# mbertagna/Galaxy-Deconv

Hardware: AMD Instinct MI355X
Metric: galaxies/sec (256x256, n_iters=8) - unrolled ADMM spectral engine (higher is better)
Workload: dtype f32; 1 GPU; Unrolled_ADMM(n_iters=8, llh='Gaussian') forward, denoiser=identity (spectral engine: SubNet + OTF + init_l2 + 8 ADMM iterations), batch 4096/GPU, 256x256 fp32 (BASELINE.json configs[2]/[3]); global_batch=4096, n_iters=8, llh=Gaussian, parallelism=dp1 (batch shards, no data-path collective), ranks_seen=1, backend=none, pipeline_streams=2, init=fused, k_psf_rows + k_gal_reg_init (one launch)

## Files before the change

### galaxy-deconv_amd/csrc/gd_engine.hip

```cpp
#include <hip/hip_runtime.h>

#include <algorithm>
#include <cstdio>
#include <cstdlib>
#include <cstring>
#include <map>
#include <mutex>
#include <string>
#include <vector>

#include "../../include/gdeconv.h"
#include "gd_fft.hpp"
#include "gd_subnet.hpp"

namespace gd {

struct GalScalar {
    const float* p;
    long long stride;
    __device__ __forceinline__ float operator()(int g) const { return p[(long long)g * stride]; }
};

struct Args {
    int N;
    float2* T;
    float2* otf;
    const float* y;
    const float* psf;
    long long psf_gstride;
    int h;
    const float* a0;
    const float* a1;
    const float* a2;
    float* o0;
    float* o1;
    float* o2;
    GalScalar alpha, rho1, rho2, rho2n;
    int llh;
    int last;
    int first;
    float* s_hh;
    float2* s_g;
    float2* s_u1;
    float2* s_w;
    int t_slot;
    float2* Tw;
    const float* ltl;
    long long ltl_gstride;
    int otf_bcast;
    float2* s_x;
    int gH, gW;
    int pw;
    int rev;
    int tail;
    GalScalar rho1n;
    const float* a3;
    float* o3;
    float* part;
    float* apart;
};

enum RowFwdMode { RF_ITER, RF_PSF_Y, RF_PSF_YP, RF_PSF_RAW, RF_PSF, RF_ONE, RF_TWO, RF_YA, RF_PSF_YAR,
                  RF_PADV, RF_PSF_YPAD, RF_PAD2,
                  RF_TRAIN_BWD,
                  RF_TRAINF_BWD };
enum ColMode { C_ITER, C_OTF_INIT, C_OTF_CONV, C_WIENER, C_OTF, C_CONV, C_CONVC, C_CONV2, C_FWD, C_INV,
               C_G_INIT, C_G_ITER, C_G_W1, C_G_ITER_F, C_G_ITER_L, C_G_ITER_FL,
               C_TIKHONOV, C_POWER, C_GX_INIT, C_GX, C_GX_BWD,
               C_TRAIN, C_TRAIN_BWD,
               C_OTF_BWD, C_XCORR,
               C_TRAINF, C_TRAINF_BWD };
enum RowInvMode { RI_ITER, RI_INIT, RI_OUT1, RI_OUT2, RI_RL_FINAL, RI_CROP, RI_CROP_BWD,
                  RI_TRAIN, RI_TRAIN_BWD,
                  RI_PSF_BWD,
                  RI_TRAINF };
enum RowInvFwdMode { RIF_CLAMP, RIF_RL_RATIO, RIF_RL_UPDATE };

constexpr int rows_per_block(int lpb, int L) {
    int rw = lpb < L ? lpb : L;
    while (L % rw || rw % 2) --rw;
    return rw;
}
constexpr int cmax(int x, int y) { return x > y ? x : y; }

template <int L>
struct Geo {
    static constexpr int F1 = Plan<L>::F1, F2 = Plan<L>::F2;
    static constexpr int K = L / 2 + 1;
    static constexpr int LPB = 256 / F1;
    static constexpr int RB = rows_per_block(LPB, L);
    static constexpr int RLD = L + 2;
    static constexpr int XCH = xch_elems<L>();
    static constexpr int COL_LDS = LPB * XCH;
    static_assert(L % RB == 0 && RB % 2 == 0, "rows per block must be even and divide L");
};

__device__ __forceinline__ size_t tidx(int g, int img, int k, int row, int K, int L) {
    return ((size_t)(g * 2 + img) * K + k) * L + row;
}

__device__ __forceinline__ float shifted_psf(const Args& a, int g, int r, int c, int L) {
    const int c0 = a.h >> 1;
    int i = r + c0, jj = c + c0;
    if (i >= L) i -= L;
    if (jj >= L) jj -= L;
    if (i >= a.h || jj >= a.h) return 0.0f;
    return a.psf[(long long)g * a.psf_gstride + (long long)i * a.h + jj];
}

__device__ __forceinline__ float v_step(int llh, float vt, float yp, float rho2, float alpha) {
    if (llh == GD_LLH_POISSON) {
        const float t1 = rho2 * vt - alpha;
        return 0.5f * (1.0f / rho2) * (-t1 + sqrtf(t1 * t1 + 4.0f * yp * rho2));
    }
    return (rho2 * vt + yp / alpha) / (1.0f + rho2);
}

__device__ __forceinline__ void v_step_grad(int llh, float vt, float yp, float rho2, float alpha, float& dvt,
                                            float& drho) {
    if (llh == GD_LLH_POISSON) {
        const float t1 = rho2 * vt - alpha;
        const float s = sqrtf(t1 * t1 + 4.0f * yp * rho2);
        const float sm = t1 > 0.f ? 4.0f * yp * rho2 / (s + t1) : s - t1;
        const float ir = 1.0f / rho2;
        const float v = 0.5f * ir * sm;
        dvt = -0.5f * sm / s;
        drho = (yp - rho2 * v * vt) * ir / s - v * ir;
        return;
    }
    const float q = 1.0f / (1.0f + rho2);
    dvt = rho2 * q;
    drho = (vt - yp / alpha) * q * q;
}

__device__ __forceinline__ void v_step_grad_in(int llh, float vt, float yp, float rho2, float alpha, float& dy,
                                               float& dal) {
    if (llh == GD_LLH_POISSON) {
        const float t1 = rho2 * vt - alpha;
        const float s = sqrtf(t1 * t1 + 4.0f * yp * rho2);
        const float sm = t1 > 0.f ? 4.0f * yp * rho2 / (s + t1) : s - t1;
        dy = 1.0f / s;
        dal = 0.5f * sm / (rho2 * s);
        return;
    }
    const float q = 1.0f / (alpha * (1.0f + rho2));
    dy = q;
    dal = -yp * q / alpha;
}

template <int L, int NI, int RBX = 0>
struct RowGeo {
    using G = Geo<L>;
    static constexpr int RB = RBX ? RBX : rows_per_block(2 * G::LPB / NI, L);
    static constexpr int PAIRS = RB / 2;
    static constexpr int LINES = NI * PAIRS;
    static constexpr int THREADS = LINES * G::F1;
    static constexpr int LDS = cmax(cmax(LINES * G::RLD, LINES * G::XCH), (NI * RB * L + 1) / 2);
    static_assert(RB % 2 == 0 && L % RB == 0, "row pairs must tile the image");
    static_assert(THREADS <= 1024, "block too large");
};

template <int L, typename R>
__device__ __forceinline__ void split_store(const Args& a, const float2* rowbuf, int g, int row0, int tid) {
    using G = Geo<L>;
    for (int idx = tid; idx < R::LINES * G::K; idx += R::THREADS) {
        const int m = idx % R::PAIRS, t = idx / R::PAIRS;
        const int k = t % G::K, im = t / G::K;
        const int line = im * R::PAIRS + m;
        const float2 C = rowbuf[line * G::RLD + k];
        const float2 D = rowbuf[line * G::RLD + (k == 0 ? 0 : L - k)];
        *reinterpret_cast<float4*>((a.Tw ? a.Tw : a.T) + tidx(g, im + a.t_slot, k, row0 + 2 * m, G::K, L)) =
            make_float4(0.5f * (C.x + D.x), 0.5f * (C.y - D.y), 0.5f * (C.y + D.y), 0.5f * (D.x - C.x));
    }
}

template <int L, typename R>
__device__ __forceinline__ void gather_rows(const Args& a, float2* rowbuf, int g, int row0, int tid) {
    using G = Geo<L>;
    for (int idx = tid; idx < R::LINES * G::K; idx += R::THREADS) {
        const int m = idx % R::PAIRS, t = idx / R::PAIRS;
        const int k = t % G::K, im = t / G::K;
        const float4 q = *reinterpret_cast<const float4*>(a.T + tidx(g, im, k, row0 + 2 * m, G::K, L));
        float2 Re = make_float2(q.x, q.y), Ro = make_float2(q.z, q.w);
        const bool self = (k == 0) || (2 * k == L);
        if (self) {
            Re.y = 0.f;
            Ro.y = 0.f;
        }
        const int line = im * R::PAIRS + m;
        rowbuf[line * G::RLD + k] = make_float2(Re.x - Ro.y, Re.y + Ro.x);
        if (!self) rowbuf[line * G::RLD + (L - k)] = make_float2(Re.x + Ro.y, Ro.x - Re.y);
    }
}

template <int MODE>
struct RfTraits {
    static constexpr int NI = (MODE == RF_PSF || MODE == RF_ONE || MODE == RF_YA || MODE == RF_PADV) ? 1 : 2;
};

__device__ __forceinline__ float4 ld4(const float* p) { return *reinterpret_cast<const float4*>(p); }
__device__ __forceinline__ void st4(float* p, float4 v) { *reinterpret_cast<float4*>(p) = v; }
__device__ __forceinline__ float f4(const float4& v, int i) { return i == 0 ? v.x : i == 1 ? v.y : i == 2 ? v.z : v.w; }
__device__ __forceinline__ void f4set(float4& v, int i, float x) {
    if (i == 0) v.x = x; else if (i == 1) v.y = x; else if (i == 2) v.z = x; else v.w = x;
}

template <int L, int MODE>
__device__ __forceinline__ float4 rf_source4(const Args& a, int g, int im, int r, int c, size_t pix) {
    if constexpr (MODE == RF_ITER) {
        if (im == 0) {
            const float4 z = ld4(a.a0 + pix), u = ld4(a.a1 + pix);
            return make_float4(z.x - u.x, z.y - u.y, z.z - u.z, z.w - u.w);
// ... 50 lines not shown
    } else if constexpr (MODE == RF_YA) {
        const float4 y = ld4(a.y + pix);
        const float al = a.alpha(g);
        return make_float4(fmaxf(y.x, 0.f) / al, fmaxf(y.y, 0.f) / al, fmaxf(y.z, 0.f) / al, fmaxf(y.w, 0.f) / al);
    } else {
        return ld4((im == 0 ? a.a0 : a.a1) + pix);
    }
}

template <int L>
__device__ __forceinline__ float4 rf_train_bwd4(const Args& a, int g, int im, size_t pix, float& acc) {
    if (im == 0) {
        const float4 gz = ld4(a.a0 + pix);
        if (a.last) {
            const float sc = a.llh == GD_LLH_POISSON ? a.alpha(g) : 1.f;
            return make_float4(gz.x * sc, gz.y * sc, gz.z * sc, gz.w * sc);
        }
        const float4 gu = ld4(a.a1 + pix);
        return make_float4(2.f * gz.x + gu.x, 2.f * gz.y + gu.y, 2.f * gz.z + gu.z, 2.f * gz.w + gu.w);
    }
    if (a.last) return make_float4(0.f, 0.f, 0.f, 0.f);
    const float4 gw = ld4(a.a2 + pix), vt = ld4(a.a3 + pix), y = ld4(a.y + pix);
    const float al = a.alpha(g), r2n = a.rho2n(g);
    float4 ghx, wp;
#pragma unroll
    for (int e = 0; e < 4; ++e) {
        float dvt, drho;
        v_step_grad(a.llh, f4(vt, e), fmaxf(f4(y, e), 0.f), r2n, al, dvt, drho);
        const float gwe = f4(gw, e), gvt = gwe * dvt;
        acc += gwe * drho;
        f4set(ghx, e, 2.f * gvt - gwe);
        f4set(wp, e, gwe - gvt);
    }
    st4(a.o2 + pix, wp);
    return ghx;
}

template <int L>
__device__ __forceinline__ float4 rf_trainf_bwd4(const Args& a, int g, int im, size_t pix, float& acc, float& acc2) {
    if (im == 0) {
        const float4 gz = ld4(a.a0 + pix);
        if (a.last) {
            float sc = 1.f;
            if (a.llh == GD_LLH_POISSON) {
                const float4 x = ld4(a.a3 + pix);
                sc = a.alpha(g);
                acc2 += gz.x * x.x + gz.y * x.y + gz.z * x.z + gz.w * x.w;
            }
            return make_float4(gz.x * sc, gz.y * sc, gz.z * sc, gz.w * sc);
        }
        const float4 gu = ld4(a.a1 + pix);
        return make_float4(2.f * gz.x + gu.x, 2.f * gz.y + gu.y, 2.f * gz.z + gu.z, 2.f * gz.w + gu.w);
    }
    if (a.last) {
        st4(a.o3 + pix, make_float4(0.f, 0.f, 0.f, 0.f));
        return make_float4(0.f, 0.f, 0.f, 0.f);
    }
    const float4 gw = ld4(a.a2 + pix), vt = ld4(a.a3 + pix), y = ld4(a.y + pix);
    const float al = a.alpha(g), r2n = a.rho2n(g);
    float4 ghx, wp, gy;
#pragma unroll
    for (int e = 0; e < 4; ++e) {
        float dvt, drho, dy, dal;
        const float ye = f4(y, e), yp = fmaxf(ye, 0.f);
        v_step_grad(a.llh, f4(vt, e), yp, r2n, al, dvt, drho);
        v_step_grad_in(a.llh, f4(vt, e), yp, r2n, al, dy, dal);
        const float gwe = f4(gw, e), gvt = gwe * dvt;
        acc += gwe * drho;
        acc2 += gwe * dal;
        f4set(ghx, e, 2.f * gvt - gwe);
        f4set(wp, e, gwe - gvt);
        f4set(gy, e, ye > 0.f ? gwe * dy : 0.f);
    }
    st4(a.o2 + pix, wp);
    st4(a.o3 + pix, gy);
    return ghx;
}

template <int L, int MODE, int RBX = 0>
__global__ __launch_bounds__((RowGeo<L, RfTraits<MODE>::NI, RBX>::THREADS)) void k_row_fwd(Args a) {
    constexpr int NI = RfTraits<MODE>::NI;
    using G = Geo<L>;
    using R = RowGeo<L, NI, RBX>;
    constexpr int F1 = G::F1, F2 = G::F2;
    __shared__ float2 tw[L];
    __shared__ __attribute__((aligned(16))) float2 lds[R::LDS];
    const int tid = threadIdx.x;
    const int blocks_per_g = L / R::RB;
    const int g = blockIdx.x / blocks_per_g;
    const int row0 = (blockIdx.x - g * blocks_per_g) * R::RB;
    const int line = tid / F1, j = tid - line * F1;
    const int im = line / R::PAIRS, m = line - im * R::PAIRS;
    fill_twiddles<L>(tw, tid, R::THREADS);
    float* stage = reinterpret_cast<float*>(lds);
    [[maybe_unused]] float acc = 0.f, acc2 = 0.f;
    for (int q = tid * 4; q < NI * R::RB * L; q += R::THREADS * 4) {
        const int imq = q / (R::RB * L), rem = q - imq * (R::RB * L);
        const int rr = rem / L, c = rem - rr * L;
        const size_t pix = ((size_t)g * L + row0 + rr) * L + c;
        if constexpr (MODE == RF_TRAIN_BWD) st4(stage + q, rf_train_bwd4<L>(a, g, imq, pix, acc));
        else if constexpr (MODE == RF_TRAINF_BWD) st4(stage + q, rf_trainf_bwd4<L>(a, g, imq, pix, acc, acc2));
        else st4(stage + q, rf_source4<L, MODE>(a, g, imq, row0 + rr, c, pix));
    }
    if constexpr (MODE == RF_TRAINF_BWD) {
        __shared__ float red2[R::THREADS];
        red2[tid] = acc2;
        __syncthreads();
        if (tid < 64) {
            float sum = 0.f;
            for (int i = tid; i < R::THREADS; i += 64) sum += red2[i];
            red2[tid] = sum;
        }
        __syncthreads();
        if (tid < R::RB) {
            float sum = 0.f;
            if (tid == 0)
                for (int i = 0; i < (R::THREADS < 64 ? R::THREADS : 64); ++i) sum += red2[i];
            a.apart[(size_t)g * L + row0 + tid] = sum;
        }
    }
    if constexpr (MODE == RF_TRAIN_BWD || MODE == RF_TRAINF_BWD) {
        __shared__ float red[R::THREADS];
        red[tid] = acc;
        __syncthreads();
        if (tid < 64) {
            float sum = 0.f;
            for (int i = tid; i < R::THREADS; i += 64) sum += red[i];
            red[tid] = sum;
        }
        __syncthreads();
        if (tid < R::RB) {
            float sum = 0.f;
            if (tid == 0)
                for (int i = 0; i < (R::THREADS < 64 ? R::THREADS : 64); ++i) sum += red[i];
            a.part[(size_t)g * (2 * G::K + L) + 2 * G::K + row0 + tid] = sum;
        }
    }
    __syncthreads();
    float2 v[F2];
#pragma unroll
    for (int s = 0; s < F2; ++s) {
        const int c = j + F1 * s;
        v[s] = make_float2(stage[(im * R::RB + 2 * m) * L + c], stage[(im * R::RB + 2 * m + 1) * L + c]);
    }
    __syncthreads();
    line_fft<L, false>(v, j, lds + line * G::XCH, tw);
    __syncthreads();
#pragma unroll
    for (int s = 0; s < F2; ++s) lds[line * G::RLD + j + F1 * s] = v[s];
    __syncthreads();
    split_store<L, R>(a, lds, g, row0, tid);
}

template <int L, bool TO_STATE = false>
__global__ __launch_bounds__(256) void k_psf_rows(Args a) {
    using G = Geo<L>;
    constexpr int F1 = G::F1, F2 = G::F2, LPB = G::LPB, K = G::K;
    __shared__ float2 tw[L];
    __shared__ __attribute__((aligned(16))) float2 lds[cmax(LPB * G::RLD, LPB * G::XCH)];
    const int tid = threadIdx.x, line = tid / F1, j = tid - line * F1;
    const int h = a.h, c0 = h >> 1, pairs = h >> 1;
    const int blocks_per_g = (pairs + LPB - 1) / LPB;
    const int g = blockIdx.x / blocks_per_g;
    const int p0 = (blockIdx.x - g * blocks_per_g) * LPB;
    fill_twiddles<L>(tw, tid, 256);
    const int p = p0 + line;
    const float* ps = a.psf + (long long)g * a.psf_gstride + (long long)(2 * p) * h;
    float2 v[F2];
#pragma unroll
    for (int s = 0; s < F2; ++s) {
        int jj = j + F1 * s + c0;
        if (jj >= L) jj -= L;
        v[s] = (p < pairs && jj < h) ? make_float2(ps[jj], ps[h + jj]) : make_float2(0.f, 0.f);
    }
    __syncthreads();
    line_fft<L, false>(v, j, lds + line * G::XCH, tw);
    __syncthreads();
#pragma unroll
    for (int s = 0; s < F2; ++s) lds[line * G::RLD + j + F1 * s] = v[s];
    __syncthreads();
    float2* P = TO_STATE ? a.s_u1 + (size_t)g * K * L : a.T + tidx(g, 1, 0, 0, K, L);
    for (int idx = tid; idx < LPB * K; idx += 256) {
        const int m = idx % LPB, k = idx / LPB;
        if (p0 + m >= pairs) continue;
        const float2 C = lds[m * G::RLD + k];
        const float2 D = lds[m * G::RLD + (k == 0 ? 0 : L - k)];
        float4 o = make_float4(0.5f * (C.x + D.x), 0.5f * (C.y - D.y), 0.5f * (C.y + D.y), 0.5f * (D.x - C.x));
        if (TO_STATE && k == 0) {
            const float2 Cn = lds[m * G::RLD + L / 2];
            o = make_float4(C.x, Cn.x, C.y, Cn.y);
        }
        *reinterpret_cast<float4*>(P + (size_t)k * h + 2 * (p0 + m)) = o;
    }
}

template <int MODE>
struct ColTraits {
    static constexpr bool IN2 = (MODE == C_ITER || MODE == C_OTF_INIT || MODE == C_OTF_CONV ||
                                 MODE == C_WIENER || MODE == C_CONV2 || MODE == C_TIKHONOV || MODE == C_GX_INIT ||
                                 MODE == C_GX_BWD || MODE == C_TRAIN || MODE == C_TRAIN_BWD || MODE == C_XCORR ||
                                 MODE == C_TRAINF || MODE == C_TRAINF_BWD);
    static constexpr bool OUT2 = (MODE == C_ITER || MODE == C_CONV2 || MODE == C_TRAIN || MODE == C_TRAIN_BWD ||
                                  MODE == C_TRAINF || MODE == C_TRAINF_BWD);
    static constexpr bool HAS_OUT = (MODE != C_OTF && MODE != C_FWD && MODE != C_G_W1 && MODE != C_POWER &&
                                     MODE != C_XCORR);
    static constexpr bool STORE_OTF = (MODE == C_OTF_INIT || MODE == C_OTF_CONV || MODE == C_OTF);
    static constexpr bool LOAD_OTF = (MODE == C_ITER || MODE == C_CONV || MODE == C_CONVC || MODE == C_CONV2 ||
                                      MODE == C_TRAIN || MODE == C_TRAIN_BWD || MODE == C_TRAINF || MODE == C_TRAINF_BWD);
    static constexpr bool FWD = (MODE != C_INV && MODE != C_OTF_BWD);
};

#ifndef GD_RCP_DIV
#define GD_RCP_DIV 1
#endif
__device__ __forceinline__ float ld_s(const float* p) { return *p; }
__device__ __forceinline__ float2 ld_s(const float2* p) { return *p; }
__device__ __forceinline__ void st_s(float* p, float v) { __builtin_nontemporal_store(v, p); }
__device__ __forceinline__ void st_s(float2* p, float2 v) {
    unsigned long long u;
    __builtin_memcpy(&u, &v, 8);
    __builtin_nontemporal_store(u, reinterpret_cast<unsigned long long*>(p));
}
typedef float f4v __attribute__((ext_vector_type(4)));
template <int L>
__device__ __forceinline__ int sidx_c(int ky) {
    if constexpr (L == 256) {
        const int j = ky & 15, s = ky >> 4;
        return 32 * (s >> 1) + 2 * j + (s & 1);
    } else {
        return ky;
    }
}
template <int L>
__device__ __forceinline__ int sidx_h(int ky) {
    if constexpr (L == 256) {
        const int j = ky & 15, s = ky >> 4;
        return 64 * (s >> 2) + 4 * j + (s & 3);
    } else {
        return ky;
    }
}
template <int L>
__device__ __forceinline__ size_t sflat_c(size_t o) {
    if constexpr (L == 256) return (o & ~size_t(255)) | (size_t)sidx_c<L>((int)(o & 255));
    else return o;
}
template <int L>
__device__ __forceinline__ size_t sflat_h(size_t o) {
    if constexpr (L == 256) return (o & ~size_t(255)) | (size_t)sidx_h<L>((int)(o & 255));
    else return o;
}
__device__ __forceinline__ float2 w1_value(float hh, float2 Gk, float2 Xk, float r2n) {
    const float d0 = 1.0f + r2n;
#if GD_RCP_DIV
    const float rd = __builtin_amdgcn_rcpf(d0);
    return make_float2((r2n * (hh * Xk.x + 0.0f) + Gk.x) * rd, (r2n * (hh * Xk.y + 0.0f) + Gk.y) * rd);
#else
    return make_float2((r2n * (hh * Xk.x + 0.0f) + Gk.x) / d0, (r2n * (hh * Xk.y + 0.0f) + Gk.y) / d0);
#endif
}

struct GState {
    float hh;
    float2 G, U1, W;
};
template <int L, bool FIRST, bool LAST>
__device__ __forceinline__ GState gauss_load(const Args& a, size_t o) {
    GState st;
    const size_t oc = sflat_c<L>(o);
    st.hh = ld_s(a.s_hh + sflat_h<L>(o));
    st.G = make_float2(0.f, 0.f);
    st.U1 = make_float2(0.f, 0.f);
    if constexpr (!LAST || FIRST) st.G = ld_s(a.s_g + oc);
    if constexpr (!FIRST) st.U1 = ld_s(a.s_u1 + oc);
    st.W = ld_s(a.s_w + oc);
    return st;
}
template <bool LAST>
__device__ __forceinline__ float2 gauss_math_w(float hh, float2 Gk, float2 U1, float2 Wt, float2 Zk, float r1, float r2,
                                               float r2w, float r2n, float inv_n, float2& U1o, float2& Wo) {
    const float lhs = r1 * hh + r2;
    const float2 A = csub(Zk, U1);
#if GD_RCP_DIV
    const float rl = __builtin_amdgcn_rcpf(lhs);
    const float2 X = make_float2((r1 * A.x + r2w * Wt.x) * rl, (r1 * A.y + r2w * Wt.y) * rl);
#else
    const float2 X = make_float2((r1 * A.x + r2w * Wt.x) / lhs, (r1 * A.y + r2w * Wt.y) / lhs);
#endif
    if constexpr (LAST) return cscale(X, inv_n);
    const float2 U1n = csub(cadd(U1, X), Zk);
    const float2 HHX = cscale(X, hh);
    const float2 U2t = csub(HHX, Wt);
    const float d = 1.0f + r2n;
#if GD_RCP_DIV
    const float rd = __builtin_amdgcn_rcpf(d);
    const float2 Vt = make_float2((r2n * (HHX.x + U2t.x) + Gk.x) * rd, (r2n * (HHX.y + U2t.y) + Gk.y) * rd);
#else
    const float2 Vt = make_float2((r2n * (HHX.x + U2t.x) + Gk.x) / d, (r2n * (HHX.y + U2t.y) + Gk.y) / d);
#endif
    U1o = U1n;
    Wo = csub(Vt, U2t);
    return cscale(cadd(X, U1n), inv_n);
}
template <bool LAST>
__device__ __forceinline__ float2 gauss_math(float hh, float2 Gk, float2 U1, float2 Wt, float2 Zk, float r1, float r2,
                                             float r2n, float inv_n, float2& U1o, float2& Wo) {
    return gauss_math_w<LAST>(hh, Gk, U1, Wt, Zk, r1, r2, r2, r2n, inv_n, U1o, Wo);
}
__device__ __forceinline__ float2 gauss_math_rt(float hh, float2 Gk, float2 U1, float2 Wt, float2 Zk, float r1,
                                                float r2, float r2w, float r2n, float inv_n, float2& U1o, float2& Wo,
                                                bool last) {
    if (last) return gauss_math_w<true>(hh, Gk, U1, Wt, Zk, r1, r2, r2w, r2n, inv_n, U1o, Wo);
    return gauss_math_w<false>(hh, Gk, U1, Wt, Zk, r1, r2, r2w, r2n, inv_n, U1o, Wo);
}
__device__ __forceinline__ float2 gauss_tail_c(float2 U1n, float2 Wn, float r1n, float r2n) {
    return make_float2(r2n * Wn.x - r1n * U1n.x, r2n * Wn.y - r1n * U1n.y);
}
template <int L, bool FIRST, bool LAST>
__device__ __forceinline__ float2 gauss_iter_st(const Args& a, size_t o, float2 Zk, const GState& st, float r1,
                                                float r2, float r2n, bool valid, float inv_n) {
    const float hh = st.hh;
    const float2 U1 = st.U1, Gk = st.G;
    float2 Wt = st.W;
    if constexpr (FIRST) Wt = w1_value(hh, Gk, st.W, r2);
    const float lhs = r1 * hh + r2;
    const float2 A = csub(Zk, U1);
#if GD_RCP_DIV
    const float rl = __builtin_amdgcn_rcpf(lhs);
    const float2 X = make_float2((r1 * A.x + r2 * Wt.x) * rl, (r1 * A.y + r2 * Wt.y) * rl);
#else
    const float2 X = make_float2((r1 * A.x + r2 * Wt.x) / lhs, (r1 * A.y + r2 * Wt.y) / lhs);
#endif
    if constexpr (LAST) return cscale(X, inv_n);
    const float2 U1n = csub(cadd(U1, X), Zk);
// ... 144 lines not shown
            if (valid) {
                a.s_hh[sflat_h<L>(ob + ky)] = hh;
                a.s_g[sflat_c<L>(ob + ky)] = a.llh == GD_LLH_POISSON ? Hk2 : Gk;
            }
            const float lhs = hh + 1.0f / al;
            P[s] = cscale(make_float2(Gk.x / lhs, Gk.y / lhs), inv_n);
        } else if constexpr (giter) {
            P[s] = gauss_iter_elem<L, gfirst, glast>(a, ob + ky, P[s], r1, r2, r2n, valid, inv_n);
        } else if constexpr (MODE == C_G_W1) {
            if (valid)
                a.s_w[sflat_c<L>(ob + ky)] = a.llh == GD_LLH_POISSON ? cmul(a.s_g[sflat_c<L>(ob + ky)], P[s]) : P[s];
        } else if constexpr (MODE == C_WIENER) {
            const float HtH = Hk.x * Hk.x + Hk.y * Hk.y;
            const float div = HtH + 350.0f / al;
            const float2 num = cmulc(Q[s], Hk);
            P[s] = cscale(make_float2(num.x / div, num.y / div), inv_n);
        } else if constexpr (MODE == C_TIKHONOV) {
            const float HtH = Hk.x * Hk.x + Hk.y * Hk.y;
            const float div = a.ltl ? HtH + lam * a.ltl[(size_t)g * a.ltl_gstride + (size_t)kx * L + ky] : HtH + lam;
            const float2 num = cmulc(Q[s], Hk);
            P[s] = cscale(make_float2(num.x / div, num.y / div), inv_n);
        } else if constexpr (MODE == C_GX_INIT) {
            const float2 Hk2 = P[s];
            const float hh = Hk2.x * Hk2.x + Hk2.y * Hk2.y;
            const float2 Gk = cmulc(Q[s], Hk2);
            if (valid) {
                a.s_hh[ob + ky] = hh;
                a.s_g[ob + ky] = Gk;
            }
            const float lhs = hh + 1.0f / al;
            P[s] = cscale(make_float2(Gk.x / lhs, Gk.y / lhs), inv_n);
        } else if constexpr (MODE == C_GX) {
            const float hh = a.s_hh[ob + ky];
            const float2 Gk = a.s_g[ob + ky];
            const float lhs = rgx + hh;
            const float2 rhs = cadd(Gk, P[s]);
            const float2 X = make_float2(rhs.x / lhs, rhs.y / lhs);
            if (a.s_w && valid) a.s_w[ob + ky] = X;
            P[s] = cscale(X, inv_n);
        } else if constexpr (MODE == C_GX_BWD) {
            const float hh = a.s_hh[ob + ky];
            const float D = rgx + hh;
            const float2 X = a.s_w[ob + ky];
            const float2 d = csub(Q[s], X);
            const float wk = (kx == 0 || 2 * kx == L) ? 1.f : 2.f;
            drho += wk * (P[s].x * d.x + P[s].y * d.y) / D;
            P[s] = cscale(make_float2(P[s].x / D, P[s].y / D), inv_n);
        } else if constexpr (MODE == C_POWER) {
            if (valid) a.s_hh[ob + ky] = P[s].x * P[s].x + P[s].y * P[s].y;
        } else if constexpr (MODE == C_OTF_CONV) {
            P[s] = cscale(cmul(Q[s], Hk), inv_n);
        } else if constexpr (MODE == C_CONV) {
            P[s] = cscale(cmul(P[s], Hk), inv_n);
        } else if constexpr (MODE == C_CONVC) {
            P[s] = cscale(cmulc(P[s], Hk), inv_n);
        } else if constexpr (MODE == C_CONV2) {
            P[s] = cscale(cmul(P[s], Hk), inv_n);
            Q[s] = cscale(cmul(Q[s], Hk), inv_n);
        } else if constexpr (MODE == C_INV) {
            P[s] = cscale(P[s], inv_n);
        } else if constexpr (MODE == C_OTF_BWD) {
            P[s] = cscale(P[s], (kx == 0 || 2 * kx == L) ? 1.f : 0.5f);
        } else if constexpr (MODE == C_XCORR) {
            const float wk = ((kx == 0 || 2 * kx == L) ? 1.f : 2.f) * inv_n;
            if (valid) a.otf[ob + ky] = cscale(a.last ? cmulc(Q[s], P[s]) : cmulc(P[s], Q[s]), wk);
        }
    }
    if constexpr (MODE == C_GX_BWD) {
#pragma unroll
        for (int off = F1 / 2; off > 0; off >>= 1) drho += __shfl_xor(drho, off, F1);
        if (valid && j == 0) a.o2[(size_t)g * K + kx] = drho * inv_n;
    }
    if constexpr (MODE == C_TRAIN_BWD || MODE == C_TRAINF_BWD) {
#pragma unroll
        for (int off = F1 / 2; off > 0; off >>= 1) drho += __shfl_xor(drho, off, F1);
        if (valid && j == 0) {
            float* pg = a.part + (size_t)g * (2 * K + L);
            pg[kx] = -(r2 / r1) * (drho * inv_n);
            pg[K + kx] = drho * inv_n;
        }
    }
    if constexpr (TR::HAS_OUT && MODE != C_FWD && VAR != 1) {
        line_fft<L, true, CLEAN, CDPP>(P, j, my, tw);
        if constexpr (TR::OUT2) line_fft<L, true, CLEAN, CDPP>(Q, j, my, tw);
    }
    if (valid) {
        if constexpr (MODE == C_FWD) {
#pragma unroll
            for (int s = 0; s < F2; ++s) a.T[c0 + j + F1 * s] = P[s];
        } else if constexpr (TR::HAS_OUT) {
#pragma unroll
            for (int s = 0; s < F2; ++s) {
                a.T[c0 + j + F1 * s] = P[s];
                if constexpr (TR::OUT2) a.T[c1 + j + F1 * s] = Q[s];
            }
        }
    }
}

__device__ __forceinline__ int opaque(int v) {
    asm volatile("" : "+v"(v));
    return v;
}

#if GD_FUSED_TRACE
__device__ unsigned long long* g_fused_trace;
#define GD_TRACE(k)                                                                                   \
    if (tid == 0) g_fused_trace[(size_t)blockIdx.x * 16 + (k)] = __builtin_amdgcn_s_memrealtime()
#else
#define GD_TRACE(k)
#endif

template <int L>
struct FusedGeo {
    static constexpr int F1 = Plan<L>::F1, F2 = Plan<L>::F2, K = L / 2 + 1;
    static constexpr int THREADS = 1024, LINES = THREADS / F1;
    static constexpr int NP = L / 2, PPL = NP / LINES;
    static constexpr int KS = L / 4;
    static constexpr int SLD = 2 * KS + 4;
    static constexpr int ALD = KS + 2;
    static constexpr int XCH = xch_elems<L>();
    static constexpr int U = cmax(cmax(NP * SLD, L * ALD), LINES * XCH);
    static_assert(LINES == KS, "one column per line and slice");
    static_assert(NP == 2 * LINES && PPL == 2, "two row pairs per line; half the rows per inverse pass");
    static_assert(KS % F1 == 0 && (L / 2) % F1 == 0, "slice edges on lane-register boundaries");
    static_assert(L <= THREADS && (NP * KS) % THREADS == 0, "Nyquist column: one element per thread");
};

template <int L, int SLD = FusedGeo<L>::SLD>
__device__ __forceinline__ void fused_gather(const float2* S, int c, int j, float2 (&C)[FusedGeo<L>::F2]) {
    using FG = FusedGeo<L>;
    c = opaque(c);
    j = opaque(j);
#pragma unroll
    for (int s = 0; s < FG::F2; ++s) {
        const int y = j + FG::F1 * s;
        const float2 u = S[(y >> 1) * SLD + c], v = S[(y >> 1) * SLD + FG::KS + c];
        C[s] = (y & 1) ? make_float2(0.5f * (u.y + v.y), 0.5f * (v.x - u.x))
                       : make_float2(0.5f * (u.x + v.x), 0.5f * (u.y - v.y));
    }
}

__device__ __forceinline__ void lds_barrier() {
    __builtin_amdgcn_fence(__ATOMIC_RELEASE, "workgroup", "local");
    __builtin_amdgcn_s_barrier();
    __builtin_amdgcn_fence(__ATOMIC_ACQUIRE, "workgroup", "local");
}

template <int L>
__device__ __forceinline__ void init_hload(const Args& a, float2 (&Hc)[FusedGeo<L>::F2], int g, int kx, int j) {
    using FG = FusedGeo<L>;
    static_assert((L & (L - 1)) == 0, "power-of-two side");
    const int h = a.h, c0p = h >> 1;
    const float2* P0 = a.s_u1 + (size_t)g * FG::K * L + (size_t)opaque(kx) * h;
    j = opaque(j);
    static_assert(FG::F1 == 16 && FG::F2 == 16, "sparse OTF column for 16 x 16 lines");
#pragma unroll
    for (int s = 0; s < FG::F2; ++s) {
        Hc[s] = make_float2(0.f, 0.f);
        if (s < 2 || s >= FG::F2 - 2) {
            const int i = (j + FG::F1 * s + c0p) & (L - 1);
            if (i < h) Hc[s] = P0[i];
        }
    }
}
template <int L>
__device__ __forceinline__ void init_hload4(const Args& a, float2 (&h4)[4], int g, int kx, int j) {
    using FG = FusedGeo<L>;
    const int h = a.h, c0p = h >> 1;
    const float2* P0 = a.s_u1 + (size_t)g * FG::K * L + (size_t)opaque(kx) * h;
    j = opaque(j);
#pragma unroll
    for (int t = 0; t < 4; ++t) {
        const int s = t < 2 ? t : FG::F2 - 4 + t;
        const int i = (j + FG::F1 * s + c0p) & (L - 1);
        h4[t] = i < h ? P0[i] : make_float2(0.f, 0.f);
    }
}
template <int L>
__device__ __forceinline__ void init_hcol(float2 (&Hc)[FusedGeo<L>::F2], const float2 (&h4)[4]) {
    using FG = FusedGeo<L>;
#pragma unroll
    for (int s = 0; s < FG::F2; ++s) Hc[s] = make_float2(0.f, 0.f);
    Hc[0] = h4[0];
    Hc[1] = h4[1];
    Hc[FG::F2 - 2] = h4[2];
    Hc[FG::F2 - 1] = h4[3];
}
template <int L>
__device__ __forceinline__ float2 init_bin(const Args& a, size_t o, float2 Yk, float2 Hk, float al, float inv_n,
                                           bool store_h = false) {
    const float hh = Hk.x * Hk.x + Hk.y * Hk.y;
    const float2 Gk = cmulc(Yk, Hk);
    a.s_hh[sflat_h<L>(o)] = hh;
    a.s_g[sflat_c<L>(o)] = store_h ? Hk : Gk;
    const float lhs = hh + 1.0f / al;
    return cscale(make_float2(Gk.x / lhs, Gk.y / lhs), inv_n);
}
template <int L>
__device__ __forceinline__ void w1_bin(const Args& a, size_t o, float2 Xk) {
    a.s_w[sflat_c<L>(o)] = a.llh == GD_LLH_POISSON ? cmul(a.s_g[sflat_c<L>(o)], Xk) : Xk;
}
#include "gd_galreg.hpp"
#include "gd_rlreg.hpp"
#include "gd_poisreg.hpp"

template <int L>
__device__ __forceinline__ void small_split(const float2 (&v)[Plan<L>::F2], int j, float2* my, float2* D, int r) {
    constexpr int F1 = Plan<L>::F1, F2 = Plan<L>::F2, K = L / 2 + 1;
#pragma unroll
    for (int s = 0; s < F2; ++s) my[j + F1 * s] = v[s];
    wave_lds_sync();
    for (int k = j; k < K; k += F1) {
        const float2 C = my[k], Dm = my[k == 0 ? 0 : L - k];
        D[k * L + r] = make_float2(0.5f * (C.x + Dm.x), 0.5f * (C.y - Dm.y));
        D[k * L + r + 1] = make_float2(0.5f * (C.y + Dm.y), 0.5f * (Dm.x - C.x));
    }
    wave_lds_sync();
}
template <int L>
__device__ __forceinline__ void small_gather(const float2* D, int j, int r, float2 (&v)[Plan<L>::F2]) {
    constexpr int F1 = Plan<L>::F1, F2 = Plan<L>::F2;
#pragma unroll
    for (int s = 0; s < F2; ++s) {
        const int k = j + F1 * s;
        const bool self = (k == 0) || (2 * k == L);
        float2 be, bo;
        if (2 * k <= L) {
            be = D[k * L + r];
            bo = D[k * L + r + 1];
        } else {
            be = cconj(D[(L - k) * L + r]);
            bo = cconj(D[(L - k) * L + r + 1]);
        }
        if (self) {
            be.y = 0.f;
            bo.y = 0.f;
        }
        v[s] = make_float2(be.x - bo.y, be.y + bo.x);
    }
}

#ifndef GD_SMALL_ZPRE
#define GD_SMALL_ZPRE 1
#endif
template <int L, bool FIRST, bool LAST>
__global__ __launch_bounds__(256) void k_gal_small(Args a) {
    constexpr int F1 = Plan<L>::F1, F2 = Plan<L>::F2, K = L / 2 + 1, LINES = 256 / F1, XCH = xch_elems<L>();
    static_assert(XCH >= L + 2, "row buffer inside the exchange area");
    constexpr float inv_n = float(1.0 / double(L * L));
    __shared__ float2 tw[L];
    __shared__ float2 S[K * L];
    __shared__ float2 xch[LINES * XCH];
    const int tid = threadIdx.x, line = tid / F1, j = tid - line * F1;
    const int g = blockIdx.x;
    float2* my = xch + line * XCH;
    GD_TRACE(0);
    constexpr bool ZPRE = GD_SMALL_ZPRE && L / 2 <= LINES;
    const float* z = a.a0 + (size_t)g * L * L;
    float2 zv[ZPRE ? F2 : 1];
    if (ZPRE && line < L / 2) {
#pragma unroll
        for (int s = 0; s < (ZPRE ? F2 : 0); ++s)
            zv[s] = make_float2(z[(2 * line) * L + j + F1 * s], z[(2 * line + 1) * L + j + F1 * s]);
    }
    fill_twiddles<L>(tw, tid, 256);
    const float r1 = a.rho1(g), r2 = a.rho2(g), r2n = LAST ? 0.f : a.rho2n(g);
    constexpr bool PRE = L <= 64;
    GState pre[PRE ? F2 : 1];
    if (PRE && line < K) {
        const size_t ob = ((size_t)g * K + line) * L + j;
#pragma unroll
        for (int s = 0; s < (PRE ? F2 : 0); ++s) pre[s] = gauss_load<L, FIRST, LAST>(a, ob + F1 * s);
    }
    __syncthreads();
    GD_TRACE(1);

    for (int p = line; p < L / 2; p += LINES) {
        float2 v[F2];
        if constexpr (ZPRE) {
#pragma unroll
            for (int s = 0; s < F2; ++s) v[s] = zv[s];
        } else {
#pragma unroll
            for (int s = 0; s < F2; ++s) v[s] = make_float2(z[(2 * p) * L + j + F1 * s], z[(2 * p + 1) * L + j + F1 * s]);
        }
        line_fft<L, false>(v, j, my, tw);
        small_split<L>(v, j, my, S, 2 * p);
    }
    __syncthreads();
    GD_TRACE(2);

    for (int kx = line; kx < K; kx += LINES) {
        float2 v[F2];
#pragma unroll
        for (int s = 0; s < F2; ++s) v[s] = S[kx * L + j + F1 * s];
        line_fft<L, false>(v, j, my, tw);
        const size_t ob = ((size_t)g * K + kx) * L + j;
        if (PRE && kx == line) {
#pragma unroll
            for (int s = 0; s < (PRE ? F2 : 0); ++s)
                v[s] = gauss_iter_st<L, FIRST, LAST>(a, ob + F1 * s, v[s], pre[s], r1, r2, r2n, true, inv_n);
        } else {
#pragma unroll
            for (int s = 0; s < F2; ++s)
                v[s] = gauss_iter_elem<L, FIRST, LAST>(a, ob + F1 * s, v[s], r1, r2, r2n, true, inv_n);
        }
        line_fft<L, true>(v, j, my, tw);
#pragma unroll
        for (int s = 0; s < F2; ++s) S[kx * L + j + F1 * s] = v[s];
    }
    __syncthreads();
    GD_TRACE(3);

    float* out = a.o0 + (size_t)g * L * L;
    for (int p = line; p < L / 2; p += LINES) {
        float2 v[F2];
        small_gather<L>(S, j, 2 * p, v);
        line_fft<L, true>(v, j, my, tw);
#pragma unroll
        for (int s = 0; s < F2; ++s) {
            out[(2 * p) * L + j + F1 * s] = v[s].x;
            out[(2 * p + 1) * L + j + F1 * s] = v[s].y;
// ... 1016 lines not shown
__global__ __launch_bounds__(256) void k_sparse_power(const int* rc, const float* vals, int ntaps, float* out,
                                                      int H, int W, int K) {
    const int idx = blockIdx.x * 256 + threadIdx.x;
    if (idx >= K * H) return;
    const int kx = idx / H, ky = idx - kx * H;
    const long long HW = (long long)H * W;
    double re = 0.0, im = 0.0;
    for (int t = 0; t < ntaps; ++t) {
        const long long ph = ((long long)ky * rc[2 * t] * W + (long long)kx * rc[2 * t + 1] * H) % HW;
        double sn, cs;
        sincospi(-2.0 * double(ph) / double(HW), &sn, &cs);
        re += double(vals[t]) * cs;
        im += double(vals[t]) * sn;
    }
    out[idx] = float(re * re + im * im);
}

thread_local std::string g_last_error;

constexpr const char* kRowFwdName = "k_row_fwd";
constexpr const char* kPsfRowsName = "k_psf_rows";
constexpr const char* kColName = "k_col";
constexpr const char* kRowInvName = "k_row_inv";
constexpr const char* kRowInvFwdName = "k_row_invfwd";
constexpr const char* kGalRegName = "k_gal_reg";
constexpr const char* kGalInitName = "k_gal_init";
constexpr const char* kGalSmallName = "k_gal_small";
constexpr const char* kGalSmallInitName = "k_gal_small_init";

inline int fail(int code, const char* msg) {
    g_last_error = msg;
    return code;
}
inline int fail(int code, const std::string& msg) {
    g_last_error = msg;
    return code;
}

inline int check_launch(const char* what) {
    hipError_t e = hipGetLastError();
    if (e != hipSuccess) {
        g_last_error = std::string(what) + ": " + hipGetErrorString(e);
        return GD_ERR_HIP;
    }
    return GD_OK;
}

struct ProfEntry {
    std::string name;
    hipEvent_t start, stop;
};
struct ProfStat {
    double ms = 0.0;
    long long launches = 0;
};
std::mutex g_prof_mu;
int g_prof_level = 0;
std::vector<ProfEntry> g_prof_pending;
std::vector<hipEvent_t> g_prof_pool;
std::map<std::string, ProfStat> g_prof_stats;

inline hipEvent_t prof_event() {
    if (!g_prof_pool.empty()) {
        hipEvent_t e = g_prof_pool.back();
        g_prof_pool.pop_back();
        return e;
    }
    hipEvent_t e;
    (void)hipEventCreate(&e);
    return e;
}

struct ProfScope {
    bool on;
    ProfEntry ent;
    hipStream_t st;
    ProfScope(const std::string& name, hipStream_t s, int level = 2) : on(false), st(s) {
        std::lock_guard<std::mutex> lk(g_prof_mu);
        if (g_prof_level < level) return;
        on = true;
        ent.name = name;
        ent.start = prof_event();
        ent.stop = prof_event();
        (void)hipEventRecord(ent.start, st);
    }
    ~ProfScope() {
        if (!on) return;
        (void)hipEventRecord(ent.stop, st);
        std::lock_guard<std::mutex> lk(g_prof_mu);
        g_prof_pending.push_back(ent);
    }
};

template <int L>
struct Launcher {
    using G = Geo<L>;
    template <int NI>
    static int row_grid(int N) { return N * (L / RowGeo<L, NI>::RB); }
    static int col_grid(int N) { return (N * G::K + G::LPB - 1) / G::LPB; }
    static std::string nm(const char* k, int mode) {
        return std::string(k) + "<" + std::to_string(L) + "," + std::to_string(mode) + ">";
    }

    template <int MODE>
    static int rf(const Args& a, hipStream_t st) {
        ProfScope ps(nm(kRowFwdName, MODE), st);
        hipLaunchKernelGGL((k_row_fwd<L, MODE>), dim3(row_grid<RfTraits<MODE>::NI>(a.N)), dim3(RowGeo<L, RfTraits<MODE>::NI>::THREADS), 0, st, a);
        return check_launch("k_row_fwd");
    }
    static int psf_rows(const Args& a, hipStream_t st) {
        ProfScope ps(nm(kPsfRowsName, 0), st);
        const int bpg = (a.h / 2 + G::LPB - 1) / G::LPB;
        hipLaunchKernelGGL((k_psf_rows<L>), dim3(a.N * bpg), dim3(256), 0, st, a);
        return check_launch("k_psf_rows");
    }
    template <int MODE>
    static int col(const Args& a, hipStream_t st) {
        ProfScope ps(nm(kColName, MODE), st);
        hipLaunchKernelGGL((k_col<L, MODE>), dim3(col_grid(a.N)), dim3(256), 0, st, a);
        return check_launch("k_col");
    }
    template <int MODE>
    static int ri(const Args& a, hipStream_t st) {
        ProfScope ps(nm(kRowInvName, MODE), st);
        hipLaunchKernelGGL((k_row_inv<L, MODE>), dim3(row_grid<RiTraits<MODE>::NI>(a.N)), dim3(RowGeo<L, RiTraits<MODE>::NI>::THREADS), 0, st, a);
        return check_launch("k_row_inv");
    }
    static int psf_rows_state(const Args& a, hipStream_t st) {
        ProfScope ps(nm(kPsfRowsName, 1), st);
        const int bpg = (a.h / 2 + G::LPB - 1) / G::LPB;
        hipLaunchKernelGGL((k_psf_rows<L, true>), dim3(a.N * bpg), dim3(256), 0, st, a);
        return check_launch("k_psf_rows");
    }
    template <bool FIRST, bool LAST>
    static int gal_small_v(const Args& a, hipStream_t st) {
        ProfScope ps(nm(kGalSmallName, FIRST + 2 * LAST), st);
        if constexpr (L == 48)
            hipLaunchKernelGGL((k_gal_small_p<L, 8, 6, FIRST, LAST>), dim3(a.N), dim3(256), 0, st, a);
        else
            hipLaunchKernelGGL((k_gal_small<L, FIRST, LAST>), dim3(a.N), dim3(256), 0, st, a);
        return check_launch("k_gal_small");
    }
    static int gal_small_init(const Args& a, hipStream_t st) {
        ProfScope ps(nm(kGalSmallInitName, 0), st);
        hipLaunchKernelGGL((k_gal_small_init<L>), dim3(a.N), dim3(256), 0, st, a);
        return check_launch("k_gal_small_init");
    }
    static int gal_small(const Args& a, hipStream_t st) {
        if (a.first) return a.last ? gal_small_v<true, true>(a, st) : gal_small_v<true, false>(a, st);
        return a.last ? gal_small_v<false, true>(a, st) : gal_small_v<false, false>(a, st);
    }
    static int gal_reg(const Args& a, hipStream_t st) {
        ProfScope ps(nm(kGalRegName, a.first + 2 * a.last), st);
        if (a.tail == 1)
            hipLaunchKernelGGL((k_gal_reg<L, false, true>), dim3(a.N), dim3(RegGeo<L>::THREADS), 0, st, a);
        else
            hipLaunchKernelGGL((k_gal_reg<L>), dim3(a.N), dim3(RegGeo<L>::THREADS), 0, st, a);
        return check_launch("k_gal_reg");
    }
    static int pois_a(const Args& a, hipStream_t st) {
        ProfScope ps(nm("k_pois_a", a.first + 2 * a.last), st);
        hipLaunchKernelGGL((k_gal_reg<L, true>), dim3(a.N), dim3(RegGeo<L>::THREADS), 0, st, a);
        return check_launch("k_gal_reg<POIS>");
    }
    static int pois_b(const Args& a, int init, hipStream_t st) {
        ProfScope ps(nm("k_pois_b", init), st);
        hipLaunchKernelGGL((k_pois_b<L>), dim3(a.N), dim3(RegGeo<L>::THREADS), 0, st, a, init);
        return check_launch("k_pois_b");
    }
    static int gal_reg_init_pois(const Args& a, hipStream_t st) {
        ProfScope ps(nm(kGalInitName, 5), st);
        hipLaunchKernelGGL((k_gal_reg_init<L, true>), dim3(a.N), dim3(RegGeo<L>::THREADS), 0, st, a);
        return check_launch("k_gal_reg_init<POIS>");
    }
    static int rl_reg(const Args& a, int n_iters, hipStream_t st) {
        ProfScope ps(nm("k_rl_reg", 0), st);
        hipLaunchKernelGGL((k_rl_reg<L>), dim3(a.N), dim3(RegGeo<L>::THREADS), 0, st, a, n_iters);
        return check_launch("k_rl_reg");
    }
    static int gal_reg_init(const Args& a, hipStream_t st) {
        ProfScope ps(nm(kGalInitName, 4), st);
        hipLaunchKernelGGL((k_gal_reg_init<L>), dim3(a.N), dim3(RegGeo<L>::THREADS), 0, st, a);
        return check_launch("k_gal_reg_init");
    }
    template <int MODE>
    static int rif(const Args& a, hipStream_t st) {
        ProfScope ps(nm(kRowInvFwdName, MODE), st);
        hipLaunchKernelGGL((k_row_invfwd<L, MODE>), dim3(row_grid<1>(a.N)), dim3(RowGeo<L, 1>::THREADS), 0, st, a);
        return check_launch("k_row_invfwd");
    }
};

#define GD_TRY(x)                    \
    do {                             \
        int _rc = (x);               \
        if (_rc != GD_OK) return _rc; \
    } while (0)

size_t g_chunk_bytes = size_t(96) << 20;
int g_pipe_streams = 2;
constexpr int kMaxPipe = 8;
int g_fused = 1;
int g_fused_rl = 1;
int g_subnet_fused_max = 256;
int g_sri_map = 0;
int g_fused_init = 1;
int g_fused_min_n = 96;
int g_combined_tail = [] {
    const char* e = std::getenv("GD_COMBINED_TAIL");
    return (e && e[0] == '0' && e[1] == '\0') ? 0 : 1;
}();
int g_pois2_min_n = 192;
int g_rl_min_n = 96;

constexpr int kCapSets = 64;
struct PipeRes {
    bool ok = false;
    hipStream_t st[kMaxPipe];
    hipEvent_t fork;
    hipEvent_t join[kMaxPipe];
    std::mutex mu;
};
PipeRes g_pipe[64];
std::mutex g_pipe_mu;
struct CapRes {
    hipStream_t st[kMaxPipe];
    hipEvent_t cfork[kCapSets];
    hipEvent_t cjoin[kCapSets][kMaxPipe];
    int cpos = 0;
};
thread_local CapRes* t_cap[64];

thread_local int g_capture_pipe_override = -1;
inline int capture_pipeline_mode() {
    static const int mode = [] {
        const char* e = std::getenv("GD_CAPTURE_PIPELINE");
        const int m = e ? std::atoi(e) : 0;
        return m == 2 ? 2 : 0;
    }();
    return g_capture_pipe_override >= 0 ? g_capture_pipe_override : mode;
}

inline CapRes* cap_res() {
    int dev = 0;
    if (hipGetDevice(&dev) != hipSuccess || dev < 0 || dev >= 64) return nullptr;
    if (t_cap[dev]) return t_cap[dev];
    CapRes* r = new CapRes();
    for (int i = 0; i < kMaxPipe; ++i)
        if (hipStreamCreateWithFlags(&r->st[i], hipStreamNonBlocking) != hipSuccess) return nullptr;
    for (int c = 0; c < kCapSets; ++c) {
        if (hipEventCreateWithFlags(&r->cfork[c], hipEventDisableTiming) != hipSuccess) return nullptr;
        for (int i = 0; i < kMaxPipe; ++i)
            if (hipEventCreateWithFlags(&r->cjoin[c][i], hipEventDisableTiming) != hipSuccess) return nullptr;
    }
    t_cap[dev] = r;
    return r;
}

inline PipeRes* pipe_res() {
    int dev = 0;
    if (hipGetDevice(&dev) != hipSuccess || dev < 0 || dev >= 64) return nullptr;
    std::lock_guard<std::mutex> lk(g_pipe_mu);
    PipeRes& r = g_pipe[dev];
    if (!r.ok) {
        for (int i = 0; i < kMaxPipe; ++i) {
            if (hipStreamCreateWithFlags(&r.st[i], hipStreamNonBlocking) != hipSuccess) return nullptr;
            if (hipEventCreateWithFlags(&r.join[i], hipEventDisableTiming) != hipSuccess) return nullptr;
        }
        if (hipEventCreateWithFlags(&r.fork, hipEventDisableTiming) != hipSuccess) return nullptr;
        r.ok = true;
    }
    return &r;
}

template <int L>
constexpr bool has_fused() { return L == 256; }

inline Args offset_args(const Args& a, int g0, int n, int H, int W) {
    Args b = a;
    b.N = n;
    const size_t img = (size_t)g0 * H * W;
    const size_t spec = (size_t)g0 * (W / 2 + 1) * H;
    if (b.otf && !b.otf_bcast) b.otf += spec;
    if (b.s_hh) b.s_hh += spec;
    if (b.s_g) b.s_g += spec;
    if (b.s_u1) b.s_u1 += spec;
    if (b.s_w) b.s_w += spec;
    if (b.ltl) b.ltl += (long long)g0 * a.ltl_gstride;
    if (b.Tw) b.Tw += 2 * spec;
    if (b.y) b.y += img;
    if (b.a0) b.a0 += img;
    if (b.a1) b.a1 += img;
    if (b.a2) b.a2 += img;
    if (b.o0) b.o0 += img;
    if (b.o1) b.o1 += img;
    if (b.o2) b.o2 += img;
    if (b.a3) b.a3 += img;
    if (b.o3) b.o3 += img;
    if (b.part) b.part += (size_t)g0 * (2 * (W / 2 + 1) + H);
    if (b.apart) b.apart += (size_t)g0 * H;
    if (b.psf) b.psf += (long long)g0 * a.psf_gstride;
    GalScalar* gs[] = {&b.alpha, &b.rho1, &b.rho2, &b.rho2n};
    for (GalScalar* x : gs)
        if (x->p) x->p += (long long)g0 * x->stride;
    return b;
}

template <typename F>
int for_chunks_hw(const Args& a, int H, int W, hipStream_t st, F&& f) {
    const size_t tgal = (size_t)2 * (W / 2 + 1) * H * sizeof(float2);
    int G = a.N;
    if (g_chunk_bytes) {
        const size_t g = g_chunk_bytes / tgal;
        G = (int)(g < 1 ? 1 : (g > (size_t)a.N ? (size_t)a.N : g));
    }
    if (G >= a.N) return f(a, st);
    int S = g_pipe_streams < kMaxPipe ? g_pipe_streams : kMaxPipe;
    if (S > a.N / G) S = a.N / G;
    hipStreamCaptureStatus cap = hipStreamCaptureStatusNone;
    const bool capturing = S > 1 && hipStreamIsCapturing(st, &cap) == hipSuccess && cap != hipStreamCaptureStatusNone;
    if (capturing && capture_pipeline_mode() != 2) S = 1;
    PipeRes* r = (S > 1 && !capturing) ? pipe_res() : nullptr;
    CapRes* cr = (S > 1 && capturing) ? cap_res() : nullptr;
    if (!r && !cr) S = 1;
    std::unique_lock<std::mutex> lk;
    if (r) lk = std::unique_lock<std::mutex>(r->mu);
    hipEvent_t fork = nullptr;
    hipEvent_t* join = nullptr;
    hipStream_t* streams = nullptr;
    if (S > 1) {
        if (cr) {
            const int c = cr->cpos;
            cr->cpos = (c + 1) % kCapSets;
            fork = cr->cfork[c];
            join = cr->cjoin[c];
            streams = cr->st;
        } else {
            fork = r->fork;
            join = r->join;
            streams = r->st;
        }
        if (hipEventRecord(fork, st) != hipSuccess) return fail(GD_ERR_HIP, "pipeline fork");
        for (int i = 0; i < S; ++i)
            if (hipStreamWaitEvent(streams[i], fork, 0) != hipSuccess) return fail(GD_ERR_HIP, "pipeline fork");
    }
    int rc = GD_OK;
    for (int g0 = 0, c = 0; g0 < a.N && rc == GD_OK; g0 += G, ++c) {
        const int n = (a.N - g0 < G) ? a.N - g0 : G;
        Args b = offset_args(a, g0, n, H, W);
        b.T = a.T + (size_t)(c % S) * G * 2 * (W / 2 + 1) * H;
        rc = f(b, S > 1 ? streams[c % S] : st);
    }
    if (S > 1) {
        for (int i = 0; i < S; ++i) {
            if (hipEventRecord(join[i], streams[i]) != hipSuccess || hipStreamWaitEvent(st, join[i], 0) != hipSuccess)
                return fail(GD_ERR_HIP, "pipeline join");
        }
    }
    return rc;
}
template <typename F>
int for_chunks(const Args& a, int L, hipStream_t st, F&& f) {
    return for_chunks_hw(a, L, L, st, std::forward<F>(f));
}

#ifndef GD_REG_REV
#define GD_REG_REV 1
#endif
#ifndef GD_POIS_SMALL
#define GD_POIS_SMALL 1
#endif
inline bool pois_split(int H, int W) {
    return GD_POIS_SMALL && g_fused && g_fused_init && H == W &&
           (H == 32 || H == 48 || H == 64 || H == 80 || H == 96 || H == 112);
}
template <int L>
int pois_small_init_launch(const Args& a, hipStream_t st) {
    using PL = PoisSmallPlan<L>;
    ProfScope ps("k_pois_small_init<" + std::to_string(L) + ">", st);
    if (pois_split(L, L)) hipLaunchKernelGGL((k_pois_small_init<L, PL::TP, PL::TQ, PL::NT, true>), dim3(a.N), dim3(PL::NT), 0, st, a);
    else hipLaunchKernelGGL((k_pois_small_init<L, PL::TP, PL::TQ, PL::NT, false>), dim3(a.N), dim3(PL::NT), 0, st, a);
    return check_launch("k_pois_small_init");
}
template <int L>
int pois_small_launch(const Args& a, hipStream_t st) {
    using PL = PoisSmallPlan<L>;
    static const std::string names[4] = {"k_pois_small<" + std::to_string(L) + ",MID>", "k_pois_small<" + std::to_string(L) + ",FIRST>",
                                         "k_pois_small<" + std::to_string(L) + ",LAST>",
                                         "k_pois_small<" + std::to_string(L) + ",FIRST_LAST>"};
    const bool first = a.first && pois_split(L, L);
    ProfScope ps(names[first + 2 * a.last], st);
    if (first) {
        if (a.last) hipLaunchKernelGGL((k_pois_small<L, PL::TP, PL::TQ, PL::NT, true, true>), dim3(a.N), dim3(PL::NT), 0, st, a);
        else hipLaunchKernelGGL((k_pois_small<L, PL::TP, PL::TQ, PL::NT, false, true>), dim3(a.N), dim3(PL::NT), 0, st, a);
    } else {
        if (a.last) hipLaunchKernelGGL((k_pois_small<L, PL::TP, PL::TQ, PL::NT, true>), dim3(a.N), dim3(PL::NT), 0, st, a);
        else hipLaunchKernelGGL((k_pois_small<L, PL::TP, PL::TQ, PL::NT, false>), dim3(a.N), dim3(PL::NT), 0, st, a);
    }
    return check_launch("k_pois_small");
}

#ifndef GD_MID_EXTRA
#define GD_MID_EXTRA 1
#endif
template <int L>
int gal_mid_launch_t(const Args& a, hipStream_t st);
template <int L>
int gal_mid_init_launch_t(const Args& a, hipStream_t st);
template <int L>
struct Ops {
    static constexpr size_t IMG = (size_t)L * L * 4, HALF = (size_t)(L / 2 + 1) * L * 8;
    using Lc = Launcher<L>;
    static int psf_to_otf(Args a, hipStream_t st) {
        GD_TRY(Lc::template rf<RF_PSF>(a, st));
        return Lc::template col<C_OTF>(a, st);
    }
    static int conv(Args a, int conj, hipStream_t st) {
        GD_TRY(Lc::template rf<RF_ONE>(a, st));
        GD_TRY(conj ? Lc::template col<C_CONVC>(a, st) : Lc::template col<C_CONV>(a, st));
        return Lc::template ri<RI_OUT1>(a, st);
    }
    static int rfft2(Args a, hipStream_t st) {
        GD_TRY(Lc::template rf<RF_ONE>(a, st));
        return Lc::template col<C_FWD>(a, st);
    }
    static int irfft2(Args a, hipStream_t st) {
        GD_TRY(Lc::template col<C_INV>(a, st));
        return Lc::template ri<RI_OUT1>(a, st);
    }
    static int psf_to_otf_bwd(Args a, hipStream_t st) {
        GD_TRY(Lc::template col<C_OTF_BWD>(a, st));
        return Lc::template ri<RI_PSF_BWD>(a, st);
    }
    static int conv_bwd_otf(Args a, hipStream_t st) {
        GD_TRY(Lc::template rf<RF_TWO>(a, st));
        return Lc::template col<C_XCORR>(a, st);
    }
    static int admm_init_pois2(Args a0, hipStream_t st0) {
        if (g_fused_init && a0.h <= 64) {
            GD_TRY(Lc::psf_rows_state(a0, st0));
            GD_TRY(Lc::gal_reg_init_pois(a0, st0));
        } else {
            GD_TRY(for_chunks(a0, L, st0, [&](const Args& a, hipStream_t st) {
                Args b = a;
                GD_TRY(Lc::template rf<RF_YA>(b, st));
                GD_TRY(Lc::psf_rows(b, st));
                GD_TRY(Lc::template col<C_G_INIT>(b, st));
                b.o0 = a.o2;
                b.t_slot = 1;
                GD_TRY(Lc::template rif<RIF_CLAMP>(b, st));
                return Lc::template col<C_G_W1>(b, st);
            }));
        }
        Args b = a0;
        b.s_x = a0.s_w;
        return Lc::pois_b(b, 1, st0);
    }
    static int admm_iter_pois2(Args a, hipStream_t st0) {
        GD_TRY(Lc::pois_a(a, st0));
        if (a.last) return GD_OK;
        return Lc::pois_b(a, 0, st0);
    }
    static int admm_init(Args a0, hipStream_t st0) {
        if constexpr (L <= 112) {
            if (GD_POIS_SMALL && g_fused_init) return pois_small_init_launch<L>(a0, st0);
        }
        return for_chunks(a0, L, st0, [&](const Args& a, hipStream_t st) {
            Args b = a;
            GD_TRY(Lc::template rf<RF_PSF_Y>(b, st));
            GD_TRY(Lc::template col<C_OTF_INIT>(b, st));
            b.o0 = a.o2;
            GD_TRY(Lc::template rif<RIF_CLAMP>(b, st));
            GD_TRY(Lc::template col<C_CONV>(b, st));
            return Lc::template ri<RI_INIT>(a, st);
        });
    }
    static int admm_init_gauss(Args a0, hipStream_t st0) {
        if constexpr (GD_MID_EXTRA && (L == 96 || L == 128)) {
            if (g_fused && g_fused_init) return gal_mid_init_launch_t<L>(a0, st0);
        }
        if constexpr (L <= 96) {
            if (g_fused) return Lc::gal_small_init(a0, st0);
        }
        if constexpr (has_fused<L>()) {
            if (g_fused_init && a0.h <= 64 && a0.N >= g_fused_min_n) {
                GD_TRY(Lc::psf_rows_state(a0, st0));
                return Lc::gal_reg_init(a0, st0);
            }
        }
        return for_chunks(a0, L, st0, [&](const Args& a, hipStream_t st) {
            Args b = a;
            GD_TRY(Lc::template rf<RF_YA>(b, st));
            GD_TRY(Lc::psf_rows(b, st));
            GD_TRY(Lc::template col<C_G_INIT>(b, st));
            b.o0 = a.o2;
            b.t_slot = 1;
            GD_TRY(Lc::template rif<RIF_CLAMP>(b, st));
            return Lc::template col<C_G_W1>(b, st);
        });
    }
    static int admm_iter_gauss(Args a, hipStream_t st0) {
        if constexpr (has_fused<L>()) {
            if (g_fused && a.N >= g_fused_min_n) return Lc::gal_reg(a, st0);
        }
        if constexpr (GD_MID_EXTRA && (L == 96 || L == 128)) {
            if (g_fused) return gal_mid_launch_t<L>(a, st0);
        }
        if constexpr (L <= 128) {
            if (g_fused) return Lc::gal_small(a, st0);
        }
        return for_chunks(a, L, st0, [&](const Args& b, hipStream_t st) {
            GD_TRY(Lc::template rf<RF_ONE>(b, st));
            if (b.first)
                GD_TRY(b.last ? Lc::template col<C_G_ITER_FL>(b, st) : Lc::template col<C_G_ITER_F>(b, st));
            else
                GD_TRY(b.last ? Lc::template col<C_G_ITER_L>(b, st) : Lc::template col<C_G_ITER>(b, st));
            return Lc::template ri<RI_OUT1>(b, st);
        });
    }
    static int admm_iter(Args a0, hipStream_t st0) {
        if constexpr (L <= 112) {
            if (GD_POIS_SMALL && g_fused) return pois_small_launch<L>(a0, st0);
        }
        return for_chunks(a0, L, st0, [&](const Args& a, hipStream_t st) {
            GD_TRY(Lc::template rf<RF_ITER>(a, st));
            GD_TRY(Lc::template col<C_ITER>(a, st));
            return Lc::template ri<RI_ITER>(a, st);
        });
    }
    static int train_init(Args a0, hipStream_t st0) {
        return for_chunks(a0, L, st0, [&](const Args& a, hipStream_t st) {
            GD_TRY(Lc::template rf<RF_PSF_Y>(a, st));
            GD_TRY(Lc::template col<C_OTF_INIT>(a, st));
            GD_TRY(Lc::template rif<RIF_CLAMP>(a, st));
            GD_TRY(Lc::template col<C_CONV>(a, st));
            Args b = a;
            b.o0 = a.o1;
            return Lc::template ri<RI_OUT1>(b, st);
        });
    }
    static int train_iter(Args a0, hipStream_t st0) {
        return for_chunks(a0, L, st0, [&](const Args& a, hipStream_t st) {
            GD_TRY(Lc::template rf<RF_ITER>(a, st));
            GD_TRY(Lc::template col<C_TRAIN>(a, st));
            return Lc::template ri<RI_TRAIN>(a, st);
        });
    }
    static int train_iter_bwd(Args a0, hipStream_t st0) {
        return for_chunks(a0, L, st0, [&](const Args& a, hipStream_t st) {
            GD_TRY(Lc::template rf<RF_TRAIN_BWD>(a, st));
            GD_TRY(Lc::template col<C_TRAIN_BWD>(a, st));
            return Lc::template ri<RI_TRAIN_BWD>(a, st);
        });
    }
    static int train_iter_full(Args a0, hipStream_t st0) {
        return for_chunks(a0, L, st0, [&](const Args& a, hipStream_t st) {
            GD_TRY(Lc::template rf<RF_ITER>(a, st));
            GD_TRY(Lc::template col<C_TRAINF>(a, st));
            return Lc::template ri<RI_TRAINF>(a, st);
        });
    }
    static int train_iter_full_bwd(Args a0, hipStream_t st0) {
        return for_chunks(a0, L, st0, [&](const Args& a, hipStream_t st) {
            GD_TRY(Lc::template rf<RF_TRAINF_BWD>(a, st));
            GD_TRY(Lc::template col<C_TRAINF_BWD>(a, st));
            return Lc::template ri<RI_TRAIN_BWD>(a, st);
        });
    }
    static int wiener(Args a0, hipStream_t st0) {
        return for_chunks(a0, L, st0, [&](const Args& a, hipStream_t st) {
            GD_TRY(Lc::template rf<RF_PSF_RAW>(a, st));
            GD_TRY(Lc::template col<C_WIENER>(a, st));
            return Lc::template ri<RI_OUT1>(a, st);
        });
    }
    static int tikhonov(Args a0, hipStream_t st0) {
        return for_chunks(a0, L, st0, [&](const Args& a, hipStream_t st) {
            GD_TRY(Lc::template rf<RF_PSF_YAR>(a, st));
            GD_TRY(Lc::template col<C_TIKHONOV>(a, st));
            return Lc::template ri<RI_OUT1>(a, st);
        });
    }
    static int gx_init(Args a, hipStream_t st) {
        GD_TRY(Lc::template rf<RF_PSF_YPAD>(a, st));
        GD_TRY(Lc::template col<C_GX_INIT>(a, st));
        return Lc::template ri<RI_CROP>(a, st);
    }
    static int gx_x(Args a, hipStream_t st) {
        GD_TRY(Lc::template rf<RF_PADV>(a, st));
        GD_TRY(Lc::template col<C_GX>(a, st));
        return Lc::template ri<RI_CROP>(a, st);
    }
    static int gx_x_bwd(Args a, hipStream_t st) {
        GD_TRY(Lc::template rf<RF_PAD2>(a, st));
        GD_TRY(Lc::template col<C_GX_BWD>(a, st));
        return Lc::template ri<RI_CROP_BWD>(a, st);
    }
    static int power(Args a, hipStream_t st) {
        GD_TRY(Lc::template rf<RF_ONE>(a, st));
        return Lc::template col<C_POWER>(a, st);
    }
    static int richardson_lucy(Args a0, int n_iters, hipStream_t st0) {
        if constexpr (has_fused<L>()) {
            if (g_fused_rl && n_iters > 0 && a0.N >= g_rl_min_n) {
                GD_TRY(for_chunks(a0, L, st0, [&](const Args& a, hipStream_t st) { return psf_to_otf(a, st); }));
                return Lc::rl_reg(a0, n_iters, st0);
            }
        }
        return for_chunks(a0, L, st0, [&](const Args& a, hipStream_t st) {
            GD_TRY(Lc::template rf<RF_PSF_YP>(a, st));
            if (n_iters <= 0) return GD_OK;
            GD_TRY(Lc::template col<C_OTF_CONV>(a, st));
            for (int it = 0; it < n_iters; ++it) {
                if (it > 0) GD_TRY(Lc::template col<C_CONV>(a, st));
                GD_TRY(Lc::template rif<RIF_RL_RATIO>(a, st));
                GD_TRY(Lc::template col<C_CONVC>(a, st));
                if (it + 1 < n_iters)
                    GD_TRY(Lc::template rif<RIF_RL_UPDATE>(a, st));
                else
                    GD_TRY(Lc::template ri<RI_RL_FINAL>(a, st));
            }
            return GD_OK;
        });
    }
};

inline bool mid_size(int H, int W) { return H == W && (H == 80 || H == 112 || H == 144 || H == 160); }
#ifndef GD_MID_BIG_THREADS
#define GD_MID_BIG_THREADS 512
#endif
#ifndef GD_MID_SMALL_THREADS
#define GD_MID_SMALL_THREADS 256
#endif
template <int L>
constexpr int mid_threads() { return L <= 112 ? GD_MID_SMALL_THREADS : GD_MID_BIG_THREADS; }
template <int L>
int gal_mid_launch_t(const Args& a, hipStream_t st) {
    constexpr int NT = mid_threads<L>(), TP = 16, TQ = L / 16;
    static const std::string names[4] = {"k_gal_mid<" + std::to_string(L) + ",MID>", "k_gal_mid<" + std::to_string(L) + ",FIRST>",
                                         "k_gal_mid<" + std::to_string(L) + ",LAST>",
                                         "k_gal_mid<" + std::to_string(L) + ",FIRST_LAST>"};
    ProfScope ps(names[a.first + 2 * a.last], st);
    if (a.first) {
        if (a.last) hipLaunchKernelGGL((k_gal_mid<L, TP, TQ, NT, true, true>), dim3(a.N), dim3(NT), 0, st, a);
        else hipLaunchKernelGGL((k_gal_mid<L, TP, TQ, NT, true, false>), dim3(a.N), dim3(NT), 0, st, a);
    } else {
        if (a.last) hipLaunchKernelGGL((k_gal_mid<L, TP, TQ, NT, false, true>), dim3(a.N), dim3(NT), 0, st, a);
        else hipLaunchKernelGGL((k_gal_mid<L, TP, TQ, NT, false, false>), dim3(a.N), dim3(NT), 0, st, a);
    }
    return check_launch("k_gal_mid");
}
template <int L>
int gal_mid_init_launch_t(const Args& a, hipStream_t st) {
    constexpr int NT = mid_threads<L>();
    ProfScope ps("k_gal_mid_init<" + std::to_string(L) + ">", st);
    hipLaunchKernelGGL((k_gal_mid_init<L, 16, L / 16, NT>), dim3(a.N), dim3(NT), 0, st, a);
    return check_launch("k_gal_mid_init");
}
inline int gal_mid_launch(const Args& a, hipStream_t st) {
    switch (a.gH) {
        case 80: return gal_mid_launch_t<80>(a, st);
        case 112: return gal_mid_launch_t<112>(a, st);
        case 144: return gal_mid_launch_t<144>(a, st);
        default: return gal_mid_launch_t<160>(a, st);
    }
}
inline int gal_mid_init_launch(const Args& a, hipStream_t st) {
    switch (a.gH) {
        case 80: return gal_mid_init_launch_t<80>(a, st);
        case 112: return gal_mid_init_launch_t<112>(a, st);
        case 144: return gal_mid_init_launch_t<144>(a, st);
        default: return gal_mid_init_launch_t<160>(a, st);
    }
}

#include "gd_generic.hpp"

inline bool specialised_size(int H, int W) {
    if (H != W) return false;
    switch (H) {
        case 32: case 48: case 64: case 96: case 128: case 256: return true;
        default: return false;
    }
}

template <template <int> class OP, typename F>
int dispatch(int H, int W, F&& f) {
    if (H == W) {
        switch (H) {
            case 32: return f(OP<32>{});
            case 48: return f(OP<48>{});
            case 64: return f(OP<64>{});
            case 96: return f(OP<96>{});
            case 128: return f(OP<128>{});
            case 256: return f(OP<256>{});
            default: break;
        }
    }
    if (gen::size_ok(H, W)) return f(GOps{});
    return fail(GD_ERR_UNSUPPORTED, "unsupported image size (H and W must be in [2, 1024])");
}

inline int check_shape(int N, int H, int W) {
    if (N < 0) return fail(GD_ERR_ARG, "negative batch");
    if (!specialised_size(H, W) && !gen::size_ok(H, W))
        return fail(GD_ERR_UNSUPPORTED, "unsupported image size (H and W must be in [2, 1024])");
    return GD_OK;
}

inline int check_psf(int h, int w, int H, int W) {
    if (h != w) return fail(GD_ERR_ARG, "psf must be square (psf_to_otf uses ker.shape[2] for both axes)");
    if (h <= 0 || (h & 1)) return fail(GD_ERR_ARG, "psf side must be even (odd sizes fail in the reference's quadrant copy)");
    if (h > H || h > W) return fail(GD_ERR_ARG, "psf larger than the image");
    return GD_OK;
}

inline Args base_args(int N, void* ws, int H, int W) {
    Args a;
    std::memset(&a, 0, sizeof(a));
    a.N = N;
    a.T = reinterpret_cast<float2*>(ws);
    a.gH = H;
    a.gW = W;
    a.alpha = GalScalar{nullptr, 0};
    a.rho1 = a.rho2 = a.rho2n = a.alpha;
    return a;
}

}

using namespace gd;
#ifndef GD_KERNELS_ONLY

extern "C" {

int gd_abi_version(void) { return GD_ABI_VERSION; }

const char* gd_engine_rev(void) { return "r09.0"; }

#ifndef GD_SRC_HASH
#define GD_SRC_HASH "unknown"
#endif
static const char g_src_hash_marker[] = "gdsrc:" GD_SRC_HASH;
const char* gd_engine_src_hash(void) { return g_src_hash_marker + 6; }

int gd_hip_runtime_version(void) {
    int v = 0;
    if (hipRuntimeGetVersion(&v) != hipSuccess) return fail(GD_ERR_HIP, "hipRuntimeGetVersion");
    return v;
}

const char* gd_last_error(void) { return g_last_error.c_str(); }

int gd_supported_size(int H, int W) {
    if (specialised_size(H, W)) return 1;
    return gen::size_ok(H, W) ? 2 : 0;
}

size_t gd_workspace_bytes(int N, int H, int W) {
    if (!gd_supported_size(H, W) || N <= 0) return 0;
    const size_t K = (size_t)W / 2 + 1;
    return (size_t)N * 2 * K * H * sizeof(float2);
}

size_t gd_otf_bytes(int N, int H, int W) {
    if (!gd_supported_size(H, W) || N <= 0) return 0;
    return (size_t)N * (W / 2 + 1) * H * sizeof(float2);
}

int gd_psf_to_otf(const float* psf, long long psf_gstride, int h, int w, int N, int H, int W,
                  void* otf_half, void* ws, void* stream) {
    GD_TRY(check_shape(N, H, W));
    GD_TRY(check_psf(h, w, H, W));
    if (N == 0) return GD_OK;
    Args a = base_args(N, ws, H, W);
    a.psf = psf; a.psf_gstride = psf_gstride; a.h = h;
    a.otf = reinterpret_cast<float2*>(otf_half);
    return dispatch<Ops>(H, W, [&](auto op) { return decltype(op)::psf_to_otf(a, (hipStream_t)stream); });
}

int gd_conv_fft_batch(const void* otf_half, int conj, const float* x, float* out, int N, int H, int W,
                      void* ws, void* stream) {
    return gd_conv_fft_batch_strided(otf_half, (long long)(W / 2 + 1) * H, conj, x, out, N, H, W, ws, stream);
}

int gd_conv_fft_batch_strided(const void* otf_half, long long otf_gstride, int conj, const float* x, float* out,
                              int N, int H, int W, void* ws, void* stream) {
    GD_TRY(check_shape(N, H, W));
    if (otf_gstride != 0 && otf_gstride != (long long)(W / 2 + 1) * H)
        return fail(GD_ERR_ARG, "otf_gstride must be 0 (one shared OTF) or (W/2+1)*H");
    if (N == 0) return GD_OK;
    Args a = base_args(N, ws, H, W);
    a.otf = reinterpret_cast<float2*>(const_cast<void*>(otf_half));
    a.otf_bcast = otf_gstride == 0;
    a.a0 = x; a.o0 = out;
    return dispatch<Ops>(H, W, [&](auto op) { return decltype(op)::conv(a, conj, (hipStream_t)stream); });
}

int gd_rfft2(const float* x, void* spec, int N, int H, int W, void* stream) {
    GD_TRY(check_shape(N, H, W));
    if (N == 0) return GD_OK;
    Args a = base_args(N, spec, H, W);
    a.a0 = x;
    return dispatch<Ops>(H, W, [&](auto op) { return decltype(op)::rfft2(a, (hipStream_t)stream); });
}

int gd_irfft2(void* spec, float* x, int N, int H, int W, void* stream) {
    GD_TRY(check_shape(N, H, W));
    if (N == 0) return GD_OK;
    Args a = base_args(N, spec, H, W);
    a.o0 = x;
    return dispatch<Ops>(H, W, [&](auto op) { return decltype(op)::irfft2(a, (hipStream_t)stream); });
}

int gd_psf_to_otf_backward(const void* g_otf_half, int h, int w, int N, int H, int W, float* g_psf, void* ws,
                           void* stream) {
    GD_TRY(check_shape(N, H, W));
    GD_TRY(check_psf(h, w, H, W));
    if (N == 0) return GD_OK;
    if (!g_otf_half || !g_psf || !ws) return fail(GD_ERR_ARG, "gd_psf_to_otf_backward: null pointer");
    if ((const void*)g_psf == g_otf_half || (void*)g_psf == ws || g_otf_half == ws)
        return fail(GD_ERR_ARG, "gd_psf_to_otf_backward: g_psf, g_otf_half and ws must be distinct buffers");
    Args a = base_args(N, ws, H, W);
    a.h = h;
    a.otf = reinterpret_cast<float2*>(const_cast<void*>(g_otf_half));
    a.o0 = g_psf;
    return dispatch<Ops>(H, W, [&](auto op) { return decltype(op)::psf_to_otf_bwd(a, (hipStream_t)stream); });
}

int gd_conv_fft_batch_backward_otf(const float* x, const float* g_out, int conj, int N, int H, int W, void* g_otf_half,
                                   void* ws, void* stream) {
    GD_TRY(check_shape(N, H, W));
    if (N == 0) return GD_OK;
    if (!x || !g_out || !g_otf_half || !ws) return fail(GD_ERR_ARG, "gd_conv_fft_batch_backward_otf: null pointer");
    if (g_otf_half == (const void*)x || g_otf_half == (const void*)g_out || g_otf_half == ws)
        return fail(GD_ERR_ARG, "gd_conv_fft_batch_backward_otf: g_otf_half aliases an input or the workspace");
    Args a = base_args(N, ws, H, W);
    a.a0 = g_out; a.a1 = x;
    a.last = conj != 0;
    a.otf = reinterpret_cast<float2*>(g_otf_half);
    return dispatch<Ops>(H, W, [&](auto op) { return decltype(op)::conv_bwd_otf(a, (hipStream_t)stream); });
}

constexpr size_t kStateSlotGap = 256 * 1024;
inline size_t state_slot_gap(int H, int W, int llh) { return (llh == GD_LLH_GAUSSIAN && H == 256 && W == 256) ? kStateSlotGap : 0; }

size_t gd_admm_state_bytes(int N, int H, int W, int llh) {
    if (!gd_supported_size(H, W) || N <= 0) return 0;
    const size_t spec = (size_t)N * (W / 2 + 1) * H * sizeof(float2), img = (size_t)N * H * W * sizeof(float);
    if (llh == GD_LLH_GAUSSIAN)
        return (spec / 8 + 1) / 2 * 8 + 3 * spec + 3 * state_slot_gap(H, W, llh);
    return (H == 256 && W == 256) ? std::max(spec + 2 * img, spec / 2 + 4 * spec + img) : spec + 2 * img;
}

namespace {
bool pois_two_pass(int N, int H, int W, int llh) {
    return llh == GD_LLH_POISSON && H == 256 && W == 256 && g_fused != 0 && N >= g_pois2_min_n;
}
void bind_state(Args& a, void* state, int N, int H, int W, int llh) {
    const size_t spec = (size_t)N * (W / 2 + 1) * H;
    float2* base = reinterpret_cast<float2*>(state);
    if (pois_two_pass(N, H, W, llh)) {
        a.s_hh = reinterpret_cast<float*>(base);
        float2* c = base + spec / 2;
        a.s_g = c;
        a.s_u1 = c + spec;
        a.s_w = c + 2 * spec;
        a.s_x = c + 3 * spec;
        a.o1 = reinterpret_cast<float*>(c + 4 * spec);
        return;
    }
    if (llh == GD_LLH_GAUSSIAN) {
        const size_t gap = state_slot_gap(H, W, llh) / sizeof(float2);
        a.s_hh = reinterpret_cast<float*>(base);
        float2* c = base + (spec + 1) / 2 + gap;
        a.s_g = c;
        a.s_u1 = c + spec + gap;
        a.s_w = c + 2 * (spec + gap);
    } else {
        a.otf = base;
        float* u1 = reinterpret_cast<float*>(base + spec);
        a.o0 = u1;
        a.o1 = u1 + (size_t)N * H * W;
    }
}
}

int gd_admm_state_layout(int N, int H, int W, int llh) {
    if (!gd_supported_size(H, W)) return GD_ERR_UNSUPPORTED;
    if (N < 0) return GD_ERR_ARG;
    if (llh == GD_LLH_GAUSSIAN) return 1;
    if (llh != GD_LLH_POISSON) return GD_ERR_ARG;
    return pois_two_pass(N, H, W, llh) ? 2 : (pois_split(H, W) ? 4 : 3);
}

int gd_admm_init_reads_rho(int H, int W, int llh) {
    if (!gd_supported_size(H, W)) return GD_ERR_UNSUPPORTED;
    if (llh == GD_LLH_GAUSSIAN) return 0;
    if (llh != GD_LLH_POISSON) return GD_ERR_ARG;
    return pois_split(H, W) ? 0 : 1;
}

int gd_admm_init(const float* y, const float* psf, long long psf_gstride, int h, int w,
                 const float* alpha, long long alpha_stride, const float* rho2, long long rho2_stride,
                 int llh, int N, int H, int W, void* state, float* zin, void* ws, void* stream) {
    GD_TRY(check_shape(N, H, W));
    GD_TRY(check_psf(h, w, H, W));
    if (llh != GD_LLH_GAUSSIAN && llh != GD_LLH_POISSON) return fail(GD_ERR_ARG, "llh must be Gaussian or Poisson");
    if (llh == GD_LLH_POISSON && rho2 == nullptr && !pois_split(H, W))
        return fail(GD_ERR_ARG, "the Poisson init takes the first V step: it needs rho2");
    if (N == 0) return GD_OK;
    Args a = base_args(N, ws, H, W);
    a.y = y; a.psf = psf; a.psf_gstride = psf_gstride; a.h = h;
    a.alpha = GalScalar{alpha, alpha_stride};
    a.rho2n = GalScalar{rho2, rho2_stride};
    a.llh = llh;
    bind_state(a, state, N, H, W, llh);
    a.o2 = zin;
    ProfScope ps("op_admm_init<" + std::to_string(H) + "," + std::to_string(llh) + ">", (hipStream_t)stream, 1);
    if (llh == GD_LLH_GAUSSIAN)
        return dispatch<Ops>(H, W, [&](auto op) { return decltype(op)::admm_init_gauss(a, (hipStream_t)stream); });
    if (pois_two_pass(N, H, W, llh)) return Ops<256>::admm_init_pois2(a, (hipStream_t)stream);
    return dispatch<Ops>(H, W, [&](auto op) { return decltype(op)::admm_init(a, (hipStream_t)stream); });
}

int gd_admm_tail_supported(int N, int H, int W, int llh) {
    return llh == GD_LLH_GAUSSIAN && H == 256 && W == 256 && has_fused<256>() && g_fused != 0 && N >= g_fused_min_n &&
                   g_combined_tail != 0
               ? 1
               : 0;
}

int gd_admm_iter_tail(const float* y, const float* z, float* zin_or_out, const float* alpha, long long alpha_stride,
                      const float* rho1, long long rho1_stride, const float* rho2, long long rho2_stride,
                      const float* rho2_next, long long rho2_next_stride, int llh, int iter, int last, int N, int H,
                      int W, void* state, void* ws, void* stream, const float* rho1_next, long long rho1_next_stride,
                      int tail) {
    GD_TRY(check_shape(N, H, W));
    if (llh != GD_LLH_GAUSSIAN && llh != GD_LLH_POISSON) return fail(GD_ERR_ARG, "llh must be Gaussian or Poisson");
    if (tail < 0 || tail > 2) return fail(GD_ERR_ARG, "tail must be 0, 1 (tail-write) or 2 (tail-read)");
    if (tail == 1 && last) return fail(GD_ERR_ARG, "tail = 1 (the next call is the last) with last set");
    if (tail == 1 && rho1_next == nullptr) return fail(GD_ERR_ARG, "tail = 1 needs rho1_next (the last iteration's rho1)");
    if (tail == 2 && !last) return fail(GD_ERR_ARG, "tail = 2 (the W~ slot holds the combined term) is the last call only");
    if (tail == 2 && iter == 0) return fail(GD_ERR_ARG, "tail = 2 follows a tail = 1 call: it cannot be iteration 0");
    if (tail != 0 && !gd_admm_tail_supported(N, H, W, llh))
        return fail(GD_ERR_UNSUPPORTED, "no combined tail on the path this call routes to (gd_admm_tail_supported)");
    if (N == 0) return GD_OK;
    if (!last && rho2_next == nullptr) return fail(GD_ERR_ARG, "rho2_next required unless last");
    Args a = base_args(N, ws, H, W);
    a.y = y;
    bind_state(a, state, N, H, W, llh);
    a.alpha = GalScalar{alpha, alpha_stride};
    a.rho1 = GalScalar{rho1, rho1_stride};
    a.rho2 = GalScalar{rho2, rho2_stride};
    a.rho2n = GalScalar{rho2_next ? rho2_next : rho2, rho2_next ? rho2_next_stride : rho2_stride};
    a.tail = tail;
    if (tail == 1) a.rho1n = GalScalar{rho1_next, rho1_next_stride};
    a.llh = llh;
    a.last = last;
    a.first = iter == 0;
    a.rev = GD_REG_REV ? (llh == GD_LLH_POISSON ? 1 : (iter % 2 == 0)) : 0;
    ProfScope ps("op_admm_iter<" + std::to_string(H) + "," + std::to_string(llh) + ">", (hipStream_t)stream, 1);
    if (llh == GD_LLH_GAUSSIAN) {
        a.a0 = z;
        a.o0 = zin_or_out;
        return dispatch<Ops>(H, W, [&](auto op) { return decltype(op)::admm_iter_gauss(a, (hipStream_t)stream); });
    }
    if (pois_two_pass(N, H, W, llh)) {
        a.a0 = z;
        a.o0 = zin_or_out;
        return Ops<256>::admm_iter_pois2(a, (hipStream_t)stream);
    }
    a.a0 = z; a.a1 = a.o0; a.a2 = a.o1;
    a.o2 = zin_or_out;
    return dispatch<Ops>(H, W, [&](auto op) { return decltype(op)::admm_iter(a, (hipStream_t)stream); });
}

int gd_admm_iter(const float* y, const float* z, float* zin_or_out, const float* alpha, long long alpha_stride,
                 const float* rho1, long long rho1_stride, const float* rho2, long long rho2_stride,
                 const float* rho2_next, long long rho2_next_stride, int llh, int iter, int last, int N, int H,
                 int W, void* state, void* ws, void* stream) {
    return gd_admm_iter_tail(y, z, zin_or_out, alpha, alpha_stride, rho1, rho1_stride, rho2, rho2_stride, rho2_next,
                             rho2_next_stride, llh, iter, last, N, H, W, state, ws, stream, nullptr, 0, 0);
}

int gd_admm_iter_tail_v(const long long* v) {
    if (v == nullptr) return fail(GD_ERR_ARG, "gd_admm_iter_tail_v: null argument vector");
    const auto p = [v](int i) { return reinterpret_cast<void*>(static_cast<intptr_t>(v[i])); };
    return gd_admm_iter_tail(static_cast<const float*>(p(0)), static_cast<const float*>(p(1)), static_cast<float*>(p(2)),
                             static_cast<const float*>(p(3)), v[4], static_cast<const float*>(p(5)), v[6],
                             static_cast<const float*>(p(7)), v[8], static_cast<const float*>(p(9)), v[10], (int)v[11],
                             (int)v[12], (int)v[13], (int)v[14], (int)v[15], (int)v[16], p(17), p(18), p(19),
                             static_cast<const float*>(p(20)), v[21], (int)v[22]);
}

int gd_admm_iter_v(const long long* v) {
    if (v == nullptr) return fail(GD_ERR_ARG, "gd_admm_iter_v: null argument vector");
    const auto p = [v](int i) { return reinterpret_cast<void*>(static_cast<intptr_t>(v[i])); };
    return gd_admm_iter(static_cast<const float*>(p(0)), static_cast<const float*>(p(1)), static_cast<float*>(p(2)),
                        static_cast<const float*>(p(3)), v[4], static_cast<const float*>(p(5)), v[6],
                        static_cast<const float*>(p(7)), v[8], static_cast<const float*>(p(9)), v[10], (int)v[11],
                        (int)v[12], (int)v[13], (int)v[14], (int)v[15], (int)v[16], p(17), p(18), p(19));
}

size_t gd_admm_train_saved_bytes(int N, int H, int W) {
    if (!gd_supported_size(H, W) || N <= 0) return 0;
    return (size_t)N * (W / 2 + 1) * H * sizeof(float2) + (size_t)N * H * W * sizeof(float);
}

int gd_admm_train_init(const float* y, const float* psf, long long psf_gstride, int h, int w, const float* alpha,
                       long long alpha_stride, int N, int H, int W, void* otf_half, float* x0, float* hx0, void* ws,
                       void* stream) {
    GD_TRY(check_shape(N, H, W));
    GD_TRY(check_psf(h, w, H, W));
    if (!y || !psf || !alpha || !otf_half || !x0 || !hx0 || !ws) return fail(GD_ERR_ARG, "gd_admm_train_init: null pointer");
    if (x0 == hx0 || x0 == y || hx0 == y) return fail(GD_ERR_ARG, "gd_admm_train_init: x0, hx0 and y must be distinct buffers");
    if (N == 0) return GD_OK;
    Args a = base_args(N, ws, H, W);
    a.y = y; a.psf = psf; a.psf_gstride = psf_gstride; a.h = h;
    a.alpha = GalScalar{alpha, alpha_stride};
    a.otf = reinterpret_cast<float2*>(otf_half);
    a.o0 = x0; a.o1 = hx0;
    ProfScope ps("op_admm_train_init<" + std::to_string(H) + ">", (hipStream_t)stream, 1);
    return dispatch<Ops>(H, W, [&](auto op) { return decltype(op)::train_init(a, (hipStream_t)stream); });
}

int gd_admm_train_iter(const float* y, const float* z, const float* u1, const float* w, const float* alpha,
                       long long alpha_stride, const float* rho1, long long rho1_stride, const float* rho2,
                       long long rho2_stride, const float* rho2_next, long long rho2_next_stride, int llh, int last,
                       int N, int H, int W, const void* otf_half, float* zin_or_out, float* u1_out, float* w_out,
                       void* saved, void* ws, void* stream) {
    GD_TRY(check_shape(N, H, W));
    if (llh != GD_LLH_GAUSSIAN && llh != GD_LLH_POISSON) return fail(GD_ERR_ARG, "llh must be Gaussian or Poisson");
    if (!y || !z || !u1 || !w || !alpha || !rho1 || !rho2 || !otf_half || !zin_or_out || !saved || !ws)
        return fail(GD_ERR_ARG, "gd_admm_train_iter: null pointer");
    if (!last && (!rho2_next || !u1_out || !w_out))
        return fail(GD_ERR_ARG, "gd_admm_train_iter: rho2_next, u1_out and w_out required unless last");
    {
        const void* in[] = {y, z, u1, w};
        const void* out[] = {zin_or_out, last ? nullptr : u1_out, last ? nullptr : w_out, saved};
        for (int i = 0; i < 4; ++i) {
            if (!out[i]) continue;
            for (const void* p : in)
                if (out[i] == p) return fail(GD_ERR_ARG, "gd_admm_train_iter: an output aliases an input (the body is out of place)");
            for (int k = 0; k < i; ++k)
                if (out[i] == out[k]) return fail(GD_ERR_ARG, "gd_admm_train_iter: two outputs share a buffer");
        }
    }
    if (N == 0) return GD_OK;
    Args a = base_args(N, ws, H, W);
    a.y = y; a.a0 = z; a.a1 = u1; a.a2 = w;
    a.alpha = GalScalar{alpha, alpha_stride};
    a.rho1 = GalScalar{rho1, rho1_stride};
    a.rho2 = GalScalar{rho2, rho2_stride};
    a.rho2n = GalScalar{rho2_next ? rho2_next : rho2, rho2_next ? rho2_next_stride : rho2_stride};
    a.llh = llh;
    a.last = last != 0;
    a.otf = reinterpret_cast<float2*>(const_cast<void*>(otf_half));
    a.o0 = u1_out; a.o1 = w_out; a.o2 = zin_or_out;
    a.s_w = reinterpret_cast<float2*>(saved);
    a.o3 = reinterpret_cast<float*>(a.s_w + (size_t)N * (W / 2 + 1) * H);
    ProfScope ps("op_admm_train_iter<" + std::to_string(H) + "," + std::to_string(llh) + ">", (hipStream_t)stream, 1);
    return dispatch<Ops>(H, W, [&](auto op) { return decltype(op)::train_iter(a, (hipStream_t)stream); });
}

int gd_admm_train_iter_backward(const float* g_zin_or_out, const float* g_u1_out, const float* g_w_out, const float* y,
                                const float* alpha, long long alpha_stride, const float* rho1, long long rho1_stride,
                                const float* rho2, long long rho2_stride, const float* rho2_next,
                                long long rho2_next_stride, int llh, int last, int N, int H, int W, const void* otf_half,
                                const void* saved, float* g_z, float* g_u1, float* g_w, float* g_rho_part, void* ws,
                                void* stream) {
    GD_TRY(check_shape(N, H, W));
    if (llh != GD_LLH_GAUSSIAN && llh != GD_LLH_POISSON) return fail(GD_ERR_ARG, "llh must be Gaussian or Poisson");
    if (!g_zin_or_out || !y || !alpha || !rho1 || !rho2 || !otf_half || !saved || !g_z || !g_u1 || !g_w || !g_rho_part || !ws)
        return fail(GD_ERR_ARG, "gd_admm_train_iter_backward: null pointer");
    if (!last && (!rho2_next || !g_u1_out || !g_w_out))
        return fail(GD_ERR_ARG, "gd_admm_train_iter_backward: rho2_next, g_u1_out and g_w_out required unless last");
    {
        const void* in[] = {g_zin_or_out, g_u1_out, g_w_out, y, saved};
        const void* out[] = {g_z, g_u1, g_w, g_rho_part};
        for (int i = 0; i < 4; ++i) {
            for (const void* p : in)
                if (out[i] == p) return fail(GD_ERR_ARG, "gd_admm_train_iter_backward: an output aliases an input");
            for (int k = 0; k < i; ++k)
                if (out[i] == out[k]) return fail(GD_ERR_ARG, "gd_admm_train_iter_backward: two outputs share a buffer");
        }
    }
    if (N == 0) return GD_OK;
    Args a = base_args(N, ws, H, W);
    a.y = y; a.a0 = g_zin_or_out; a.a1 = g_u1_out; a.a2 = g_w_out;
    a.alpha = GalScalar{alpha, alpha_stride};
    a.rho1 = GalScalar{rho1, rho1_stride};
    a.rho2 = GalScalar{rho2, rho2_stride};
    a.rho2n = GalScalar{rho2_next ? rho2_next : rho2, rho2_next ? rho2_next_stride : rho2_stride};
    a.llh = llh;
    a.last = last != 0;
    a.otf = reinterpret_cast<float2*>(const_cast<void*>(otf_half));
    a.s_w = reinterpret_cast<float2*>(const_cast<void*>(saved));
    a.a3 = reinterpret_cast<const float*>(a.s_w + (size_t)N * (W / 2 + 1) * H);
    a.o0 = g_z; a.o1 = g_u1; a.o2 = g_w;
    a.part = g_rho_part;
    ProfScope ps("op_admm_train_bwd<" + std::to_string(H) + "," + std::to_string(llh) + ">", (hipStream_t)stream, 1);
    return dispatch<Ops>(H, W, [&](auto op) { return decltype(op)::train_iter_bwd(a, (hipStream_t)stream); });
}

size_t gd_admm_train_full_saved_bytes(int N, int H, int W) {
    if (!gd_supported_size(H, W) || N <= 0) return 0;
    return 2 * (size_t)N * (W / 2 + 1) * H * sizeof(float2) + (size_t)N * H * W * sizeof(float);
}

int gd_admm_train_iter_full(const float* y, const float* z, const float* u1, const float* w, const float* alpha,
                            long long alpha_stride, const float* rho1, long long rho1_stride, const float* rho2,
                            long long rho2_stride, const float* rho2_next, long long rho2_next_stride, int llh, int last,
                            int N, int H, int W, const void* otf_half, float* zin_or_out, float* u1_out, float* w_out,
                            void* saved, void* ws, void* stream) {
    GD_TRY(check_shape(N, H, W));
    if (llh != GD_LLH_GAUSSIAN && llh != GD_LLH_POISSON) return fail(GD_ERR_ARG, "llh must be Gaussian or Poisson");
    if (!y || !z || !u1 || !w || !alpha || !rho1 || !rho2 || !otf_half || !zin_or_out || !saved || !ws)
        return fail(GD_ERR_ARG, "gd_admm_train_iter_full: null pointer");
    if (!last && (!rho2_next || !u1_out || !w_out))
        return fail(GD_ERR_ARG, "gd_admm_train_iter_full: rho2_next, u1_out and w_out required unless last");
    {
        const void* in[] = {y, z, u1, w, otf_half};
        const void* out[] = {zin_or_out, last ? nullptr : u1_out, last ? nullptr : w_out, saved};
        for (int i = 0; i < 4; ++i) {
            if (!out[i]) continue;
            for (const void* p : in)
                if (out[i] == p) return fail(GD_ERR_ARG, "gd_admm_train_iter_full: an output aliases an input (the body is out of place)");
            for (int k = 0; k < i; ++k)
                if (out[i] == out[k]) return fail(GD_ERR_ARG, "gd_admm_train_iter_full: two outputs share a buffer");
        }
    }
    if (N == 0) return GD_OK;
    const size_t spec = (size_t)N * (W / 2 + 1) * H;
    Args a = base_args(N, ws, H, W);
    a.y = y; a.a0 = z; a.a1 = u1; a.a2 = w;
    a.alpha = GalScalar{alpha, alpha_stride};
    a.rho1 = GalScalar{rho1, rho1_stride};
    a.rho2 = GalScalar{rho2, rho2_stride};
    a.rho2n = GalScalar{rho2_next ? rho2_next : rho2, rho2_next ? rho2_next_stride : rho2_stride};
    a.llh = llh;
    a.last = last != 0;
    a.otf = reinterpret_cast<float2*>(const_cast<void*>(otf_half));
    a.o0 = u1_out; a.o1 = w_out; a.o2 = zin_or_out;
    a.s_w = reinterpret_cast<float2*>(saved);
    a.s_u1 = a.s_w + spec;
// ... 122 lines not shown
size_t gd_gx_spec_bytes(int N, int H, int W) {
    if (check_gx(N, H, W) != GD_OK || N <= 0) return 0;
    return gx_spec_elems(N, H, W) * sizeof(float2);
}

int gd_gx_init(const float* y, const float* psf, long long psf_gstride, int h, int w, const float* alpha,
               long long alpha_stride, int N, int H, int W, void* state, float* z0, void* ws, void* stream) {
    GD_TRY(check_gx(N, H, W));
    if (h != H || w != W) return fail(GD_ERR_ARG, "UnrolledADMMGaussian pads the PSF like the image: psf must be H x W");
    if (N == 0) return GD_OK;
    Args a = base_args(N, ws, 2 * H, 2 * W);
    a.y = y; a.psf = psf; a.psf_gstride = psf_gstride; a.h = h;
    a.pw = w == h ? 0 : w;
    a.alpha = GalScalar{alpha, alpha_stride};
    bind_gx_state(a, state, N, H, W);
    a.o0 = z0;
    return dispatch<Ops>(2 * H, 2 * W, [&](auto op) { return decltype(op)::gx_init(a, (hipStream_t)stream); });
}

int gd_gx_xupdate(const float* z, float* u, const float* x_prev, const float* rho, long long rho_stride,
                  const float* rho_prev, long long rho_prev_stride, float* x, float* zin, void* xspec,
                  int N, int H, int W, void* state, void* ws, void* stream) {
    GD_TRY(check_gx(N, H, W));
    if (x_prev && (!u || !rho_prev)) return fail(GD_ERR_ARG, "the fused dual update needs u and rho_prev");
    if (N == 0) return GD_OK;
    Args a = base_args(N, ws, 2 * H, 2 * W);
    bind_gx_state(a, state, N, H, W);
    a.a0 = z; a.a1 = u; a.a2 = x_prev; a.o1 = u;
    a.rho1 = GalScalar{rho, rho_stride};
    a.rho2 = GalScalar{rho_prev ? rho_prev : rho, rho_prev ? rho_prev_stride : rho_stride};
    a.s_w = reinterpret_cast<float2*>(xspec);
    a.o0 = x; a.o2 = zin;
    return dispatch<Ops>(2 * H, 2 * W, [&](auto op) { return decltype(op)::gx_x(a, (hipStream_t)stream); });
}

int gd_gx_xupdate_backward(const float* grad_x, const float* z, const float* rho, long long rho_stride,
                           const void* xspec, float* grad_z, float* grad_u, float* grad_rho_part, int N, int H,
                           int W, void* state, void* ws, void* stream) {
    GD_TRY(check_gx(N, H, W));
    if (!xspec) return fail(GD_ERR_ARG, "backward needs the forward's saved spectrum");
    if (N == 0) return GD_OK;
    Args a = base_args(N, ws, 2 * H, 2 * W);
    bind_gx_state(a, state, N, H, W);
    a.a0 = grad_x; a.a1 = z;
    a.rho1 = GalScalar{rho, rho_stride};
    a.s_w = reinterpret_cast<float2*>(const_cast<void*>(xspec));
    a.o0 = grad_z; a.o1 = grad_u; a.o2 = grad_rho_part;
    return dispatch<Ops>(2 * H, 2 * W, [&](auto op) { return decltype(op)::gx_x_bwd(a, (hipStream_t)stream); });
}

int gd_filter_power_taps(const int* rc, const float* vals, int ntaps, float* power_half, int H, int W,
                         void* stream) {
    if (H <= 0 || W <= 0 || H > 4096 || W > 4096) return fail(GD_ERR_UNSUPPORTED, "image sides must be in [1, 4096]");
    if (ntaps < 0 || (ntaps > 0 && (!rc || !vals))) return fail(GD_ERR_ARG, "bad tap list");
    const int K = W / 2 + 1;
    hipLaunchKernelGGL(k_sparse_power, dim3((K * H + 255) / 256), dim3(256), 0, (hipStream_t)stream, rc, vals, ntaps,
                       power_half, H, W, K);
    return check_launch("k_sparse_power");
}

int gd_profile_enable(int level) {
    std::lock_guard<std::mutex> lk(g_prof_mu);
    g_prof_level = level < 0 ? 0 : level;
    return GD_OK;
}

int gd_profile_collect(void) {
    std::lock_guard<std::mutex> lk(g_prof_mu);
    for (auto& e : g_prof_pending) {
        float ms = 0.f;
        if (hipEventSynchronize(e.stop) != hipSuccess || hipEventElapsedTime(&ms, e.start, e.stop) != hipSuccess)
            return fail(GD_ERR_HIP, "profile event query failed");
        ProfStat& st = g_prof_stats[e.name];
        st.ms += ms;
        st.launches += 1;
        g_prof_pool.push_back(e.start);
        g_prof_pool.push_back(e.stop);
    }
    g_prof_pending.clear();
    return (int)g_prof_stats.size();
}

int gd_profile_get(int i, char* name, int name_len, double* total_ms, long long* launches) {
    std::lock_guard<std::mutex> lk(g_prof_mu);
    if (i < 0 || i >= (int)g_prof_stats.size()) return fail(GD_ERR_ARG, "profile index out of range");
    auto it = g_prof_stats.begin();
    std::advance(it, i);
    if (name && name_len > 0) {
        std::strncpy(name, it->first.c_str(), (size_t)name_len - 1);
        name[name_len - 1] = 0;
    }
    if (total_ms) *total_ms = it->second.ms;
    if (launches) *launches = it->second.launches;
    return GD_OK;
}

int gd_profile_reset(void) {
    std::lock_guard<std::mutex> lk(g_prof_mu);
    g_prof_stats.clear();
    return GD_OK;
}

size_t gd_set_chunk_bytes(size_t bytes) {
    const size_t old = g_chunk_bytes;
    g_chunk_bytes = bytes;
    return old;
}

int gd_set_capture_pipeline(int mode) {
    if (mode != -1 && mode != 0 && mode != 2) return fail(GD_ERR_UNSUPPORTED, "capture pipeline mode must be -1, 0 or 2");
    const int old = g_capture_pipe_override;
    g_capture_pipe_override = mode;
    return old;
}

int gd_set_pipeline_streams(int streams) {
    const int old = g_pipe_streams;
    if (streams >= 1) g_pipe_streams = streams < kMaxPipe ? streams : kMaxPipe;
    return old;
}

int gd_set_fused_init(int on) {
    if (on != 0 && on != 1) return fail(GD_ERR_ARG, "gd_set_fused_init: 0 or 1");
    const int old = g_fused_init;
    g_fused_init = on;
    return old;
}

int gd_set_fused_rl(int on) {
    if (on != 0 && on != 1) return fail(GD_ERR_ARG, "gd_set_fused_rl: 0 or 1");
    const int old = g_fused_rl;
    g_fused_rl = on;
    return old;
}

int gd_set_fused_min_batch(int op, int n) {
    int* t = op == GD_LLH_GAUSSIAN ? &g_fused_min_n : op == GD_LLH_POISSON ? &g_pois2_min_n : op == 2 ? &g_rl_min_n : nullptr;
    if (!t) return fail(GD_ERR_ARG, "gd_set_fused_min_batch: op must be 0 (Gaussian), 1 (Poisson) or 2 (Richardson-Lucy)");
    const int old = *t;
    if (n >= 0) *t = n;
    return old;
}

int gd_set_subnet_fused_max(int n) {
    const int old = g_subnet_fused_max;
    if (n >= 0) g_subnet_fused_max = n;
    return old;
}

int gd_set_combined_tail(int on) {
    if (on != 0 && on != 1) return fail(GD_ERR_ARG, "gd_set_combined_tail: 0 or 1");
    const int old = g_combined_tail;
    g_combined_tail = on;
    return old;
}

int gd_set_fused_iteration(int on) {
    if (on != 0 && on != 1) return fail(GD_ERR_ARG, "gd_set_fused_iteration: 0 or 1");
    const int old = g_fused;
    g_fused = on;
    return old;
}

static int subnet_mlp(const float* feat, const float* mlp_params, const float* alpha, long long alpha_stride, float* rhos,
                      int n_out, int N, hipStream_t stream) {
    ProfScope ps("k_subnet_mlp<128,0>", stream, 1);
    if (GD_MLP_MFMA) {
        hipLaunchKernelGGL(gd::subnet::k_subnet_mlp_mfma, dim3((N + gd::subnet::kMG - 1) / gd::subnet::kMG),
                           dim3(gd::subnet::kMlpThreads), 0, stream, feat, mlp_params, alpha, alpha_stride, rhos, n_out, N);
        return check_launch("k_subnet_mlp_mfma");
    }
    hipLaunchKernelGGL(gd::subnet::k_subnet_mlp, dim3((N + gd::subnet::kMlpG - 1) / gd::subnet::kMlpG),
                       dim3(gd::subnet::kMlpThreads), 0, stream, feat, mlp_params, alpha, alpha_stride, rhos, n_out, N);
    return check_launch("k_subnet_mlp");
}

int gd_subnet_param_count(void) { return gd::subnet::kParams; }

int gd_subnet_mlp_param_count(int n_out) {
    return (n_out >= 1 && n_out <= gd::subnet::kMaxOut) ? gd::subnet::mlp_param_count(n_out) : 0;
}

int gd_subnet_rhos(const void* otf128_half, const float* params, const float* mlp_params, const float* alpha,
                   long long alpha_stride, float* feat, float* rhos, int n_out, int N, void* stream) {
    if (N < 0) return fail(GD_ERR_ARG, "negative batch");
    if (n_out < 1 || n_out > gd::subnet::kMaxOut) return fail(GD_ERR_ARG, "n_out must be in [1, 64]");
    if (N == 0) return GD_OK;
    GD_TRY(gd_subnet_features(otf128_half, params, feat, N, stream));
    return subnet_mlp(feat, mlp_params, alpha, alpha_stride, rhos, n_out, N, (hipStream_t)stream);
}

int gd_subnet_rhos_psf(const float* psf, long long psf_gstride, int h, const float* params, const float* mlp_params,
                       const float* alpha, long long alpha_stride, float* feat, float* rhos, int n_out, int N,
                       void* stream) {
    if (N < 0) return fail(GD_ERR_ARG, "negative batch");
    if (n_out < 1 || n_out > gd::subnet::kMaxOut) return fail(GD_ERR_ARG, "n_out must be in [1, 64]");
    if (h < 2 || h > gd::subnet::kPsfMaxH || (h & 1)) return fail(GD_ERR_UNSUPPORTED, "PSF side must be even and <= 64");
    if (N == 0) return GD_OK;
    if (N <= g_subnet_fused_max) {
        ProfScope ps("k_subnet_rhos<128,2>", (hipStream_t)stream, 1);
        hipLaunchKernelGGL(gd::subnet::k_subnet_rhos_psf, dim3(N), dim3(gd::subnet::kThreads), 0, (hipStream_t)stream,
                           psf, psf_gstride, h, params, mlp_params, alpha, alpha_stride, rhos, n_out, N);
        return check_launch("k_subnet_rhos_psf");
    }
    {
        ProfScope ps("k_subnet_features<128,1>", (hipStream_t)stream, 1);
        hipLaunchKernelGGL(gd::subnet::k_subnet_features_psf, dim3(N), dim3(gd::subnet::kThreads), 0,
                           (hipStream_t)stream, psf, psf_gstride, h, params, feat, N);
        GD_TRY(check_launch("k_subnet_features_psf"));
    }
    return subnet_mlp(feat, mlp_params, alpha, alpha_stride, rhos, n_out, N, (hipStream_t)stream);
}

int gd_admm_init_subnet_supported(int N, int H, int W, int h, int w, int llh, int n_out) {
    if (H != W || !(H == 32 || H == 48 || H == 64) || !g_fused) return 0;
    if (llh != GD_LLH_GAUSSIAN && !(llh == GD_LLH_POISSON && pois_split(H, W))) return 0;
    if (h != w || h < 2 || (h & 1) || h > gd::subnet::kPsfMaxH || h > H) return 0;
    return N >= 1 && N <= g_subnet_fused_max && n_out >= 1 && n_out <= gd::subnet::kMaxOut;
}

int gd_admm_init_subnet(const float* y, const float* psf, long long psf_gstride, int h, int w, const float* alpha,
                        long long alpha_stride, int llh, int N, int H, int W, void* state, float* zin,
                        const float* params, const float* mlp_params, float* rhos, int n_out, void* ws, void* stream) {
    GD_TRY(check_shape(N, H, W));
    GD_TRY(check_psf(h, w, H, W));
    if (!gd_admm_init_subnet_supported(N, H, W, h, w, llh, n_out))
        return fail(GD_ERR_UNSUPPORTED, "gd_admm_init_subnet: not fusable here (gd_admm_init_subnet_supported)");
    Args a = base_args(N, ws, H, W);
    a.y = y; a.psf = psf; a.psf_gstride = psf_gstride; a.h = h;
    a.alpha = GalScalar{alpha, alpha_stride};
    a.llh = llh;
    bind_state(a, state, N, H, W, llh);
    a.o2 = zin;
    ProfScope ps("op_admm_init_subnet<" + std::to_string(H) + "," + std::to_string(llh) + ">", (hipStream_t)stream, 1);
    const int map = g_sri_map;
    const dim3 grid(map == 1 ? 2 * ((N + 7) / 8 * 8) : 2 * N), block(gd::subnet::kThreads);
#define GD_SRI_LAUNCH(LL)                                                                                            \
    hipLaunchKernelGGL(k_subnet_rhos_init<LL>, grid, block, 0, (hipStream_t)stream, a, psf, psf_gstride, h, params, \
                       mlp_params, alpha, alpha_stride, rhos, n_out, map)
    if (H == 32) GD_SRI_LAUNCH(32);
    else if (H == 48) GD_SRI_LAUNCH(48);
    else GD_SRI_LAUNCH(64);
#undef GD_SRI_LAUNCH
    return check_launch("k_subnet_rhos_init");
}

int gd_subnet_features(const void* otf128_half, const float* params, float* feat, int N, void* stream) {
    if (N < 0) return fail(GD_ERR_ARG, "negative batch");
    if (N == 0) return GD_OK;
    ProfScope ps("k_subnet_features<128,0>", (hipStream_t)stream, 1);
    hipLaunchKernelGGL(gd::subnet::k_subnet_features, dim3(N), dim3(gd::subnet::kThreads), 0, (hipStream_t)stream,
                       reinterpret_cast<const float2*>(otf128_half), params, feat, N);
    return check_launch("k_subnet_features");
}

}

#include "gd_ingest.hpp"
#endif
```

### galaxy-deconv_amd/csrc/gd_galreg.hpp

```cpp

__device__ __forceinline__ void pin4(float2& a, float2& b, float2& c, float2& d) {
    asm volatile("" : "+v"(a.x), "+v"(a.y), "+v"(b.x), "+v"(b.y), "+v"(c.x), "+v"(c.y), "+v"(d.x), "+v"(d.y));
}
template <int N>
__device__ __forceinline__ void pin(float2 (&v)[N]) {
    static_assert(N % 4 == 0, "pin in fours");
#pragma unroll
    for (int i = 0; i < N; i += 4) pin4(v[i], v[i + 1], v[i + 2], v[i + 3]);
}

__device__ __forceinline__ void drain_vm() { asm volatile("s_waitcnt vmcnt(0)" ::: "memory"); }

__device__ __forceinline__ int soff_c(int kx, int m, int j) { return kx * 256 + 32 * m + 2 * j; }
__device__ __forceinline__ int soff_h(int kx, int q, int j) { return kx * 256 + 64 * q + 4 * j; }
__device__ __forceinline__ f4v ld4v(const void* p) { return *reinterpret_cast<const f4v*>(p); }
__device__ __forceinline__ f4v ld4s(const void* p) { return *reinterpret_cast<const f4v*>(p); }
__device__ __forceinline__ void st4v(void* p, f4v v) { __builtin_nontemporal_store(v, reinterpret_cast<f4v*>(p)); }

__device__ __forceinline__ float2 pois_math(float2 Hk, float2 U1, float2 Wf, float2 Zk, float r1, float r2, float inv_n,
                                            float2& U1o, float2& HXo, bool last) {
    const float hh = Hk.x * Hk.x + Hk.y * Hk.y;
    const float2 Wt = cmulc(Wf, Hk);
    const float lhs = r1 * hh + r2;
    const float2 A = csub(Zk, U1);
    const float rl = __builtin_amdgcn_rcpf(lhs);
    const float2 X = make_float2((r1 * A.x + r2 * Wt.x) * rl, (r1 * A.y + r2 * Wt.y) * rl);
    HXo = cmul(Hk, X);
    if (last) return cscale(X, inv_n);
    const float2 U1n = csub(cadd(U1, X), Zk);
    U1o = U1n;
    return cscale(cadd(X, U1n), inv_n);
}

template <int L, bool POIS = false>
__device__ __forceinline__ float2 gauss_bin4(const Args& a, int g, int ky, float2 Zk, float r1, float r2, float r2n,
                                             bool first, bool last, float r2w, bool tread, bool twrite, float r1n) {
    constexpr float inv_n = float(1.0 / double(L * L));
    const size_t cb = ((size_t)g * (L / 2 + 1) + L / 2) * L;
    const int pc = sidx_c<L>(ky);
    if constexpr (POIS) {
        const float2 U1 = first ? make_float2(0.f, 0.f) : a.s_u1[cb + pc];
        float2 U1n, HXo;
        const float2 r = pois_math(a.s_g[cb + pc], U1, a.s_w[cb + pc], Zk, r1, r2, inv_n, U1n, HXo, last);
        if (!last) {
            st_s(a.s_u1 + cb + pc, U1n);
            st_s(a.s_x + cb + pc, HXo);
        }
        return r;
    }
    const float hh = a.s_hh[cb + sidx_h<L>(ky)];
    const float2 Gk = (last && !first) ? make_float2(0.f, 0.f) : a.s_g[cb + pc];
    const float2 U1 = (first || tread) ? make_float2(0.f, 0.f) : a.s_u1[cb + pc];
    float2 Wt = a.s_w[cb + pc];
    if (first) Wt = w1_value(hh, Gk, Wt, r2);
    float2 U1n, Wn;
    const float2 r = gauss_math_rt(hh, Gk, U1, Wt, Zk, r1, r2, r2w, r2n, inv_n, U1n, Wn, last);
    if (!last) {
        if (twrite) Wn = gauss_tail_c(U1n, Wn, r1n, r2n);
        else st_s(a.s_u1 + cb + pc, U1n);
        st_s(a.s_w + cb + pc, Wn);
    }
    return r;
}

#ifndef GD_REG_DEPTH
#define GD_REG_DEPTH 2
#endif
#ifndef GD_POIS_DEPTH
#define GD_POIS_DEPTH 2
#endif

struct SGroup {
    f4v h, g[2], u[2], w[2];
};
template <int L, bool POIS = false>
__device__ __forceinline__ void sgroup_load(const Args& a, SGroup& G, size_t gb, int kx, int q, int j, bool first,
                                            bool last, bool tread) {
    G.h = POIS ? f4v{0.f, 0.f, 0.f, 0.f} : ld4s(a.s_hh + gb + soff_h(kx, q, j));
#pragma unroll
    for (int h = 0; h < 2; ++h) {
        const size_t off = gb + soff_c(kx, 2 * q + h, j);
        G.g[h] = (!POIS && last && !first) ? f4v{0.f, 0.f, 0.f, 0.f} : ld4s(a.s_g + off);
        G.u[h] = (first || tread) ? f4v{0.f, 0.f, 0.f, 0.f} : ld4s(a.s_u1 + off);
        G.w[h] = ld4s(a.s_w + off);
    }
}
#ifndef GD_REG_PAIR
#define GD_REG_PAIR 3
#endif
#ifndef GD_POIS_PAIR
#define GD_POIS_PAIR 0
#endif
#ifndef GD_POIS_SPF
#define GD_POIS_SPF 1
#endif
#ifndef GD_REG_SPF
#define GD_REG_SPF 1
#endif
template <int L, int NC, bool POIS = false, int D = GD_REG_DEPTH>
__device__ __forceinline__ void fused_prefetch4x(const Args& a, SGroup (&P)[D], int g, int kx0, int kstep, int j, bool first,
                                                 bool last, bool tread) {
    j = opaque(j);
    kx0 = opaque(kx0);
    const size_t gb = (size_t)g * (L / 2 + 1) * L;
#pragma unroll
    for (int t = 0; t < D && t < 4 * NC; ++t) sgroup_load<L, POIS>(a, P[t], gb, kx0 + kstep * (t / 4), t % 4, j, first, last, tread);
    __builtin_amdgcn_sched_barrier(0);
}
template <int L, int NC, bool POIS = false, int D = GD_REG_DEPTH, bool PRE = false, bool TWRITE = false>
__device__ __forceinline__ void fused_update4x(const Args& a, float2 (&C)[NC][16], int g, int kx0, int kstep, int j,
                                               float r1, float r2, float r2n, bool first, bool last, float r2w, bool tread,
                                               float r1n,
                                               const SGroup (*pre)[D] = nullptr) {
    constexpr float inv_n = float(1.0 / double(L * L));
    constexpr int NG = 4 * NC;
    j = opaque(j);
    kx0 = opaque(kx0);
    __builtin_amdgcn_sched_barrier(0);
    const size_t gb = (size_t)g * (L / 2 + 1) * L;
    SGroup G[NG];
#pragma unroll
    for (int t = 0; t < D && t < NG; ++t) {
        if constexpr (PRE) G[t] = (*pre)[t];
        else sgroup_load<L, POIS>(a, G[t], gb, kx0 + kstep * (t / 4), t % 4, j, first, last, tread);
    }
    __builtin_amdgcn_sched_barrier(0);
#pragma unroll
    for (int t = 0; t < NG; ++t) {
        const int u = t / 4, q = t % 4;
        f4v uo[2], wo[2];
#pragma unroll
        for (int e = 0; e < 4; ++e) {
            const int h = e >> 1, c = 2 * (e & 1);
            float2 U1n, Wn;
            const float2 Gk = make_float2(G[t].g[h][c], G[t].g[h][c + 1]);
            float2 Wt = make_float2(G[t].w[h][c], G[t].w[h][c + 1]);
            if constexpr (POIS) {
                C[u][4 * q + e] = pois_math(Gk, make_float2(G[t].u[h][c], G[t].u[h][c + 1]), Wt, C[u][4 * q + e],
                                            r1, r2, inv_n, U1n, Wn, last);
            } else {
                if (first) Wt = w1_value(G[t].h[e], Gk, Wt, r2);
                C[u][4 * q + e] = gauss_math_rt(G[t].h[e], Gk, make_float2(G[t].u[h][c], G[t].u[h][c + 1]), Wt,
                                                C[u][4 * q + e], r1, r2, r2w, r2n, inv_n, U1n, Wn, last);
                if constexpr (TWRITE) Wn = gauss_tail_c(U1n, Wn, r1n, r2n);
            }
            uo[h][c] = U1n.x; uo[h][c + 1] = U1n.y;
            wo[h][c] = Wn.x; wo[h][c + 1] = Wn.y;
        }
        if (!last) {
#pragma unroll
            for (int h = 0; h < 2; ++h) {
                const size_t off = gb + soff_c(kx0 + kstep * u, 2 * q + h, j);
                if constexpr (!TWRITE) st4v(a.s_u1 + off, uo[h]);
                st4v((POIS ? a.s_x : a.s_w) + off, wo[h]);
            }
        }
        if (t + D < NG) sgroup_load<L, POIS>(a, G[t + D], gb, kx0 + kstep * ((t + D) / 4), (t + D) % 4, j, first, last, tread);
        __builtin_amdgcn_sched_barrier(0);
    }
}

#ifndef GD_REG_LEAN
#define GD_REG_LEAN 1
#endif
template <int L, bool INV, bool DPP = false>
__device__ __forceinline__ void reg_fft(float2 (&v)[16], int j, float2* xch, const float2* tw) {
    line_fft<L, INV, GD_REG_LEAN != 0, DPP>(v, j, xch, tw);
}
template <int L, bool INV>
__device__ __forceinline__ void reg_fft2(float2 (&v0)[16], float2 (&v1)[16], int j, float2* xch, const float2* tw) {
    line_fft2<L, INV, GD_REG_LEAN != 0>(v0, v1, j, xch, tw);
}

template <int L>
struct RegGeo {
    static constexpr int F1 = Plan<L>::F1, F2 = Plan<L>::F2, K = L / 2 + 1;
    static constexpr int THREADS = 512, LINES = THREADS / F1;
    static constexpr int NP = L / 2, PPL = NP / LINES;
    static constexpr int KS = L / 4, CPL = KS / LINES;
    static constexpr int SLD = FusedGeo<L>::SLD + 1;
    static constexpr int XCH = xch_elems<L>();
    static constexpr int HPL = (NP / 2) / LINES;
    static constexpr int U = cmax(NP * SLD, LINES * XCH);
    static constexpr int RB0 = KS / F1, RB1 = (L - KS) / F1;
    static constexpr int XA = LINES * XCH;
    static constexpr int PK = (U - XA) / THREADS;
    static constexpr int PXB = PK / PPL;
    static_assert(F1 == 16 && F2 == 16 && PPL == 4 && CPL == 2 && HPL == 2, "256 x 256 geometry");
    static_assert(SLD >= 2 * KS && SLD > L / 2, "row half spectra fit a slice row");
    static_assert(PK >= F2 && PXB >= 1 && RB0 + PXB <= RB1, "parking area above the exchange areas");
};

#ifndef GD_REG_STAGGER
#define GD_REG_STAGGER 60
#endif
#ifndef GD_INIT_STAGGER
#define GD_INIT_STAGGER 60
#endif
#ifndef GD_RL_STAGGER
#define GD_RL_STAGGER 0
#endif
#ifndef GD_STAGGER_N
#define GD_STAGGER_N 4
#endif
#ifndef GD_STAGGER_MIN_N
#define GD_STAGGER_MIN_N 256
#endif
template <int US>
__device__ __forceinline__ void stagger_start(int g, int N) {
    if (US > 0 && N > GD_STAGGER_MIN_N && g < 256 && (g % GD_STAGGER_N) != 0) {
        const unsigned long long t0 = __builtin_amdgcn_s_memrealtime();
        const unsigned long long d = (unsigned long long)US * 100 * (g % GD_STAGGER_N) / GD_STAGGER_N;
        while (__builtin_amdgcn_s_memrealtime() - t0 < d) __builtin_amdgcn_s_sleep(32);
    }
}

template <int L, bool POIS = false, bool TWRITE = false>
__global__ __launch_bounds__(512) void k_gal_reg(Args a) {
    static_assert(!POIS || !TWRITE, "the combined tail is Gaussian only");
    using RG = RegGeo<L>;
    constexpr int F1 = RG::F1, F2 = RG::F2, KS = RG::KS, SLD = RG::SLD, LINES = RG::LINES, T = RG::THREADS;
    constexpr int RB0 = RG::RB0, RB1 = RG::RB1;
    constexpr float inv_n = float(1.0 / double(L * L));
    __shared__ float2 tw[L];
    __shared__ __attribute__((aligned(16))) float2 S[RG::U];
    __shared__ float2 nyq[RG::NP];
    __shared__ float2 nyqc[L];
    __shared__ float2 nyqx[L];
    __shared__ float nyqo[L];
    const int tid = threadIdx.x, line = tid / F1, j = tid - line * F1;
    const int b = blockIdx.x, g = a.rev ? a.N - 1 - b : b;
    const bool l0 = (line == 0);
    float2* my = S + line * RG::XCH;
    fill_twiddles<L>(tw, tid, T);
    const float r1 = a.rho1(g), r2 = a.rho2(g);
    const bool first = __builtin_amdgcn_readfirstlane(a.first) != 0, last = __builtin_amdgcn_readfirstlane(a.last) != 0;
    const float r2n = (POIS || last) ? 0.f : a.rho2n(g);
    bool tread = false;
    float r1n = 0.f;
    if constexpr (TWRITE) r1n = a.rho1n(g);
    else if constexpr (!POIS) tread = __builtin_amdgcn_readfirstlane(a.tail) == 2;
    const float r2w = tread ? 1.f : r2;
    const float al = POIS ? a.alpha(g) : 1.f;
    GD_TRACE(0);

    float2 X[RG::PPL][F2];
    {
        const float* z = a.a0 + (size_t)g * L * L;
#pragma unroll
        for (int q = 0; q < RG::PPL; ++q) {
            const float* r0 = z + (size_t)(2 * (opaque(line) + LINES * q)) * L + opaque(j);
#pragma unroll
            for (int r = 0; r < F2; ++r) X[q][r] = make_float2(ld_s(r0 + F1 * r), ld_s(r0 + L + F1 * r));
        }
    }
    stagger_start<GD_REG_STAGGER>(b, a.N);
    __syncthreads();
    GD_TRACE(1);
#pragma unroll
    for (int q = 0; q < RG::PPL; ++q) {
        reg_fft<L, false>(X[q], opaque(j), my, tw);
        pin(X[q]);
        __builtin_amdgcn_sched_barrier(0);
    }
    lds_barrier();
    GD_TRACE(2);

#pragma unroll
    for (int q = 0; q < RG::PPL; ++q) {
        const int p = opaque(line) + LINES * q, jq = opaque(j);
        float2* row = S + p * SLD;
#pragma unroll
        for (int r = 0; r < F2; ++r) {
            const int k = jq + F1 * r;
            if (r < KS / F1) row[k] = X[q][r];
            if (r == 0 && jq == 0) row[KS] = X[q][r];
            if (r == L / 2 / F1 && jq == 0) nyq[p] = X[q][r];
            if (r > (L - KS) / F1 || (r == (L - KS) / F1 && jq > 0)) row[KS + L - k] = X[q][r];
        }
        __builtin_amdgcn_sched_barrier(0);
    }
    lds_barrier();
    float2 CA[RG::CPL][F2];
#pragma unroll
    for (int u = 0; u < RG::CPL; ++u) fused_gather<L, SLD>(S, line + LINES * u, j, CA[u]);
#pragma unroll
    for (int s = 0; s < F2; ++s) {
        const int y = j + F1 * s;
        const float2 w = nyq[y >> 1];
        if (l0) CA[0][s].y = (y & 1) ? w.y : w.x;
    }
    lds_barrier();
    float2* park = S + RG::XA;
#pragma unroll
    for (int q = 0; q < RG::PPL; ++q)
#pragma unroll
        for (int r = RB0; r < RB0 + RG::PXB; ++r) park[(q * RG::PXB + r - RB0) * T + tid] = X[q][r];
    __builtin_amdgcn_sched_barrier(0);
    GD_TRACE(3);
    constexpr int DPT = POIS ? GD_POIS_DEPTH : GD_REG_DEPTH;
    constexpr bool SPF = GD_REG_SPF && (!POIS || GD_POIS_SPF);
    SGroup preA[DPT];
    if constexpr (SPF) fused_prefetch4x<L, RG::CPL, POIS, DPT>(a, preA, g, line, LINES, j, first, last, tread);
    if constexpr ((GD_REG_PAIR & 1) != 0 && (!POIS || GD_POIS_PAIR)) {
        reg_fft2<L, false>(CA[0], CA[1], opaque(j), my, tw);
        __builtin_amdgcn_sched_barrier(0);
    } else {
#pragma unroll
        for (int u = 0; u < RG::CPL; ++u) {
            reg_fft<L, false>(CA[u], opaque(j), my, tw);
            __builtin_amdgcn_sched_barrier(0);
        }
    }
    if (l0) {
#pragma unroll
        for (int s = 0; s < F2; ++s) nyqx[j + F1 * s] = CA[0][s];
        wave_lds_sync();
#pragma unroll
        for (int s = 0; s < F2; ++s) {
            const int ky = j + F1 * s;
            const float2 z = CA[0][s], zm = nyqx[(L - ky) & (L - 1)];
            nyqc[ky] = make_float2(0.5f * (z.y + zm.y), 0.5f * (zm.x - z.x));
            CA[0][s] = make_float2(0.5f * (z.x + zm.x), 0.5f * (z.y - zm.y));
        }
    }
    lds_barrier();
    if (__builtin_amdgcn_readfirstlane(tid >> 6) < L / 64) {
        nyqc[tid] = gauss_bin4<L, POIS>(a, g, tid, nyqc[tid], r1, r2, r2n, first, last, r2w, tread, TWRITE, r1n);
    }
    fused_update4x<L, RG::CPL, POIS, DPT, SPF, TWRITE>(a, CA, g, line, LINES, j, r1, r2, r2n, first, last, r2w, tread, r1n, &preA);
    lds_barrier();
    GD_TRACE(4);
#pragma unroll
    for (int s = 0; s < F2; ++s) {
        const float2 cn = nyqc[j + F1 * s];
        if (l0) CA[0][s] = make_float2(CA[0][s].x - cn.y, CA[0][s].y + cn.x);
    }
    if constexpr ((GD_REG_PAIR & 2) != 0 && (!POIS || GD_POIS_PAIR)) {
        reg_fft2<L, true>(CA[0], CA[1], opaque(j), my, tw);
        __builtin_amdgcn_sched_barrier(0);
    } else
#pragma unroll
    for (int u = 0; u < RG::CPL; ++u) {
        reg_fft<L, true>(CA[u], opaque(j), my, tw);
        if (POIS) pin(CA[u]);
        __builtin_amdgcn_sched_barrier(0);
    }
    if (l0) {
#pragma unroll
        for (int s = 0; s < F2; ++s) nyqo[j + F1 * s] = CA[0][s].y;
    }
#pragma unroll
    for (int q = 0; q < RG::PPL; ++q)
#pragma unroll
        for (int r = RB0; r < RB0 + RG::PXB; ++r) X[q][r] = park[(q * RG::PXB + r - RB0) * T + opaque(tid)];
    lds_barrier();
    GD_TRACE(5);

#pragma unroll
    for (int q = 0; q < RG::PPL; ++q) {
        const int jq = opaque(j);
        float2* row = S + (opaque(line) + LINES * q) * SLD;
#pragma unroll
        for (int r = RB0; r <= RB1; ++r) {
            const int k = jq + F1 * r;
            if (r < 2 * KS / F1) row[k - KS] = X[q][r];
            if (r > L / 2 / F1 || (r == L / 2 / F1 && jq > 0)) {
                if (r < RB1 || jq == 0) row[L - k] = X[q][r];
            }
        }
        __builtin_amdgcn_sched_barrier(0);
    }
    lds_barrier();
    float2 CB[RG::CPL][F2];
#pragma unroll
    for (int u = 0; u < RG::CPL; ++u) fused_gather<L, SLD>(S, line + LINES * u, j, CB[u]);
    lds_barrier();
#pragma unroll
    for (int s = 0; s < F2; ++s) park[s * T + tid] = CA[RG::CPL - 1][s];
    __builtin_amdgcn_sched_barrier(0);
    GD_TRACE(6);
    SGroup preB[DPT];
    if constexpr (SPF) fused_prefetch4x<L, RG::CPL, POIS, DPT>(a, preB, g, KS + line, LINES, j, first, last, tread);
    if constexpr ((GD_REG_PAIR & 1) != 0 && (!POIS || GD_POIS_PAIR)) {
        reg_fft2<L, false>(CB[0], CB[1], opaque(j), my, tw);
        __builtin_amdgcn_sched_barrier(0);
    } else {
#pragma unroll
        for (int u = 0; u < RG::CPL; ++u) {
            reg_fft<L, false>(CB[u], opaque(j), my, tw);
            __builtin_amdgcn_sched_barrier(0);
        }
    }
    fused_update4x<L, RG::CPL, POIS, DPT, SPF, TWRITE>(a, CB, g, KS + line, LINES, j, r1, r2, r2n, first, last, r2w, tread, r1n, &preB);
    if constexpr ((GD_REG_PAIR & 2) != 0 && (!POIS || GD_POIS_PAIR)) {
        reg_fft2<L, true>(CB[0], CB[1], opaque(j), my, tw);
        __builtin_amdgcn_sched_barrier(0);
    } else
#pragma unroll
    for (int u = 0; u < RG::CPL; ++u) {
        reg_fft<L, true>(CB[u], opaque(j), my, tw);
        if (POIS) pin(CB[u]);
        __builtin_amdgcn_sched_barrier(0);
    }
#pragma unroll
    for (int s = 0; s < F2; ++s) CA[RG::CPL - 1][s] = park[s * T + opaque(tid)];

    float* out = a.o0 + (size_t)g * L * L;
    static_for<0, 2>([&](auto hfc) {
        constexpr int hf = decltype(hfc)::value;
        lds_barrier();
        GD_TRACE(7 + hf);
#pragma unroll
        for (int s = hf * F2 / 2; s < (hf + 1) * F2 / 2; ++s) {
            float2* rr = S + (j + F1 * s - hf * L / 2) * SLD;
#pragma unroll
            for (int u = 0; u < RG::CPL; ++u) {
                const float2 c = CA[u][s];
                rr[line + LINES * u] = (u == 0 && l0) ? make_float2(c.x, 0.f) : c;
                rr[KS + line + LINES * u] = CB[u][s];
            }
        }
        for (int i = tid; i < L / 2; i += T) S[i * SLD + L / 2] = make_float2(nyqo[hf * L / 2 + i], 0.f);
        lds_barrier();
        float2 V[RG::HPL][F2];
#pragma unroll
        for (int w = 0; w < RG::HPL; ++w) {
            const int jj = opaque(j);
            const float2* re = S + (2 * (opaque(line) + LINES * w)) * SLD;
            const float2* ro = re + SLD;
#pragma unroll
            for (int r = 0; r < F2; ++r) {
                const int k = jj + F1 * r;
                float2 be, bo;
                if (k <= L / 2) {
                    be = re[k];
                    bo = ro[k];
                } else {
                    be = cconj(re[L - k]);
                    bo = cconj(ro[L - k]);
                }
                V[w][r] = make_float2(be.x - bo.y, be.y + bo.x);
            }
        }
        lds_barrier();
#pragma unroll
        for (int w = 0; w < RG::HPL; ++w) {
            reg_fft<L, true>(V[w], opaque(j), my, tw);
            float* o = out + (size_t)(hf * L / 2 + 2 * (opaque(line) + LINES * w)) * L + opaque(j);
            if constexpr (POIS) {
                if (last) {
#pragma unroll
                    for (int r = 0; r < F2; ++r) V[w][r] = make_float2(V[w][r].x * al, V[w][r].y * al);
                }
            }
#pragma unroll
            for (int r = 0; r < F2; ++r) {
                st_s(o + F1 * r, V[w][r].x);
                st_s(o + L + F1 * r, V[w][r].y);
            }
        }
    });
    drain_vm();
    __syncthreads();
    GD_TRACE(9);
}


template <int L, bool POIS = false>
__device__ __forceinline__ void init_update4(const Args& a, float2 (&C)[16], const float2 (&Hc)[16], int g, int kx,
                                             int j, float ial) {
    constexpr float inv_n = float(1.0 / double(L * L));
    j = opaque(j);
    kx = opaque(kx);
    __builtin_amdgcn_sched_barrier(0);
    const size_t gb = (size_t)g * (L / 2 + 1) * L;
    if constexpr (POIS) {
#pragma unroll
        for (int m = 0; m < 8; ++m)
            *reinterpret_cast<f4v*>(a.s_g + gb + soff_c(kx, m, j)) =
                f4v{Hc[2 * m].x, Hc[2 * m].y, Hc[2 * m + 1].x, Hc[2 * m + 1].y};
    }
#pragma unroll
    for (int q = 0; q < 4; ++q) {
        f4v h4, g4[2];
#pragma unroll
        for (int e = 0; e < 4; ++e) {
            const int s = 4 * q + e, h = e >> 1, c = 2 * (e & 1);
            const float2 Hk = Hc[s];
            const float hh = Hk.x * Hk.x + Hk.y * Hk.y;
            const float2 Gk = cmulc(C[s], Hk);
            h4[e] = hh;
            g4[h][c] = Gk.x;
            g4[h][c + 1] = Gk.y;
            const float rl = __builtin_amdgcn_rcpf(hh + ial);
            C[s] = cscale(make_float2(Gk.x * rl, Gk.y * rl), inv_n);
        }
        if constexpr (!POIS) {
            *reinterpret_cast<f4v*>(a.s_hh + gb + soff_h(kx, q, j)) = h4;
#pragma unroll
            for (int h = 0; h < 2; ++h) *reinterpret_cast<f4v*>(a.s_g + gb + soff_c(kx, 2 * q + h, j)) = g4[h];
        }
    }
}
template <int L, bool POIS = false>
__device__ __forceinline__ void w1_update4(const Args& a, const float2 (&C)[16], int g, int kx, int j) {
    j = opaque(j);
    kx = opaque(kx);
    __builtin_amdgcn_sched_barrier(0);
    const size_t gb = (size_t)g * (L / 2 + 1) * L;
#pragma unroll
    for (int m = 0; m < 8; ++m) {
        float2 c0 = C[2 * m], c1 = C[2 * m + 1];
        if constexpr (POIS) {
            const f4v h = ld4v(a.s_g + gb + soff_c(kx, m, j));
            c0 = cmul(make_float2(h[0], h[1]), c0);
            c1 = cmul(make_float2(h[2], h[3]), c1);
        }
        st4v(a.s_w + gb + soff_c(kx, m, j), f4v{c0.x, c0.y, c1.x, c1.y});
    }
}
#ifndef GD_INIT_HPF
#define GD_INIT_HPF 1
#endif
template <int L>
__device__ __forceinline__ void init_otf_column(const Args& a, float2 (&Hc)[16], int g, int kx, int j, bool l0,
                                                float2* my, const float2* tw, float2* nyqh,
                                                const float2 (*h4)[4] = nullptr) {
    if (h4)
        init_hcol<L>(Hc, *h4);
    else
        init_hload<L>(a, Hc, g, kx, j);
    reg_fft<L, false>(Hc, opaque(j), my, tw);
    if (l0) {
#pragma unroll
        for (int s = 0; s < 16; ++s) my[j + 16 * s] = Hc[s];
        wave_lds_sync();
        float2 zm[16];
#pragma unroll
        for (int s = 0; s < 16; ++s) zm[s] = my[(L - j - 16 * s) & (L - 1)];
        wave_lds_sync();
#pragma unroll
        for (int s = 0; s < 16; ++s) {
            const float2 z = Hc[s];
            nyqh[j + 16 * s] = make_float2(0.5f * (z.y + zm[s].y), 0.5f * (zm[s].x - z.x));
            Hc[s] = make_float2(0.5f * (z.x + zm[s].x), 0.5f * (z.y - zm[s].y));
        }
// ... 308 lines not shown
```

### galaxy-deconv_amd/gdeconv/_lib.py

```python
import ctypes
import os

import torch

LIB_PATH = os.path.join(os.path.dirname(os.path.abspath(__file__)), "libgdeconv.so")

GD_OK = 0
ABI_VERSION = 5
GD_LLH = {"Gaussian": 0, "Poisson": 1}

_P = ctypes.c_void_p
_I = ctypes.c_int
_LL = ctypes.c_longlong
_SZ = ctypes.c_size_t

SIGNATURES = {
    "gd_abi_version": (_I, []),
    "gd_engine_rev": (ctypes.c_char_p, []),
    "gd_engine_src_hash": (ctypes.c_char_p, []),
    "gd_hip_runtime_version": (_I, []),
    "gd_last_error": (ctypes.c_char_p, []),
    "gd_supported_size": (_I, [_I, _I]),
    "gd_workspace_bytes": (_SZ, [_I, _I, _I]),
    "gd_otf_bytes": (_SZ, [_I, _I, _I]),
    "gd_psf_to_otf": (_I, [_P, _LL, _I, _I, _I, _I, _I, _P, _P, _P]),
    "gd_conv_fft_batch": (_I, [_P, _I, _P, _P, _I, _I, _I, _P, _P]),
    "gd_conv_fft_batch_strided": (_I, [_P, _LL, _I, _P, _P, _I, _I, _I, _P, _P]),
    "gd_rfft2": (_I, [_P, _P, _I, _I, _I, _P]),
    "gd_irfft2": (_I, [_P, _P, _I, _I, _I, _P]),
    "gd_admm_state_bytes": (_SZ, [_I, _I, _I, _I]),
    "gd_admm_state_layout": (_I, [_I, _I, _I, _I]),
    "gd_admm_init_reads_rho": (_I, [_I, _I, _I]),
    "gd_admm_init": (_I, [_P, _P, _LL, _I, _I, _P, _LL, _P, _LL, _I, _I, _I, _I, _P, _P, _P, _P]),
    "gd_admm_iter": (_I, [_P, _P, _P, _P, _LL, _P, _LL, _P, _LL, _P, _LL, _I, _I, _I, _I, _I, _I, _P, _P,
                          _P]),
    "gd_admm_iter_v": (_I, [_P]),
    "gd_admm_iter_tail": (_I, [_P, _P, _P, _P, _LL, _P, _LL, _P, _LL, _P, _LL, _I, _I, _I, _I, _I, _I, _P, _P,
                               _P, _P, _LL, _I]),
    "gd_admm_iter_tail_v": (_I, [_P]),
    "gd_admm_tail_supported": (_I, [_I, _I, _I, _I]),
    "gd_set_combined_tail": (_I, [_I]),
    "gd_admm_train_saved_bytes": (_SZ, [_I, _I, _I]),
    "gd_admm_train_init": (_I, [_P, _P, _LL, _I, _I, _P, _LL, _I, _I, _I, _P, _P, _P, _P, _P]),
    "gd_admm_train_iter": (_I, [_P, _P, _P, _P, _P, _LL, _P, _LL, _P, _LL, _P, _LL, _I, _I, _I, _I, _I, _P, _P, _P,
                                _P, _P, _P, _P]),
    "gd_admm_train_iter_backward": (_I, [_P, _P, _P, _P, _P, _LL, _P, _LL, _P, _LL, _P, _LL, _I, _I, _I, _I, _I, _P,
                                         _P, _P, _P, _P, _P, _P, _P]),
    "gd_admm_train_full_saved_bytes": (_SZ, [_I, _I, _I]),
    "gd_admm_train_iter_full": (_I, [_P, _P, _P, _P, _P, _LL, _P, _LL, _P, _LL, _P, _LL, _I, _I, _I, _I, _I, _P, _P,
                                     _P, _P, _P, _P, _P]),
    "gd_admm_train_iter_full_backward": (_I, [_P, _P, _P, _P, _P, _LL, _P, _LL, _P, _LL, _P, _LL, _I, _I, _I, _I, _I,
                                              _P, _P, _P, _P, _P, _P, _P, _P, _P, _P, _P]),
    "gd_psf_to_otf_backward": (_I, [_P, _I, _I, _I, _I, _I, _P, _P, _P]),
    "gd_conv_fft_batch_backward_otf": (_I, [_P, _P, _I, _I, _I, _I, _P, _P, _P]),
    "gd_wiener": (_I, [_P, _P, _LL, _I, _I, _P, _LL, _P, _I, _I, _I, _P, _P]),
    "gd_richardson_lucy": (_I, [_P, _P, _LL, _I, _I, _I, _P, _I, _I, _I, _P, _P, _P]),
    "gd_tikhonov": (_I, [_P, _P, _LL, _I, _I, _P, _LL, _P, _LL, _P, _LL, _P, _I, _I, _I, _P, _P]),
    "gd_filter_power": (_I, [_P, _P, _I, _I, _I, _P, _P]),
    "gd_filter_power_taps": (_I, [_P, _P, _I, _P, _I, _I, _P]),
    "gd_gx_state_bytes": (_SZ, [_I, _I, _I]),
    "gd_gx_spec_bytes": (_SZ, [_I, _I, _I]),
    "gd_gx_init": (_I, [_P, _P, _LL, _I, _I, _P, _LL, _I, _I, _I, _P, _P, _P, _P]),
    "gd_gx_xupdate": (_I, [_P, _P, _P, _P, _LL, _P, _LL, _P, _P, _P, _I, _I, _I, _P, _P, _P]),
    "gd_gx_xupdate_backward": (_I, [_P, _P, _P, _LL, _P, _P, _P, _P, _I, _I, _I, _P, _P, _P]),
    "gd_set_chunk_bytes": (_SZ, [_SZ]),
    "gd_set_pipeline_streams": (_I, [_I]),
    "gd_set_capture_pipeline": (_I, [_I]),
    "gd_set_fused_iteration": (_I, [_I]),
    "gd_set_fused_rl": (_I, [_I]),
    "gd_set_subnet_fused_max": (_I, [_I]),
    "gd_set_fused_init": (_I, [_I]),
    "gd_set_fused_min_batch": (_I, [_I, _I]),
    "gd_subnet_param_count": (_I, []),
    "gd_subnet_features": (_I, [_P, _P, _P, _I, _P]),
    "gd_subnet_mlp_param_count": (_I, [_I]),
    "gd_subnet_rhos": (_I, [_P, _P, _P, _P, _LL, _P, _P, _I, _I, _P]),
    "gd_subnet_rhos_psf": (_I, [_P, _LL, _I, _P, _P, _P, _LL, _P, _P, _I, _I, _P]),
    "gd_admm_init_subnet_supported": (_I, [_I, _I, _I, _I, _I, _I, _I]),
    "gd_admm_init_subnet": (_I, [_P, _P, _LL, _I, _I, _P, _LL, _I, _I, _I, _I, _P, _P, _P, _P, _P, _I, _P, _P]),
    "gd_profile_enable": (_I, [_I]),
    "gd_profile_collect": (_I, []),
    "gd_profile_get": (_I, [_I, ctypes.c_char_p, _I, ctypes.POINTER(ctypes.c_double), ctypes.POINTER(_LL)]),
    "gd_profile_reset": (_I, []),
    "gd_pack_open": (_I, [ctypes.c_char_p, ctypes.POINTER(_P), ctypes.POINTER(_LL), ctypes.POINTER(_I)]),
    "gd_pack_section_bytes": (_LL, [_P, _I]),
    "gd_pack_read": (_I, [_P, _I, _LL, _LL, _P, _I]),
    "gd_pack_gather": (_I, [_P, _I, _P, _LL, _P, _I]),
    "gd_pack_close": (_I, [_P]),
}

_lib = None

ROOT = os.path.dirname(os.path.dirname(os.path.dirname(os.path.abspath(__file__))))


def source_files():
    import glob
    csrc = os.path.join(ROOT, "galaxy-deconv_amd", "csrc")
    return [os.path.join(csrc, "gd_engine.hip"), *sorted(glob.glob(os.path.join(csrc, "*.hpp"))),
            os.path.join(ROOT, "include", "gdeconv.h")]


BUILD_FLAGS = ["--offload-arch=gfx950", "-O3", "-std=c++17", "-fPIC", "-shared", "-Wno-unused-result"]


def _toolchain_id():
    try:
        with open("/opt/rocm/.info/version") as f:
            return f.read().strip()
    except OSError:
        return "unknown"


def source_hash():
    import hashlib
    h = hashlib.sha256()
    for p in source_files():
        h.update(os.path.basename(p).encode() + b"\0")
        with open(p, "rb") as f:
            h.update(f.read())
        h.update(b"\0")
    h.update(("flags:" + " ".join(BUILD_FLAGS) + "\0rocm:" + _toolchain_id()).encode())
    return h.hexdigest()[:16]


class EngineError(RuntimeError):
    pass


def load(path=LIB_PATH):
    global _lib
    if _lib is not None:
        return _lib
    if not os.path.exists(path):
        raise EngineError(f"HIP engine library not found at {path}: build it with "
                          "`python -c 'import __graft_entry__ as g; g.build()'` (no CPU fallback)")
    lib = ctypes.CDLL(path)
    for name, (res, args) in SIGNATURES.items():
        fn = getattr(lib, name)
        fn.restype = res
        fn.argtypes = args
    if lib.gd_abi_version() != ABI_VERSION:
        raise EngineError("libgdeconv.so ABI version mismatch")
    _lib = lib
    return lib


def profile_enable(level=2):
    load().gd_profile_enable(int(level))


def profile_reset():
    load().gd_profile_reset()


def profile_collect():
    lib = load()
    n = lib.gd_profile_collect()
    if n < 0:
        check(n, "gd_profile_collect")
    out = {}
    buf = ctypes.create_string_buffer(128)
    for i in range(n):
        ms, cnt = ctypes.c_double(), _LL()
        check(lib.gd_profile_get(i, buf, 128, ctypes.byref(ms), ctypes.byref(cnt)), "gd_profile_get")
        out[buf.value.decode()] = (ms.value, cnt.value)
    return out


def check(rc, what):
    if rc != GD_OK:
        msg = load().gd_last_error()
        raise EngineError(f"{what} failed ({rc}): {msg.decode() if msg else ''}")


__all__ = ["load", "check", "EngineError", "SIGNATURES", "LIB_PATH", "GD_LLH", "source_hash", "source_files"]
```

### galaxy-deconv_amd/gdeconv/engine.py

```python
import contextlib
import ctypes

import torch

from . import _lib


_raw_stream = getattr(torch._C, "_cuda_getCurrentRawStream", None)
_cur_device = getattr(torch._C, "_cuda_getDevice", None)


def _stream(device=None):
    if _raw_stream is not None and device is not None and device.index is not None:
        return _raw_stream(device.index)
    return torch.cuda.current_stream(device).cuda_stream


def _current_device():
    return _cur_device() if _cur_device is not None else torch.cuda.current_device()


def _require_device(*ts):
    dev = None
    for t in ts:
# ... 394 lines not shown
    def init(self):
        return self.z0

    def _init(self):
        z0 = torch.empty_like(self.y)
        k = self.psf
        _lib.check(self.lib.gd_gx_init(self.y.data_ptr(), k.data_ptr(), self.psf_gs, k.shape[2], k.shape[3],
                                       self.alpha.data_ptr(), self.alpha_s, self.N, self.H, self.W,
                                       self.state.data_ptr(), z0.data_ptr(), self._ws().data_ptr(),
                                       _stream(self.dev)), "gd_gx_init")
        return z0

    def rho(self, rho):
        return _galaxy_scalar(rho.detach() if torch.is_tensor(rho) else rho, self.N, "rho", self.dev)

    def x_update(self, z, u, rho, x_prev=None, rho_prev=None, zin=False, save=False):
        _require_device(z, u, x_prev, self.y)
        z = _img(z, "z")
        r, rs = self.rho(rho)
        if x_prev is not None:
            if u is None or rho_prev is None:
                raise ValueError("the fused dual update needs u and rho_prev")
            if not u.is_contiguous() or u.dtype != torch.float32:
                raise ValueError("u is updated in place: it must be contiguous fp32")
            x_prev = _img(x_prev, "x_prev")
        elif u is not None:
            u = _img(u, "u")
        rp, rps = self.rho(rho_prev) if rho_prev is not None else (None, 0)
        x = torch.empty_like(self.y)
        zi = torch.empty_like(self.y) if zin else None
        xs = torch.empty(self.spec_bytes, dtype=torch.uint8, device=self.y.device) if save else None
        ptr = lambda t: None if t is None else t.data_ptr()
        with _on(self.dev):
            _lib.check(self.lib.gd_gx_xupdate(z.data_ptr(), ptr(u), ptr(x_prev), r.data_ptr(), rs, ptr(rp), rps,
                                              x.data_ptr(), ptr(zi), ptr(xs), self.N, self.H, self.W,
                                              self.state.data_ptr(), self._ws().data_ptr(), _stream(self.dev)),
                       "gd_gx_xupdate")
        return x, zi, xs

    def x_backward(self, grad_x, z, rho, xs):
        g = _img(grad_x, "grad_x")
        z = _img(z, "z")
        r, rs = self.rho(rho)
        gz, gu = torch.empty_like(self.y), torch.empty_like(self.y)
        part = torch.empty(self.N, self.W + 1, dtype=torch.float32, device=self.y.device)
        with _on(self.dev):
            _lib.check(self.lib.gd_gx_xupdate_backward(g.data_ptr(), z.data_ptr(), r.data_ptr(), rs, xs.data_ptr(),
                                                       gz.data_ptr(), gu.data_ptr(), part.data_ptr(), self.N, self.H,
                                                       self.W, self.state.data_ptr(), self._ws().data_ptr(),
                                                       _stream(self.dev)), "gd_gx_xupdate_backward")
        return gz, gu, part.sum(1)


class _XUpdateGaussianFn(torch.autograd.Function):

    @staticmethod
    def forward(ctx, z, u, rho, st):
        x, _, xs = st.x_update(z.detach(), u.detach(), rho, save=True)
        ctx.st, ctx.xs = st, xs
        ctx.rho_shape = rho.shape if torch.is_tensor(rho) else None
        ctx.save_for_backward(z.detach().float().contiguous(), rho if torch.is_tensor(rho) else torch.tensor(rho))
        return x

    @staticmethod
    def backward(ctx, gx):
        z, rho = ctx.saved_tensors
        st = ctx.st
        gz, gu, grho = st.x_backward(gx.contiguous(), z, rho, ctx.xs)
        gr = None
        if ctx.needs_input_grad[2]:
            gr = (grho.sum() if rho.numel() == 1 else grho).reshape(ctx.rho_shape).to(rho.dtype)
        return (gz if ctx.needs_input_grad[0] else None, gu if ctx.needs_input_grad[1] else None, gr, None)


def gx_x_update(st, z, u, rho):
    return _XUpdateGaussianFn.apply(z, u, rho, st)


class RhoSchedule:

    __slots__ = ("t", "base", "gs", "n")

    def __init__(self, rho_iters, N, device):
        t = rho_iters.detach()
        if t.dtype != torch.float32:
            t = t.float()
        if t.device != torch.device(device):
            raise ValueError(f"rho schedule is on {t.device}, the inputs on {device}")
        if t.dim() == 4:
            t = t.reshape(t.shape[0], t.shape[-1]) if t.shape[1] == 1 and t.shape[2] == 1 else None
            if t is None:
                raise ValueError("rho schedule must be [N,1,1,n]")
            if t.stride(1) != 1:
                t = t.contiguous()
            if t.shape[0] not in (1, N):
                raise ValueError(f"rho schedule batch must be 1 or N={N}")
            self.gs = t.stride(0) if (t.shape[0] == N and N > 1) else 0
            self.n = t.shape[1]
        elif t.dim() == 1:
            t = t.contiguous()
            self.gs, self.n = 0, t.shape[0]
        else:
            raise ValueError("rho schedule must be [N,1,1,n] or [n]")
        self.t, self.base = t, t.data_ptr()

    def __getitem__(self, it):
        if not 0 <= it < self.n:
            raise IndexError(f"iteration {it} outside the schedule of {self.n}")
        return self.base + 4 * it, self.gs


def _scalar_arg(x, dev):
    p, s = x
    if torch.is_tensor(p):
        if p.device != dev:
            raise ValueError(f"per-galaxy scalar on {p.device}, the inputs on {dev}")
        if p.dtype != torch.float32:
            raise ValueError("per-galaxy scalars must be fp32")
        return p.data_ptr(), s
    return int(p), s


_NESTED_FORK_SAFE = None


def _nested_capture_fork_safe(lib):
    global _NESTED_FORK_SAFE
    if _NESTED_FORK_SAFE is None:
        _NESTED_FORK_SAFE = lib.gd_hip_runtime_version() >= 70200000
    return _NESTED_FORK_SAFE


class ADMMState:

    def __init__(self, y, psf, alpha, llh):
        self.dev = _require_device(y, psf, alpha)
        self.lib = _lib.load()
        self.y = _img(y, "y")
        self.N, _, self.H, self.W = self.y.shape
        self.psf, self.psf_gs = _psf(psf, self.N, self.H)
        if llh not in _lib.GD_LLH:
            raise ValueError("llh must be 'Gaussian' or 'Poisson'")
        self.llh = _lib.GD_LLH[llh]
        skey = (self.N, self.H, self.W, self.llh)
        nbytes = ADMMState._state_bytes.get(skey)
        if nbytes is None:
            if not self.lib.gd_supported_size(self.H, self.W):
                raise ValueError(f"unsupported image size {self.H}x{self.W} (H and W must be in [2, 4096])")
            nbytes = ADMMState._state_bytes[skey] = int(self.lib.gd_admm_state_bytes(max(self.N, 1), self.H, self.W,
                                                                                      self.llh))
        with _on(self.dev):
            self.alpha, self.alpha_s = _galaxy_scalar(alpha, self.N, "alpha", self.dev)
            self.state = torch.empty(nbytes, dtype=torch.uint8, device=self.dev)
            self.zin = torch.empty_like(self.y)
            self.ws = workspace(self.N, self.H, self.W, self.dev)
        self._fixed = (self.y.data_ptr(), self.alpha.data_ptr(), self.alpha_s, self.state.data_ptr(),
                       self.ws.data_ptr())
        self._dev_index = self.dev.index if self.dev.index is not None else torch.cuda.current_device()
        self._shape = tuple(self.y.shape)
        self._bind()
        self.layout = None
        self.iter = 0
        self._tail = False
        self._side = None
        r = ADMMState._reads_rho.get((self.H, self.W, self.llh))
        if r is None:
            r = int(self.lib.gd_admm_init_reads_rho(self.H, self.W, self.llh))
        self.init_reads_rho = r > 0

    _reads_rho = {}
    _state_bytes = {}
    _side_streams = {}
    _SIDE_STREAMS_MAX = 16

    @property
    def otf(self):
        if self.llh != _lib.GD_LLH["Poisson"]:
            raise AttributeError("the Gaussian ADMM state stores |H|^2, not the OTF")
        K = self.W // 2 + 1
        return self.state[: self.N * K * self.H * 8].view(torch.complex64).view(self.N, K, self.H)

    def init(self, rho2_first):
        if rho2_first is None:
            if self.init_reads_rho:
                raise ValueError("this init takes the first V step: it needs rho2_first")
            r2, r2s = None, 0
        else:
            r2, r2s = _scalar_arg(rho2_first, self.dev)
        k = self.psf
        yp, ap, as_, sp, wp = self._fixed
        with _on(self.dev):
            _lib.check(self.lib.gd_admm_init(
                yp, k.data_ptr(), self.psf_gs, k.shape[2], k.shape[3], ap, as_, r2, r2s, self.llh, self.N, self.H,
                self.W, sp, self.zin.data_ptr(), wp, _stream(self.dev)), "gd_admm_init")
        self.layout = self.lib.gd_admm_state_layout(self.N, self.H, self.W, self.llh)
        self.iter = 0
        self._tail = False

    def init_with_subnet(self, params, mlp_params, n_out):
        if self.init_reads_rho:
            return None
        k = self.psf
        if not self.lib.gd_admm_init_subnet_supported(self.N, self.H, self.W, k.shape[2], k.shape[3], self.llh,
                                                      int(n_out)):
            return None
        if params.numel() != _subnet_param_count() or params.dtype != torch.float32 or params.device != self.dev:
            raise ValueError("bad SubNet parameter pack")
        if mlp_params.numel() != _mlp_param_count(int(n_out)) or mlp_params.dtype != torch.float32 \
                or mlp_params.device != self.dev:
            raise ValueError("bad SubNet MLP parameter pack")
        yp, ap, as_, sp, wp = self._fixed
        with _on(self.dev):
            rhos = torch.empty(self.N, int(n_out), dtype=torch.float32, device=self.dev)
            _lib.check(self.lib.gd_admm_init_subnet(
                yp, k.data_ptr(), self.psf_gs, k.shape[2], k.shape[3], ap, as_, self.llh, self.N, self.H, self.W, sp,
                self.zin.data_ptr(), params.contiguous().data_ptr(), mlp_params.contiguous().data_ptr(),
                rhos.data_ptr(), int(n_out), wp, _stream(self.dev)), "gd_admm_init_subnet")
        self.layout = self.lib.gd_admm_state_layout(self.N, self.H, self.W, self.llh)
        self.iter = 0
        self._tail = False
        return rhos

    def init_concurrent(self):
        if self.init_reads_rho:
            raise ValueError("this init takes the first V step: it needs the rhos (use init(rho2_first))")
        main = torch.cuda.current_stream(self.dev)
        key = (self._dev_index, main.cuda_stream)
        entry = ADMMState._side_streams.pop(key, None)
        if entry is None:
            entry = (torch.cuda.Stream(device=self.dev), torch.cuda.Event(), torch.cuda.Event())
        ADMMState._side_streams[key] = entry
        while len(ADMMState._side_streams) > ADMMState._SIDE_STREAMS_MAX:
            ADMMState._side_streams.pop(next(iter(ADMMState._side_streams)))
        side, fork, _ = entry
        fork.record(main)
        side.wait_event(fork)
        serial = torch.cuda.is_current_stream_capturing() and not _nested_capture_fork_safe(self.lib)
        old = self.lib.gd_set_capture_pipeline(0) if serial else None
        try:
            with torch.cuda.stream(side):
                self.init(None)
        finally:
            if serial:
                self.lib.gd_set_capture_pipeline(old)
        self._side = entry

    def join(self):
        if self._side is not None:
            side, _, ev = self._side
            ev.record(side)
            torch.cuda.current_stream(self.dev).wait_event(ev)
            self._side = None

    def _bind(self):
        yp, ap, as_, sp, wp = self._fixed
        v = self._argv = (ctypes.c_longlong * 23)()
        v[0], v[3], v[4], v[11] = yp, ap, as_, self.llh
        v[14], v[15], v[16], v[17], v[18] = self.N, self.H, self.W, sp, wp
        self._argv_addr = ctypes.addressof(v)
        self._iter_v = self.lib.gd_admm_iter_tail_v

    def step(self, z, rho1, rho2, rho2_next, out=None, *, rho1_next=None):
        if self.layout is None:
            raise _lib.EngineError("ADMMState.step before init")
        if self._side is not None:
            self.join()
        if z.dtype != torch.float32 or not z.is_contiguous():
            z = z.float().contiguous()
        if z.shape != self._shape:
            raise ValueError(f"denoiser returned {tuple(z.shape)}, expected {self._shape}")
        if z.device != self.dev:
            raise ValueError(f"denoiser returned a tensor on {z.device}, the state is on {self.dev}")
        last = rho2_next is None
        if last:
            if out is None or out.shape != self._shape or out.dtype != torch.float32 or out.device != self.dev \
                    or not out.is_contiguous():
                raise ValueError("the last iteration needs a contiguous fp32 `out` shaped like y on the state's device")
            dst = out
        else:
            dst = self.zin
        if self.llh != 0 and self.lib.gd_admm_state_layout(self.N, self.H, self.W, self.llh) != self.layout:
            raise _lib.EngineError("the ADMM state layout changed since init (gd_set_fused_iteration toggled "
                                   "between gd_admm_init and gd_admm_iter)")
        v = self._argv
        tail = 0
        if self._tail:
            if not last:
                raise _lib.EngineError("the previous step was a tail-write (rho1_next given): the state holds the "
                                       "last iteration's combined term only, the next step must be the last")
            tail = 2
        elif rho1_next is not None and not last and self.llh == 0 and self.H == 256 and self.W == 256 \
                and self.lib.gd_admm_tail_supported(self.N, self.H, self.W, self.llh) == 1:
            tail = 1
        if tail == 1:
            v[20], v[21] = _scalar_arg(rho1_next, self.dev)
        else:
            v[20], v[21] = 0, 0
        v[22] = tail
        v[5], v[6] = _scalar_arg(rho1, self.dev)
        v[7], v[8] = _scalar_arg(rho2, self.dev)
        if last:
            v[9], v[10] = 0, 0
        else:
            v[9], v[10] = _scalar_arg(rho2_next, self.dev)
        v[1], v[2], v[12], v[13] = z.data_ptr(), dst.data_ptr(), self.iter, last
        if _current_device() == self._dev_index:
            v[19] = _stream(self.dev) or 0
            rc = self._iter_v(self._argv_addr)
        else:
            with _on(self.dev):
                v[19] = _stream(self.dev) or 0
                rc = self._iter_v(self._argv_addr)
        if rc:
            _lib.check(rc, "gd_admm_iter")
        self._tail = tail == 1
        self.iter += 1
        return dst


class ADMMTrainState:

    def __init__(self, y, psf, alpha, llh, input_grads=False):
        self.input_grads = bool(input_grads)
        self.dev = _require_device(y, psf, alpha)
        self.lib = _lib.load()
        self.y = _img(y.detach(), "y")
        self.N, _, self.H, self.W = self.y.shape
        self.psf, self.psf_gs = _psf(psf.detach(), self.N, self.H)
        if llh not in _lib.GD_LLH:
            raise ValueError("llh must be 'Gaussian' or 'Poisson'")
        self.llh_name, self.llh = llh, _lib.GD_LLH[llh]
        if not self.lib.gd_supported_size(self.H, self.W):
            raise ValueError(f"unsupported image size {self.H}x{self.W} (H and W must be in [2, 4096])")
        self.saved_bytes = int(self.lib.gd_admm_train_saved_bytes(max(self.N, 1), self.H, self.W))
        self.K = self.W // 2 + 1
        k = self.psf
        if self.input_grads:
            self._init_input_grads(y, psf, alpha)
            return
        with _on(self.dev):
            self.alpha, self.alpha_s = _galaxy_scalar(alpha.detach() if torch.is_tensor(alpha) else alpha, self.N,
                                                      "alpha", self.dev)
            self.otf = empty_otf(self.N, self.H, self.W, self.dev)
            self.x0, self.hx0 = torch.empty_like(self.y), torch.empty_like(self.y)
            _lib.check(self.lib.gd_admm_train_init(
                self.y.data_ptr(), k.data_ptr(), self.psf_gs, k.shape[2], k.shape[3], self.alpha.data_ptr(),
                self.alpha_s, self.N, self.H, self.W, self.otf.data_ptr(), self.x0.data_ptr(), self.hx0.data_ptr(),
                workspace(self.N, self.H, self.W, self.dev).data_ptr(), _stream(self.dev)), "gd_admm_train_init")

    def _init_input_grads(self, y, psf, alpha):
        self.full_saved_bytes = int(self.lib.gd_admm_train_full_saved_bytes(max(self.N, 1), self.H, self.W))
        with _on(self.dev):
            self.alpha, self.alpha_s = _galaxy_scalar(alpha.detach() if torch.is_tensor(alpha) else alpha, self.N,
                                                      "alpha", self.dev)
        self.y_in = y
        self.alpha_in = alpha if torch.is_tensor(alpha) else self.alpha
        self.otf_in = psf_to_otf_half(psf, self.N, self.H, self.W)
        self.otf = self.otf_in.detach()
        y4 = y.float()
        self.yp_in = torch.where(y4 > 0, y4, torch.zeros_like(y4))
        self.alpha4_in = self.alpha_in.float().reshape(-1, 1, 1, 1)
        zero = torch.zeros_like(self.y)
        x0raw = _ADMMTrainIterFullFn.apply(zero, zero, self.yp_in, 1.0, 1.0 / self.alpha4_in, None, None, None,
                                           self.otf_in, self, True, _lib.GD_LLH["Gaussian"])
        self.x0 = x0raw.clamp(0.0, 1.0)
        self.hx0 = conv_half(self.otf_in, self.x0)

    def alpha4(self):
        if self.input_grads:
            return self.alpha4_in
        return self.alpha.view(-1, 1, 1, 1)

    def w0(self, rho2_first):
        yp, al = (self.yp_in if self.input_grads else self.y.clamp_min(0.0)), self.alpha4()
        if self.llh_name == "Poisson":
            t1 = rho2_first * self.hx0 - al
            return 0.5 * (1 / rho2_first) * (-t1 + torch.sqrt(t1 ** 2 + 4 * yp * rho2_first))
        return (rho2_first * self.hx0 + yp / al) / (1 + rho2_first)

    def rho(self, t):
        if torch.is_tensor(t):
            t = t.detach()
            if t.device != self.dev:
                raise ValueError(f"rho is on {t.device}, the inputs on {self.dev}")
            if t.dtype == torch.float32 and t.dim() == 4 and t.shape[0] == self.N and t.numel() == self.N and self.N > 1:
                return t, t.data_ptr(), t.stride(0)
        t, s = _galaxy_scalar(t, self.N, "rho", self.dev)
        return t, t.data_ptr(), s


class _ADMMTrainIterFn(torch.autograd.Function):

    @staticmethod
    def forward(ctx, z, u1, w, rho1, rho2, rho2_next, st, last):
        N, H, W, dev = st.N, st.H, st.W, st.dev
        shape = tuple(st.y.shape)
        ins = []
        for t, name in ((z, "z"), (u1, "u1"), (w, "w")):
            t = _img(t.detach(), name)
            if tuple(t.shape) != shape or t.device != dev:
                raise ValueError(f"{name} must be {shape} on {dev}, got {tuple(t.shape)} on {t.device}")
            ins.append(t)
        r1 = st.rho(rho1)
        r2 = st.rho(rho2)
        r2n = st.rho(rho2_next) if not last else (None, None, 0)
        with _on(dev):
            zin = torch.empty_like(st.y)
            u1o = None if last else torch.empty_like(st.y)
            wo = None if last else torch.empty_like(st.y)
            saved = torch.empty(st.saved_bytes, dtype=torch.uint8, device=dev)
            _lib.check(st.lib.gd_admm_train_iter(
                st.y.data_ptr(), ins[0].data_ptr(), ins[1].data_ptr(), ins[2].data_ptr(), st.alpha.data_ptr(),
                st.alpha_s, r1[1], r1[2], r2[1], r2[2], r2n[1], r2n[2], st.llh, int(last), N, H, W,
# ... 120 lines not shown
```

### include/gdeconv.h

```cpp
#ifndef GDECONV_H
#define GDECONV_H

#include <stddef.h>

#ifdef __cplusplus
extern "C" {
#endif

#define GD_ABI_VERSION 5

#define GD_OK 0
#define GD_ERR_ARG (-1)
#define GD_ERR_UNSUPPORTED (-2)
#define GD_ERR_HIP (-3)

#define GD_LLH_GAUSSIAN 0
#define GD_LLH_POISSON 1

int gd_abi_version(void);
const char* gd_engine_rev(void);
const char* gd_engine_src_hash(void);
int gd_hip_runtime_version(void);
const char* gd_last_error(void);
int gd_supported_size(int H, int W);
size_t gd_workspace_bytes(int N, int H, int W);
size_t gd_otf_bytes(int N, int H, int W);

int gd_psf_to_otf(const float* psf, long long psf_gstride, int h, int w, int N, int H, int W,
                  void* otf_half, void* ws, void* stream);

int gd_conv_fft_batch(const void* otf_half, int conj, const float* x, float* out, int N, int H, int W,
                      void* ws, void* stream);
int gd_conv_fft_batch_strided(const void* otf_half, long long otf_gstride, int conj, const float* x, float* out,
                              int N, int H, int W, void* ws, void* stream);

int gd_rfft2(const float* x, void* spec, int N, int H, int W, void* stream);
int gd_irfft2(void* spec, float* x, int N, int H, int W, void* stream);

size_t gd_admm_state_bytes(int N, int H, int W, int llh);
int gd_admm_state_layout(int N, int H, int W, int llh);
int gd_admm_init_reads_rho(int H, int W, int llh);
int gd_admm_init(const float* y, const float* psf, long long psf_gstride, int h, int w,
                 const float* alpha, long long alpha_stride, const float* rho2, long long rho2_stride,
                 int llh, int N, int H, int W, void* state, float* zin, void* ws, void* stream);
int gd_admm_iter(const float* y, const float* z, float* zin_or_out, const float* alpha, long long alpha_stride,
                 const float* rho1, long long rho1_stride, const float* rho2, long long rho2_stride,
                 const float* rho2_next, long long rho2_next_stride, int llh, int iter, int last, int N, int H,
                 int W, void* state, void* ws, void* stream);
int gd_admm_iter_v(const long long* argv);

int gd_admm_iter_tail(const float* y, const float* z, float* zin_or_out, const float* alpha, long long alpha_stride,
                      const float* rho1, long long rho1_stride, const float* rho2, long long rho2_stride,
                      const float* rho2_next, long long rho2_next_stride, int llh, int iter, int last, int N, int H,
                      int W, void* state, void* ws, void* stream, const float* rho1_next, long long rho1_next_stride,
                      int tail);
int gd_admm_iter_tail_v(const long long* argv);
int gd_admm_tail_supported(int N, int H, int W, int llh);

size_t gd_admm_train_saved_bytes(int N, int H, int W);
int gd_admm_train_init(const float* y, const float* psf, long long psf_gstride, int h, int w, const float* alpha,
                       long long alpha_stride, int N, int H, int W, void* otf_half, float* x0, float* hx0, void* ws,
                       void* stream);
int gd_admm_train_iter(const float* y, const float* z, const float* u1, const float* w, const float* alpha,
                       long long alpha_stride, const float* rho1, long long rho1_stride, const float* rho2,
                       long long rho2_stride, const float* rho2_next, long long rho2_next_stride, int llh, int last,
                       int N, int H, int W, const void* otf_half, float* zin_or_out, float* u1_out, float* w_out,
                       void* saved, void* ws, void* stream);
int gd_admm_train_iter_backward(const float* g_zin_or_out, const float* g_u1_out, const float* g_w_out, const float* y,
                                const float* alpha, long long alpha_stride, const float* rho1, long long rho1_stride,
                                const float* rho2, long long rho2_stride, const float* rho2_next,
                                long long rho2_next_stride, int llh, int last, int N, int H, int W, const void* otf_half,
                                const void* saved, float* g_z, float* g_u1, float* g_w, float* g_rho_part, void* ws,
                                void* stream);

size_t gd_admm_train_full_saved_bytes(int N, int H, int W);
int gd_admm_train_iter_full(const float* y, const float* z, const float* u1, const float* w, const float* alpha,
                            long long alpha_stride, const float* rho1, long long rho1_stride, const float* rho2,
                            long long rho2_stride, const float* rho2_next, long long rho2_next_stride, int llh, int last,
                            int N, int H, int W, const void* otf_half, float* zin_or_out, float* u1_out, float* w_out,
                            void* saved, void* ws, void* stream);
int gd_admm_train_iter_full_backward(const float* g_zin_or_out, const float* g_u1_out, const float* g_w_out,
                                     const float* y, const float* alpha, long long alpha_stride, const float* rho1,
                                     long long rho1_stride, const float* rho2, long long rho2_stride,
                                     const float* rho2_next, long long rho2_next_stride, int llh, int last, int N, int H,
                                     int W, const void* otf_half, const void* saved, float* g_z, float* g_u1, float* g_w,
                                     float* g_rho_part, void* g_otf_half, float* g_y, float* g_alpha_part, void* ws,
                                     void* stream);

int gd_psf_to_otf_backward(const void* g_otf_half, int h, int w, int N, int H, int W, float* g_psf, void* ws,
                           void* stream);
int gd_conv_fft_batch_backward_otf(const float* x, const float* g_out, int conj, int N, int H, int W, void* g_otf_half,
                                   void* ws, void* stream);

int gd_wiener(const float* y, const float* psf, long long psf_gstride, int h, int w, const float* alpha,
              long long alpha_stride, float* x, int N, int H, int W, void* ws, void* stream);

int gd_richardson_lucy(const float* y, const float* psf, long long psf_gstride, int h, int w, int n_iters,
                       float* x, int N, int H, int W, void* otf_half, void* ws, void* stream);

int gd_tikhonov(const float* y, const float* psf, long long psf_gstride, int h, int w, const float* alpha,
                long long alpha_stride, const float* lam, long long lam_stride, const float* ltl,
                long long ltl_gstride, float* x, int N, int H, int W, void* ws, void* stream);

int gd_filter_power(const float* filt, float* power_half, int N, int H, int W, void* ws, void* stream);

int gd_filter_power_taps(const int* rc, const float* vals, int ntaps, float* power_half, int H, int W,
                         void* stream);

size_t gd_gx_state_bytes(int N, int H, int W);
size_t gd_gx_spec_bytes(int N, int H, int W);
int gd_gx_init(const float* y, const float* psf, long long psf_gstride, int h, int w, const float* alpha,
               long long alpha_stride, int N, int H, int W, void* state, float* z0, void* ws, void* stream);
int gd_gx_xupdate(const float* z, float* u, const float* x_prev, const float* rho, long long rho_stride,
                  const float* rho_prev, long long rho_prev_stride, float* x, float* zin, void* xspec,
                  int N, int H, int W, void* state, void* ws, void* stream);
int gd_gx_xupdate_backward(const float* grad_x, const float* z, const float* rho, long long rho_stride,
                           const void* xspec, float* grad_z, float* grad_u, float* grad_rho_part, int N, int H,
                           int W, void* state, void* ws, void* stream);

int gd_subnet_param_count(void);
int gd_subnet_features(const void* otf128_half, const float* params, float* feat, int N, void* stream);

int gd_subnet_mlp_param_count(int n_out);
int gd_subnet_rhos(const void* otf128_half, const float* params, const float* mlp_params, const float* alpha,
                   long long alpha_stride, float* feat, float* rhos, int n_out, int N, void* stream);

int gd_subnet_rhos_psf(const float* psf, long long psf_gstride, int h, const float* params, const float* mlp_params,
                       const float* alpha, long long alpha_stride, float* feat, float* rhos, int n_out, int N,
                       void* stream);

int gd_admm_init_subnet_supported(int N, int H, int W, int h, int w, int llh, int n_out);
int gd_admm_init_subnet(const float* y, const float* psf, long long psf_gstride, int h, int w, const float* alpha,
                        long long alpha_stride, int llh, int N, int H, int W, void* state, float* zin,
                        const float* params, const float* mlp_params, float* rhos, int n_out, void* ws, void* stream);

size_t gd_set_chunk_bytes(size_t bytes);
int gd_set_pipeline_streams(int streams);

int gd_set_capture_pipeline(int mode);

int gd_set_fused_iteration(int on);

int gd_set_combined_tail(int on);

int gd_set_fused_rl(int on);

int gd_set_subnet_fused_max(int n);

int gd_set_fused_min_batch(int op, int n);

int gd_set_fused_init(int on);

int gd_profile_enable(int level);
int gd_profile_collect(void);
int gd_profile_get(int i, char* name, int name_len, double* total_ms, long long* launches);
int gd_profile_reset(void);

#define GD_PACK_OBS 0
#define GD_PACK_PSF 1
#define GD_PACK_GT 2
#define GD_PACK_ALPHA 3
#define GD_PACK_INFO 4

int gd_pack_open(const char* path, void** handle, long long* n, int* dims);
long long gd_pack_section_bytes(void* handle, int section);
int gd_pack_read(void* handle, int section, long long g0, long long count, void* dst, int nthreads);
int gd_pack_gather(void* handle, int section, const long long* idx, long long count, void* dst, int nthreads);
int gd_pack_close(void* handle);

#ifdef __cplusplus
}
#endif

#endif
```

Measured before the change: 337,900 galaxies/s.

## Regenerate OTF |H|^2 in-kernel from compact PSF row spectra instead of loading

Adds a compact per-galaxy buffer holding the row-FFT of the small PSF (h rows × K columns) and, in non-last Gaussian ADMM iterations, has the fused k_gal_reg kernel recompute |H|^2 from a sparse column FFT of those rows instead of reading the full s_hh spectrum from state. This trades HBM reads of the full |H|^2 array for extra in-register FFT work and LDS staging. Enabled by default for 256x256 with an even PSF side of at most 64, and switchable off via GD_ROWS_HH. It adds an extra psf_rows_state launch at init.

```diff
diff --git a/galaxy-deconv_amd/csrc/gd_engine.hip b/galaxy-deconv_amd/csrc/gd_engine.hip
--- a/galaxy-deconv_amd/csrc/gd_engine.hip
+++ b/galaxy-deconv_amd/csrc/gd_engine.hip
@@ -58,6 +58,7 @@
     float* o3;
     float* part;
     float* apart;
+    float2* rows;
 };
 
 enum RowFwdMode { RF_ITER, RF_PSF_Y, RF_PSF_YP, RF_PSF_RAW, RF_PSF, RF_ONE, RF_TWO, RF_YA, RF_PSF_YAR,
@@ -414,6 +415,11 @@
     split_store<L, R>(a, lds, g, row0, tid);
 }
 
+template <int L>
+__device__ __forceinline__ float2* psf_rows_of(const Args& a, int g) {
+    constexpr int K = L / 2 + 1;
+    return a.rows ? a.rows + (size_t)g * K * a.h : a.s_u1 + (size_t)g * K * L;
+}
 template <int L, bool TO_STATE = false>
 __global__ __launch_bounds__(256) void k_psf_rows(Args a) {
     using G = Geo<L>;
@@ -441,7 +447,7 @@
 #pragma unroll
     for (int s = 0; s < F2; ++s) lds[line * G::RLD + j + F1 * s] = v[s];
     __syncthreads();
-    float2* P = TO_STATE ? a.s_u1 + (size_t)g * K * L : a.T + tidx(g, 1, 0, 0, K, L);
+    float2* P = TO_STATE ? psf_rows_of<L>(a, g) : a.T + tidx(g, 1, 0, 0, K, L);
     for (int idx = tid; idx < LPB * K; idx += 256) {
         const int m = idx % LPB, k = idx / LPB;
         if (p0 + m >= pairs) continue;
@@ -892,7 +898,7 @@
     using FG = FusedGeo<L>;
     static_assert((L & (L - 1)) == 0, "power-of-two side");
     const int h = a.h, c0p = h >> 1;
-    const float2* P0 = a.s_u1 + (size_t)g * FG::K * L + (size_t)opaque(kx) * h;
+    const float2* P0 = psf_rows_of<L>(a, g) + (size_t)opaque(kx) * h;
     j = opaque(j);
     static_assert(FG::F1 == 16 && FG::F2 == 16, "sparse OTF column for 16 x 16 lines");
 #pragma unroll
@@ -908,7 +914,7 @@
 __device__ __forceinline__ void init_hload4(const Args& a, float2 (&h4)[4], int g, int kx, int j) {
     using FG = FusedGeo<L>;
     const int h = a.h, c0p = h >> 1;
-    const float2* P0 = a.s_u1 + (size_t)g * FG::K * L + (size_t)opaque(kx) * h;
+    const float2* P0 = psf_rows_of<L>(a, g) + (size_t)opaque(kx) * h;
     j = opaque(j);
 #pragma unroll
     for (int t = 0; t < 4; ++t) {
@@ -2231,7 +2237,12 @@
     }
     static int gal_reg(const Args& a, hipStream_t st) {
         ProfScope ps(nm(kGalRegName, a.first + 2 * a.last), st);
-        if (a.tail == 1)
+        if (a.rows != nullptr && !a.last) {
+            if (a.tail == 1)
+                hipLaunchKernelGGL((k_gal_reg<L, false, true, true>), dim3(a.N), dim3(RegGeo<L>::THREADS), 0, st, a);
+            else
+                hipLaunchKernelGGL((k_gal_reg<L, false, false, true>), dim3(a.N), dim3(RegGeo<L>::THREADS), 0, st, a);
+        } else if (a.tail == 1)
             hipLaunchKernelGGL((k_gal_reg<L, false, true>), dim3(a.N), dim3(RegGeo<L>::THREADS), 0, st, a);
         else
             hipLaunchKernelGGL((k_gal_reg<L>), dim3(a.N), dim3(RegGeo<L>::THREADS), 0, st, a);
@@ -2287,6 +2298,10 @@
 int g_fused_min_n = 96;
 int g_combined_tail = [] {
     const char* e = std::getenv("GD_COMBINED_TAIL");
+    return (e && e[0] == '0' && e[1] == '\0') ? 0 : 1;
+}();
+int g_rows_hh = [] {
+    const char* e = std::getenv("GD_ROWS_HH");
     return (e && e[0] == '0' && e[1] == '\0') ? 0 : 1;
 }();
 int g_pois2_min_n = 192;
@@ -2567,7 +2582,7 @@
                 return Lc::gal_reg_init(a0, st0);
             }
         }
-        return for_chunks(a0, L, st0, [&](const Args& a, hipStream_t st) {
+        GD_TRY(for_chunks(a0, L, st0, [&](const Args& a, hipStream_t st) {
             Args b = a;
             GD_TRY(Lc::template rf<RF_YA>(b, st));
             GD_TRY(Lc::psf_rows(b, st));
@@ -2576,12 +2591,20 @@
             b.t_slot = 1;
             GD_TRY(Lc::template rif<RIF_CLAMP>(b, st));
             return Lc::template col<C_G_W1>(b, st);
-        });
+        }));
+        if constexpr (has_fused<L>()) {
+            if (a0.rows != nullptr) return Lc::psf_rows_state(a0, st0);
+        }
+        return GD_OK;
     }
     static int admm_iter_gauss(Args a, hipStream_t st0) {
         if constexpr (has_fused<L>()) {
-            if (g_fused && a.N >= g_fused_min_n) return Lc::gal_reg(a, st0);
-        }
+            if (g_fused && a.N >= g_fused_min_n) {
+                if (!(g_rows_hh && a.h <= 64 && !a.last)) a.rows = nullptr;
+                return Lc::gal_reg(a, st0);
+            }
+        }
+        a.rows = nullptr;
         if constexpr (GD_MID_EXTRA && (L == 96 || L == 128)) {
             if (g_fused) return gal_mid_launch_t<L>(a, st0);
         }
@@ -2815,7 +2838,7 @@
 
 int gd_abi_version(void) { return GD_ABI_VERSION; }
 
-const char* gd_engine_rev(void) { return "r09.0"; }
+const char* gd_engine_rev(void) { return "r10.0"; }
 
 #ifndef GD_SRC_HASH
 #define GD_SRC_HASH "unknown"
@@ -2980,11 +3003,32 @@
     return pois_split(H, W) ? 0 : 1;
 }
 
+size_t gd_admm_rows_bytes(int N, int H, int W, int h) {
+    if (H != 256 || W != 256 || !has_fused<256>() || N <= 0 || h < 2 || h > 64 || (h & 1)) return 0;
+    return (size_t)N * h * (W / 2 + 1) * sizeof(float2);
+}
+
+int gd_admm_rows_supported(int N, int H, int W, int h, int llh) {
+    return llh == GD_LLH_GAUSSIAN && gd_admm_rows_bytes(N, H, W, h) != 0 && g_fused != 0 && N >= g_fused_min_n &&
+                   g_rows_hh != 0
+               ? 1
+               : 0;
+}
+
 int gd_admm_init(const float* y, const float* psf, long long psf_gstride, int h, int w,
                  const float* alpha, long long alpha_stride, const float* rho2, long long rho2_stride,
                  int llh, int N, int H, int W, void* state, float* zin, void* ws, void* stream) {
+    return gd_admm_init_rows(y, psf, psf_gstride, h, w, alpha, alpha_stride, rho2, rho2_stride, llh, N, H, W, state, zin, ws,
+                             stream, nullptr);
+}
+
+int gd_admm_init_rows(const float* y, const float* psf, long long psf_gstride, int h, int w,
+                      const float* alpha, long long alpha_stride, const float* rho2, long long rho2_stride,
+                      int llh, int N, int H, int W, void* state, float* zin, void* ws, void* stream, void* rows) {
     GD_TRY(check_shape(N, H, W));
     GD_TRY(check_psf(h, w, H, W));
+    if (rows != nullptr && (llh != GD_LLH_GAUSSIAN || gd_admm_rows_bytes(N > 0 ? N : 1, H, W, h) == 0))
+        return fail(GD_ERR_UNSUPPORTED, "a rows buffer where gd_admm_rows_bytes is 0 (256 x 256 Gaussian, even PSF side <= 64)");
     if (llh != GD_LLH_GAUSSIAN && llh != GD_LLH_POISSON) return fail(GD_ERR_ARG, "llh must be Gaussian or Poisson");
     if (llh == GD_LLH_POISSON && rho2 == nullptr && !pois_split(H, W))
         return fail(GD_ERR_ARG, "the Poisson init takes the first V step: it needs rho2");
@@ -2996,6 +3040,7 @@
     a.llh = llh;
     bind_state(a, state, N, H, W, llh);
     a.o2 = zin;
+    a.rows = reinterpret_cast<float2*>(rows);
     ProfScope ps("op_admm_init<" + std::to_string(H) + "," + std::to_string(llh) + ">", (hipStream_t)stream, 1);
     if (llh == GD_LLH_GAUSSIAN)
         return dispatch<Ops>(H, W, [&](auto op) { return decltype(op)::admm_init_gauss(a, (hipStream_t)stream); });
@@ -3015,7 +3060,19 @@
                       const float* rho2_next, long long rho2_next_stride, int llh, int iter, int last, int N, int H,
                       int W, void* state, void* ws, void* stream, const float* rho1_next, long long rho1_next_stride,
                       int tail) {
+    return gd_admm_iter_rows(y, z, zin_or_out, alpha, alpha_stride, rho1, rho1_stride, rho2, rho2_stride, rho2_next,
+                             rho2_next_stride, llh, iter, last, N, H, W, state, ws, stream, rho1_next, rho1_next_stride,
+                             tail, nullptr, 0);
+}
+
+int gd_admm_iter_rows(const float* y, const float* z, float* zin_or_out, const float* alpha, long long alpha_stride,
+                      const float* rho1, long long rho1_stride, const float* rho2, long long rho2_stride,
+                      const float* rho2_next, long long rho2_next_stride, int llh, int iter, int last, int N, int H,
+                      int W, void* state, void* ws, void* stream, const float* rho1_next, long long rho1_next_stride,
+                      int tail, const void* rows, int h) {
     GD_TRY(check_shape(N, H, W));
+    if (rows != nullptr && (llh != GD_LLH_GAUSSIAN || gd_admm_rows_bytes(N > 0 ? N : 1, H, W, h) == 0))
+        return fail(GD_ERR_UNSUPPORTED, "a rows buffer where gd_admm_rows_bytes is 0 (256 x 256 Gaussian, even PSF side <= 64)");
     if (llh != GD_LLH_GAUSSIAN && llh != GD_LLH_POISSON) return fail(GD_ERR_ARG, "llh must be Gaussian or Poisson");
     if (tail < 0 || tail > 2) return fail(GD_ERR_ARG, "tail must be 0, 1 (tail-write) or 2 (tail-read)");
     if (tail == 1 && last) return fail(GD_ERR_ARG, "tail = 1 (the next call is the last) with last set");
@@ -3038,6 +3095,8 @@
     a.llh = llh;
     a.last = last;
     a.first = iter == 0;
+    a.rows = reinterpret_cast<float2*>(const_cast<void*>(rows));
+    a.h = rows ? h : 0;
     a.rev = GD_REG_REV ? (llh == GD_LLH_POISSON ? 1 : (iter % 2 == 0)) : 0;
     ProfScope ps("op_admm_iter<" + std::to_string(H) + "," + std::to_string(llh) + ">", (hipStream_t)stream, 1);
     if (llh == GD_LLH_GAUSSIAN) {
@@ -3071,6 +3130,16 @@
                              static_cast<const float*>(p(7)), v[8], static_cast<const float*>(p(9)), v[10], (int)v[11],
                              (int)v[12], (int)v[13], (int)v[14], (int)v[15], (int)v[16], p(17), p(18), p(19),
                              static_cast<const float*>(p(20)), v[21], (int)v[22]);
+}
+
+int gd_admm_iter_rows_v(const long long* v) {
+    if (v == nullptr) return fail(GD_ERR_ARG, "gd_admm_iter_rows_v: null argument vector");
+    const auto p = [v](int i) { return reinterpret_cast<void*>(static_cast<intptr_t>(v[i])); };
+    return gd_admm_iter_rows(static_cast<const float*>(p(0)), static_cast<const float*>(p(1)), static_cast<float*>(p(2)),
+                             static_cast<const float*>(p(3)), v[4], static_cast<const float*>(p(5)), v[6],
+                             static_cast<const float*>(p(7)), v[8], static_cast<const float*>(p(9)), v[10], (int)v[11],
+                             (int)v[12], (int)v[13], (int)v[14], (int)v[15], (int)v[16], p(17), p(18), p(19),
+                             static_cast<const float*>(p(20)), v[21], (int)v[22], p(23), (int)v[24]);
 }
 
 int gd_admm_iter_v(const long long* v) {
@@ -3499,6 +3568,13 @@
     if (on != 0 && on != 1) return fail(GD_ERR_ARG, "gd_set_combined_tail: 0 or 1");
     const int old = g_combined_tail;
     g_combined_tail = on;
+    return old;
+}
+
+int gd_set_rows_hh(int on) {
+    if (on != 0 && on != 1) return fail(GD_ERR_ARG, "gd_set_rows_hh: 0 or 1");
+    const int old = g_rows_hh;
+    g_rows_hh = on;
     return old;
 }
 
diff --git a/galaxy-deconv_amd/csrc/gd_galreg.hpp b/galaxy-deconv_amd/csrc/gd_galreg.hpp
--- a/galaxy-deconv_amd/csrc/gd_galreg.hpp
+++ b/galaxy-deconv_amd/csrc/gd_galreg.hpp
@@ -34,7 +34,8 @@
 
 template <int L, bool POIS = false>
 __device__ __forceinline__ float2 gauss_bin4(const Args& a, int g, int ky, float2 Zk, float r1, float r2, float r2n,
-                                             bool first, bool last, float r2w, bool tread, bool twrite, float r1n) {
+                                             bool first, bool last, float r2w, bool tread, bool twrite, float r1n,
+                                             const float* nyqhh = nullptr) {
     constexpr float inv_n = float(1.0 / double(L * L));
     const size_t cb = ((size_t)g * (L / 2 + 1) + L / 2) * L;
     const int pc = sidx_c<L>(ky);
@@ -48,7 +49,7 @@
         }
         return r;
     }
-    const float hh = a.s_hh[cb + sidx_h<L>(ky)];
+    const float hh = nyqhh ? nyqhh[ky] : a.s_hh[cb + sidx_h<L>(ky)];
     const float2 Gk = (last && !first) ? make_float2(0.f, 0.f) : a.s_g[cb + pc];
     const float2 U1 = (first || tread) ? make_float2(0.f, 0.f) : a.s_u1[cb + pc];
     float2 Wt = a.s_w[cb + pc];
@@ -73,10 +74,10 @@
 struct SGroup {
     f4v h, g[2], u[2], w[2];
 };
-template <int L, bool POIS = false>
+template <int L, bool POIS = false, bool REGEN = false>
 __device__ __forceinline__ void sgroup_load(const Args& a, SGroup& G, size_t gb, int kx, int q, int j, bool first,
                                             bool last, bool tread) {
-    G.h = POIS ? f4v{0.f, 0.f, 0.f, 0.f} : ld4s(a.s_hh + gb + soff_h(kx, q, j));
+    G.h = (POIS || REGEN) ? f4v{0.f, 0.f, 0.f, 0.f} : ld4s(a.s_hh + gb + soff_h(kx, q, j));
 #pragma unroll
     for (int h = 0; h < 2; ++h) {
         const size_t off = gb + soff_c(kx, 2 * q + h, j);
@@ -97,21 +98,22 @@
 #ifndef GD_REG_SPF
 #define GD_REG_SPF 1
 #endif
-template <int L, int NC, bool POIS = false, int D = GD_REG_DEPTH>
+template <int L, int NC, bool POIS = false, int D = GD_REG_DEPTH, bool REGEN = false>
 __device__ __forceinline__ void fused_prefetch4x(const Args& a, SGroup (&P)[D], int g, int kx0, int kstep, int j, bool first,
                                                  bool last, bool tread) {
     j = opaque(j);
     kx0 = opaque(kx0);
     const size_t gb = (size_t)g * (L / 2 + 1) * L;
 #pragma unroll
-    for (int t = 0; t < D && t < 4 * NC; ++t) sgroup_load<L, POIS>(a, P[t], gb, kx0 + kstep * (t / 4), t % 4, j, first, last, tread);
+    for (int t = 0; t < D && t < 4 * NC; ++t)
+        sgroup_load<L, POIS, REGEN>(a, P[t], gb, kx0 + kstep * (t / 4), t % 4, j, first, last, tread);
     __builtin_amdgcn_sched_barrier(0);
 }
-template <int L, int NC, bool POIS = false, int D = GD_REG_DEPTH, bool PRE = false, bool TWRITE = false>
+template <int L, int NC, bool POIS = false, int D = GD_REG_DEPTH, bool PRE = false, bool TWRITE = false, bool REGEN = false>
 __device__ __forceinline__ void fused_update4x(const Args& a, float2 (&C)[NC][16], int g, int kx0, int kstep, int j,
                                                float r1, float r2, float r2n, bool first, bool last, float r2w, bool tread,
                                                float r1n,
-                                               const SGroup (*pre)[D] = nullptr) {
+                                               const SGroup (*pre)[D] = nullptr, const float* hs = nullptr) {
     constexpr float inv_n = float(1.0 / double(L * L));
     constexpr int NG = 4 * NC;
     j = opaque(j);
@@ -122,13 +124,15 @@
 #pragma unroll
     for (int t = 0; t < D && t < NG; ++t) {
         if constexpr (PRE) G[t] = (*pre)[t];
-        else sgroup_load<L, POIS>(a, G[t], gb, kx0 + kstep * (t / 4), t % 4, j, first, last, tread);
+        else sgroup_load<L, POIS, REGEN>(a, G[t], gb, kx0 + kstep * (t / 4), t % 4, j, first, last, tread);
     }
     __builtin_amdgcn_sched_barrier(0);
 #pragma unroll
     for (int t = 0; t < NG; ++t) {
         const int u = t / 4, q = t % 4;
         f4v uo[2], wo[2];
+        f4v hq = G[t].h;
+        if constexpr (REGEN) hq = *reinterpret_cast<const f4v*>(hs + 64 * t + 4 * j);
 #pragma unroll
         for (int e = 0; e < 4; ++e) {
             const int h = e >> 1, c = 2 * (e & 1);
@@ -139,8 +143,8 @@
                 C[u][4 * q + e] = pois_math(Gk, make_float2(G[t].u[h][c], G[t].u[h][c + 1]), Wt, C[u][4 * q + e],
                                             r1, r2, inv_n, U1n, Wn, last);
             } else {
-                if (first) Wt = w1_value(G[t].h[e], Gk, Wt, r2);
-                C[u][4 * q + e] = gauss_math_rt(G[t].h[e], Gk, make_float2(G[t].u[h][c], G[t].u[h][c + 1]), Wt,
+                if (first) Wt = w1_value(hq[e], Gk, Wt, r2);
+                C[u][4 * q + e] = gauss_math_rt(hq[e], Gk, make_float2(G[t].u[h][c], G[t].u[h][c + 1]), Wt,
                                                 C[u][4 * q + e], r1, r2, r2w, r2n, inv_n, U1n, Wn, last);
                 if constexpr (TWRITE) Wn = gauss_tail_c(U1n, Wn, r1n, r2n);
             }
@@ -155,7 +159,7 @@
                 st4v((POIS ? a.s_x : a.s_w) + off, wo[h]);
             }
         }
-        if (t + D < NG) sgroup_load<L, POIS>(a, G[t + D], gb, kx0 + kstep * ((t + D) / 4), (t + D) % 4, j, first, last, tread);
+        if (t + D < NG) sgroup_load<L, POIS, REGEN>(a, G[t + D], gb, kx0 + kstep * ((t + D) / 4), (t + D) % 4, j, first, last, tread);
         __builtin_amdgcn_sched_barrier(0);
     }
 }
@@ -170,6 +174,42 @@
 template <int L, bool INV>
 __device__ __forceinline__ void reg_fft2(float2 (&v0)[16], float2 (&v1)[16], int j, float2* xch, const float2* tw) {
     line_fft2<L, INV, GD_REG_LEAN != 0>(v0, v1, j, xch, tw);
+}
+
+template <int L>
+__device__ __forceinline__ void regen_hh(float (&hh)[16], const float2 (&hp)[4], int j, bool l0, float2* my,
+                                         const float2* tw, float* nyqhh) {
+    float2 Hc[16];
+    init_hcol<L>(Hc, hp);
+    reg_fft<L, false>(Hc, opaque(j), my, tw);
+    if (l0) {
+#pragma unroll
+        for (int s = 0; s < 16; ++s) my[j + 16 * s] = Hc[s];
+        wave_lds_sync();
+#pragma unroll
+        for (int s = 0; s < 16; ++s) {
+            const float2 z = Hc[s], zm = my[(L - j - 16 * s) & (L - 1)];
+            const float2 n = make_float2(0.5f * (z.y + zm.y), 0.5f * (zm.x - z.x));
+            nyqhh[j + 16 * s] = n.x * n.x + n.y * n.y;
+            Hc[s] = make_float2(0.5f * (z.x + zm.x), 0.5f * (z.y - zm.y));
+        }
+        wave_lds_sync();
+    }
+#pragma unroll
+    for (int s = 0; s < 16; ++s) hh[s] = Hc[s].x * Hc[s].x + Hc[s].y * Hc[s].y;
+    __builtin_amdgcn_sched_barrier(0);
+}
+
+template <int L>
+__device__ __forceinline__ void regen_stage(const float (&hh)[2][16], int j, float2* my) {
+    wave_lds_sync();
+    float* hs = reinterpret_cast<float*>(my);
+#pragma unroll
+    for (int t = 0; t < 8; ++t)
+        *reinterpret_cast<f4v*>(hs + 64 * t + 4 * opaque(j)) =
+            f4v{hh[t / 4][4 * (t % 4)], hh[t / 4][4 * (t % 4) + 1], hh[t / 4][4 * (t % 4) + 2], hh[t / 4][4 * (t % 4) + 3]};
+    wave_lds_sync();
+    __builtin_amdgcn_sched_barrier(0);
 }
 
 template <int L>
@@ -215,9 +255,10 @@
     }
 }
 
-template <int L, bool POIS = false, bool TWRITE = false>
+template <int L, bool POIS = false, bool TWRITE = false, bool REGEN = false>
 __global__ __launch_bounds__(512) void k_gal_reg(Args a) {
     static_assert(!POIS || !TWRITE, "the combined tail is Gaussian only");
+    static_assert(!POIS || !REGEN, "|H|^2 from the PSF rows is Gaussian only");
     using RG = RegGeo<L>;
     constexpr int F1 = RG::F1, F2 = RG::F2, KS = RG::KS, SLD = RG::SLD, LINES = RG::LINES, T = RG::THREADS;
     constexpr int RB0 = RG::RB0, RB1 = RG::RB1;
@@ -228,18 +269,20 @@
     __shared__ float2 nyqc[L];
     __shared__ float2 nyqx[L];
     __shared__ float nyqo[L];
+    __shared__ float nyqhh[REGEN ? L : 1];
     const int tid = threadIdx.x, line = tid / F1, j = tid - line * F1;
     const int b = blockIdx.x, g = a.rev ? a.N - 1 - b : b;
     const bool l0 = (line == 0);
     float2* my = S + line * RG::XCH;
     fill_twiddles<L>(tw, tid, T);
     const float r1 = a.rho1(g), r2 = a.rho2(g);
-    const bool first = __builtin_amdgcn_readfirstlane(a.first) != 0, last = __builtin_amdgcn_readfirstlane(a.last) != 0;
+    const bool first = __builtin_amdgcn_readfirstlane(a.first) != 0;
+    const bool last = REGEN ? false : __builtin_amdgcn_readfirstlane(a.last) != 0;
     const float r2n = (POIS || last) ? 0.f : a.rho2n(g);
     bool tread = false;
     float r1n = 0.f;
     if constexpr (TWRITE) r1n = a.rho1n(g);
-    else if constexpr (!POIS) tread = __builtin_amdgcn_readfirstlane(a.tail) == 2;
+    else if constexpr (!POIS && !REGEN) tread = __builtin_amdgcn_readfirstlane(a.tail) == 2;
     const float r2w = tread ? 1.f : r2;
     const float al = POIS ? a.alpha(g) : 1.f;
     GD_TRACE(0);
@@ -261,6 +304,12 @@
     for (int q = 0; q < RG::PPL; ++q) {
         reg_fft<L, false>(X[q], opaque(j), my, tw);
         pin(X[q]);
+        __builtin_amdgcn_sched_barrier(0);
+    }
+    float2 hpA[RG::CPL][4];
+    if constexpr (REGEN) {
+#pragma unroll
+        for (int u = 0; u < RG::CPL; ++u) init_hload4<L>(a, hpA[u], g, line + LINES * u, j);
         __builtin_amdgcn_sched_barrier(0);
     }
     lds_barrier();
@@ -300,8 +349,9 @@
     GD_TRACE(3);
     constexpr int DPT = POIS ? GD_POIS_DEPTH : GD_REG_DEPTH;
     constexpr bool SPF = GD_REG_SPF && (!POIS || GD_POIS_SPF);
+    constexpr bool SPFR = SPF && !REGEN;
     SGroup preA[DPT];
-    if constexpr (SPF) fused_prefetch4x<L, RG::CPL, POIS, DPT>(a, preA, g, line, LINES, j, first, last, tread);
+    if constexpr (SPFR) fused_prefetch4x<L, RG::CPL, POIS, DPT>(a, preA, g, line, LINES, j, first, last, tread);
     if constexpr ((GD_REG_PAIR & 1) != 0 && (!POIS || GD_POIS_PAIR)) {
         reg_fft2<L, false>(CA[0], CA[1], opaque(j), my, tw);
         __builtin_amdgcn_sched_barrier(0);
@@ -324,11 +374,22 @@
             CA[0][s] = make_float2(0.5f * (z.x + zm.x), 0.5f * (z.y - zm.y));
         }
     }
+    float hh[RG::CPL][F2];
+    const float* hs = reinterpret_cast<const float*>(my);
+    if constexpr (REGEN) {
+#pragma unroll
+        for (int u = 0; u < RG::CPL; ++u) regen_hh<L>(hh[u], hpA[u], j, l0 && u == 0, my, tw, nyqhh);
+        regen_stage<L>(hh, j, my);
+        fused_prefetch4x<L, RG::CPL, false, DPT, true>(a, preA, g, line, LINES, j, first, last, tread);
+    }
     lds_barrier();
     if (__builtin_amdgcn_readfirstlane(tid >> 6) < L / 64) {
-        nyqc[tid] = gauss_bin4<L, POIS>(a, g, tid, nyqc[tid], r1, r2, r2n, first, last, r2w, tread, TWRITE, r1n);
-    }
-    fused_update4x<L, RG::CPL, POIS, DPT, SPF, TWRITE>(a, CA, g, line, LINES, j, r1, r2, r2n, first, last, r2w, tread, r1n, &preA);
+        nyqc[tid] = gauss_bin4<L, POIS>(a, g, tid, nyqc[tid], r1, r2, r2n, first, last, r2w, tread, TWRITE, r1n,
+                                        REGEN ? nyqhh : nullptr);
+    }
+    fused_update4x<L, RG::CPL, POIS, DPT, SPF, TWRITE, REGEN>(a, CA, g, line, LINES, j, r1, r2, r2n, first, last, r2w, tread,
+                                                              r1n, &preA, hs);
+    if constexpr (REGEN) wave_lds_sync();
     lds_barrier();
     GD_TRACE(4);
 #pragma unroll
@@ -357,6 +418,12 @@
     lds_barrier();
     GD_TRACE(5);
 
+    float2 hpB[RG::CPL][4];
+    if constexpr (REGEN) {
+#pragma unroll
+        for (int u = 0; u < RG::CPL; ++u) init_hload4<L>(a, hpB[u], g, KS + line + LINES * u, j);
+        __builtin_amdgcn_sched_barrier(0);
+    }
 #pragma unroll
     for (int q = 0; q < RG::PPL; ++q) {
         const int jq = opaque(j);
@@ -381,7 +448,7 @@
     __builtin_amdgcn_sched_barrier(0);
     GD_TRACE(6);
     SGroup preB[DPT];
-    if constexpr (SPF) fused_prefetch4x<L, RG::CPL, POIS, DPT>(a, preB, g, KS + line, LINES, j, first, last, tread);
+    if constexpr (SPFR) fused_prefetch4x<L, RG::CPL, POIS, DPT>(a, preB, g, KS + line, LINES, j, first, last, tread);
     if constexpr ((GD_REG_PAIR & 1) != 0 && (!POIS || GD_POIS_PAIR)) {
         reg_fft2<L, false>(CB[0], CB[1], opaque(j), my, tw);
         __builtin_amdgcn_sched_barrier(0);
@@ -392,7 +459,15 @@
             __builtin_amdgcn_sched_barrier(0);
         }
     }
-    fused_update4x<L, RG::CPL, POIS, DPT, SPF, TWRITE>(a, CB, g, KS + line, LINES, j, r1, r2, r2n, first, last, r2w, tread, r1n, &preB);
+    if constexpr (REGEN) {
+#pragma unroll
+        for (int u = 0; u < RG::CPL; ++u) regen_hh<L>(hh[u], hpB[u], j, false, my, tw, nyqhh);
+        regen_stage<L>(hh, j, my);
+        fused_prefetch4x<L, RG::CPL, false, DPT, true>(a, preB, g, KS + line, LINES, j, first, last, tread);
+    }
+    fused_update4x<L, RG::CPL, POIS, DPT, SPF, TWRITE, REGEN>(a, CB, g, KS + line, LINES, j, r1, r2, r2n, first, last, r2w, tread,
+                                                              r1n, &preB, hs);
+    if constexpr (REGEN) wave_lds_sync();
     if constexpr ((GD_REG_PAIR & 2) != 0 && (!POIS || GD_POIS_PAIR)) {
         reg_fft2<L, true>(CB[0], CB[1], opaque(j), my, tw);
         __builtin_amdgcn_sched_barrier(0);
diff --git a/galaxy-deconv_amd/gdeconv/_lib.py b/galaxy-deconv_amd/gdeconv/_lib.py
--- a/galaxy-deconv_amd/gdeconv/_lib.py
+++ b/galaxy-deconv_amd/gdeconv/_lib.py
@@ -40,6 +40,13 @@
     "gd_admm_iter_tail_v": (_I, [_P]),
     "gd_admm_tail_supported": (_I, [_I, _I, _I, _I]),
     "gd_set_combined_tail": (_I, [_I]),
+    "gd_admm_rows_bytes": (_SZ, [_I, _I, _I, _I]),
+    "gd_admm_init_rows": (_I, [_P, _P, _LL, _I, _I, _P, _LL, _P, _LL, _I, _I, _I, _I, _P, _P, _P, _P, _P]),
+    "gd_admm_iter_rows": (_I, [_P, _P, _P, _P, _LL, _P, _LL, _P, _LL, _P, _LL, _I, _I, _I, _I, _I, _I, _P, _P,
+                               _P, _P, _LL, _I, _P, _I]),
+    "gd_admm_iter_rows_v": (_I, [_P]),
+    "gd_admm_rows_supported": (_I, [_I, _I, _I, _I, _I]),
+    "gd_set_rows_hh": (_I, [_I]),
     "gd_admm_train_saved_bytes": (_SZ, [_I, _I, _I]),
     "gd_admm_train_init": (_I, [_P, _P, _LL, _I, _I, _P, _LL, _I, _I, _I, _P, _P, _P, _P, _P]),
     "gd_admm_train_iter": (_I, [_P, _P, _P, _P, _P, _LL, _P, _LL, _P, _LL, _P, _LL, _I, _I, _I, _I, _I, _P, _P, _P,
diff --git a/galaxy-deconv_amd/gdeconv/engine.py b/galaxy-deconv_amd/gdeconv/engine.py
--- a/galaxy-deconv_amd/gdeconv/engine.py
+++ b/galaxy-deconv_amd/gdeconv/engine.py
@@ -570,6 +570,12 @@
         with _on(self.dev):
             self.alpha, self.alpha_s = _galaxy_scalar(alpha, self.N, "alpha", self.dev)
             self.state = torch.empty(nbytes, dtype=torch.uint8, device=self.dev)
+            self.rows = None
+            hk = int(self.psf.shape[2])
+            if self.llh == 0 and self.psf.shape[3] == hk and \
+                    self.lib.gd_admm_rows_supported(self.N, self.H, self.W, hk, self.llh) == 1:
+                self.rows = torch.empty(int(self.lib.gd_admm_rows_bytes(self.N, self.H, self.W, hk)), dtype=torch.uint8,
+                                        device=self.dev)
             self.zin = torch.empty_like(self.y)
             self.ws = workspace(self.N, self.H, self.W, self.dev)
         self._fixed = (self.y.data_ptr(), self.alpha.data_ptr(), self.alpha_s, self.state.data_ptr(),
@@ -608,9 +614,10 @@
         k = self.psf
         yp, ap, as_, sp, wp = self._fixed
         with _on(self.dev):
-            _lib.check(self.lib.gd_admm_init(
+            _lib.check(self.lib.gd_admm_init_rows(
                 yp, k.data_ptr(), self.psf_gs, k.shape[2], k.shape[3], ap, as_, r2, r2s, self.llh, self.N, self.H,
-                self.W, sp, self.zin.data_ptr(), wp, _stream(self.dev)), "gd_admm_init")
+                self.W, sp, self.zin.data_ptr(), wp, _stream(self.dev),
+                self.rows.data_ptr() if self.rows is not None else None), "gd_admm_init")
         self.layout = self.lib.gd_admm_state_layout(self.N, self.H, self.W, self.llh)
         self.iter = 0
         self._tail = False
@@ -672,11 +679,13 @@
 
     def _bind(self):
         yp, ap, as_, sp, wp = self._fixed
-        v = self._argv = (ctypes.c_longlong * 23)()
+        v = self._argv = (ctypes.c_longlong * 25)()
         v[0], v[3], v[4], v[11] = yp, ap, as_, self.llh
         v[14], v[15], v[16], v[17], v[18] = self.N, self.H, self.W, sp, wp
+        if self.rows is not None:
+            v[23], v[24] = self.rows.data_ptr(), int(self.psf.shape[2])
         self._argv_addr = ctypes.addressof(v)
-        self._iter_v = self.lib.gd_admm_iter_tail_v
+        self._iter_v = self.lib.gd_admm_iter_rows_v
 
     def step(self, z, rho1, rho2, rho2_next, out=None, *, rho1_next=None):
         if self.layout is None:
diff --git a/include/gdeconv.h b/include/gdeconv.h
--- a/include/gdeconv.h
+++ b/include/gdeconv.h
@@ -56,6 +56,18 @@
                       int tail);
 int gd_admm_iter_tail_v(const long long* argv);
 int gd_admm_tail_supported(int N, int H, int W, int llh);
+
+size_t gd_admm_rows_bytes(int N, int H, int W, int h);
+int gd_admm_init_rows(const float* y, const float* psf, long long psf_gstride, int h, int w,
+                      const float* alpha, long long alpha_stride, const float* rho2, long long rho2_stride,
+                      int llh, int N, int H, int W, void* state, float* zin, void* ws, void* stream, void* rows);
+int gd_admm_iter_rows(const float* y, const float* z, float* zin_or_out, const float* alpha, long long alpha_stride,
+                      const float* rho1, long long rho1_stride, const float* rho2, long long rho2_stride,
+                      const float* rho2_next, long long rho2_next_stride, int llh, int iter, int last, int N, int H,
+                      int W, void* state, void* ws, void* stream, const float* rho1_next, long long rho1_next_stride,
+                      int tail, const void* rows, int h);
+int gd_admm_iter_rows_v(const long long* argv);
+int gd_admm_rows_supported(int N, int H, int W, int h, int llh);
 
 size_t gd_admm_train_saved_bytes(int N, int H, int W);
 int gd_admm_train_init(const float* y, const float* psf, long long psf_gstride, int h, int w, const float* alpha,
@@ -143,6 +155,8 @@
 
 int gd_set_combined_tail(int on);
 
+int gd_set_rows_hh(int on);
+
 int gd_set_fused_rl(int on);
 
 int gd_set_subnet_fused_max(int n);
```

Measured after the change: 338,500 galaxies/s, median of 5. No clear change (+0.2%).
